# astra-vision/rain-rendering

Hardware: AMD Instinct MI355X
Metric: rainy frames/sec @ 1242x375, 100 mm/hr (higher is better)
Workload: dtype f64 alpha/mask, f32 colour

## Files before the change

__graft_entry__.py:

```python
import importlib
import os
import subprocess
import sys
import tempfile

ROOT = os.path.dirname(os.path.abspath(__file__))
if ROOT not in sys.path:
    sys.path.insert(0, ROOT)

CSRC = os.path.join(ROOT, 'rain-rendering_amd', 'csrc')
HIPCC = os.environ.get('HIPCC', '/opt/rocm/bin/hipcc')
HIP_FLAGS = ['--offload-arch=gfx950', '-O3', '-std=c++17', '-ffp-contract=off', '-fPIC', '-shared',
             '-Wno-unused-value', '-Wno-unused-result']


def _newer(target, sources):
    if not os.path.exists(target):
        return True
    t = os.path.getmtime(target)
    return any(os.path.getmtime(s) > t for s in sources)


def build(force=False):
    hip_src = os.path.join(CSRC, 'rainhip.hip')
    host_src = os.path.join(CSRC, 'rr_host.cpp')
    png_src = os.path.join(CSRC, 'rr_png.cpp')
    hip_dep = [hip_src, host_src, png_src] + sorted(os.path.join(CSRC, f) for f in os.listdir(CSRC) if f.endswith('.h')) + \
              [os.path.join(ROOT, 'include', 'rainhip.h')]
    lib = os.path.join(CSRC, 'librainhip.so')
    if force or _newer(lib, hip_dep):
        inc = ['-I' + os.path.join(ROOT, 'include'), '-I' + CSRC]
        objs = [os.path.join(CSRC, 'rainhip.o')]
        compile_flags = [f for f in HIP_FLAGS if f != '-shared']
        subprocess.check_call([HIPCC] + compile_flags + inc + ['-c', hip_src, '-o', objs[0]])
        for src in (host_src, png_src):
            obj = os.path.join(CSRC, os.path.basename(src)[:-4] + '.o')
            subprocess.check_call(['g++', '-O2', '-std=c++17', '-ffp-contract=off', '-fPIC', '-pthread', '-c'] + inc + [src, '-o', obj])
            objs.append(obj)
        subprocess.check_call([HIPCC, '--offload-arch=gfx950', '-fPIC', '-shared'] + objs + ['-lz', '-lpthread', '-o', lib])
    emu_src = os.path.join(ROOT, 'tests', 'hostemu', 'hostemu.cpp')
    emu = os.path.join(ROOT, 'tests', 'hostemu', 'libhostemu.so')
    if force or _newer(emu, [emu_src] + hip_dep[2:]):
        subprocess.check_call(['g++', '-O2', '-std=c++17', '-ffp-contract=off', '-fPIC', '-shared',
                               '-I' + os.path.join(ROOT, 'include'), '-I' + CSRC, emu_src, '-o', emu])
    noise_src = os.path.join(ROOT, 'tests', 'hostemu', 'noise_emu.cpp')
    noise_lib = os.path.join(ROOT, 'tests', 'hostemu', 'libnoiseemu.so')
    if force or _newer(noise_lib, [noise_src] + hip_dep[3:]):
        subprocess.check_call(['g++', '-O2', '-std=c++17', '-ffp-contract=off', '-fPIC', '-shared',
                               '-I' + os.path.join(ROOT, 'include'), '-I' + CSRC, noise_src, '-o', noise_lib])
    field_src = os.path.join(ROOT, 'tests', 'hostemu', 'field_emu.cpp')
    field_lib = os.path.join(ROOT, 'tests', 'hostemu', 'libfieldemu.so')
    if force or _newer(field_lib, [field_src] + hip_dep[3:]):
        subprocess.check_call(['g++', '-O2', '-std=c++17', '-ffp-contract=off', '-fPIC', '-shared',
                               '-I' + os.path.join(ROOT, 'include'), '-I' + CSRC, field_src, '-o', field_lib])
    rig_src = os.path.join(ROOT, 'tests', 'hostemu', 'rig_emu.cpp')
    rig_lib = os.path.join(ROOT, 'tests', 'hostemu', 'librigemu.so')
    if force or _newer(rig_lib, [rig_src] + hip_dep[3:]):
        subprocess.check_call(['g++', '-O2', '-std=c++17', '-ffp-contract=off', '-fPIC', '-shared',
                               '-I' + os.path.join(ROOT, 'include'), '-I' + CSRC, rig_src, '-o', rig_lib])
    importlib.import_module('rain-rendering_amd')
    hb = importlib.import_module('rain-rendering_amd.hip_backend')
    hb.load_library()


def smoke():
    import numpy as np
    build()
    sys.path.insert(0, os.path.join(ROOT, 'tests'))
    import helpers as h
    with tempfile.TemporaryDirectory() as tmp:
        sc = h.Scene(tmp, 96, 160, 120)
        bg, env = sc.frame_inputs(0)
        drops = sc.product_drops(0)
        rh = h.hb.RainHip(0)
        rh.set_streak_db(sc.db.streaks_light)
        rh.set_camera(sc.cam)
        out = rh.render_frames([dict(bg=bg, rainy_bg=bg, env_xyY=env, omega=sc.omega, drops=drops)])[0]
        ref = h.oracle_render(sc, 0, bg, bg, env, faithful=True)
        assert np.array_equal(out['status'], ref['status']), 'drop status mismatch'
        assert np.array_equal(out['mask'], ref['mask']), 'rainy_mask (f64) not bit-exact'
        assert np.array_equal(out['mask_i32'], ref['mask_i32']), 'rainy_mask (i32) not bit-exact'
        d = np.abs(out['image_u8'].astype(int) - ref['image_u8'].astype(int)).max()
        assert d <= 1, 'rainy_image differs by %d LSB' % d
        rh.close()
    print('smoke ok: %d drops, mask bit-exact, image max |d| = %d LSB' % (len(drops), d))


if __name__ == '__main__':
    build(force='--force' in sys.argv)
    if '--smoke' in sys.argv:
        smoke()
```

rain-rendering_amd/csrc/rainhip.hip:

```cpp
#include <hip/hip_runtime.h>

#include <dlfcn.h>

#include <cstddef>
#include <cstdio>
#include <cstdlib>
#include <algorithm>
#include <cstring>
#include <string>
#include <mutex>
#include <unordered_map>
#include <vector>

#include "rainhip.h"
#include "rr_device.h"
#include "rr_prepass.h"
#include "rr_deflate.h"
#include "rr_pngrows.h"
#include "rr_particles.h"

using namespace rr;

namespace {

// ... 59 lines not shown
    const global_ptr<const uint8_t> s = as_global(static_cast<const uint8_t*>(base)) + pix * 3;
    out[0] = (double)s[0] / 255.0; out[1] = (double)s[1] / 255.0; out[2] = (double)s[2] / 255.0;
  }
}
struct RawPx {
  uint32_t a, b, c, d, e, f;
};
typedef uint32_t u32x2_t __attribute__((ext_vector_type(2)));
__device__ inline void load_px3_raw2(const void* base, int kind, int64_t pa, int64_t pb, RawPx& qa, RawPx& qb) {
  if (kind == 0) {
    const global_ptr<const u32x2_t> s = as_global(static_cast<const u32x2_t*>(base));
    const u32x2_t a0 = s[pa * 3], a1 = s[pa * 3 + 1], a2 = s[pa * 3 + 2], b0 = s[pb * 3], b1 = s[pb * 3 + 1], b2 = s[pb * 3 + 2];
    qa = RawPx{a0.x, a0.y, a1.x, a1.y, a2.x, a2.y};
    qb = RawPx{b0.x, b0.y, b1.x, b1.y, b2.x, b2.y};
  } else if (kind == 1) {
    const global_ptr<const uint32_t> s = as_global(static_cast<const uint32_t*>(base));
    const uint32_t a0 = s[pa * 3], a1 = s[pa * 3 + 1], a2 = s[pa * 3 + 2], b0 = s[pb * 3], b1 = s[pb * 3 + 1], b2 = s[pb * 3 + 2];
    qa = RawPx{a0, a1, a2, 0u, 0u, 0u};
    qb = RawPx{b0, b1, b2, 0u, 0u, 0u};
  } else {
    const global_ptr<const uint8_t> s = as_global(static_cast<const uint8_t*>(base));
    const uint32_t a0 = s[pa * 3], a1 = s[pa * 3 + 1], a2 = s[pa * 3 + 2], b0 = s[pb * 3], b1 = s[pb * 3 + 1], b2 = s[pb * 3 + 2];
    qa = RawPx{a0, a1, a2, 0u, 0u, 0u};
    qb = RawPx{b0, b1, b2, 0u, 0u, 0u};
  }
}
__device__ inline void decode_px3(const RawPx& q, int kind, double out[3]) {
  if (kind == 0) {
    out[0] = __hiloint2double((int)q.b, (int)q.a);
    out[1] = __hiloint2double((int)q.d, (int)q.c);
    out[2] = __hiloint2double((int)q.f, (int)q.e);
  } else if (kind == 1) {
    out[0] = (double)__uint_as_float(q.a);
    out[1] = (double)__uint_as_float(q.b);
    out[2] = (double)__uint_as_float(q.c);
  } else {
    out[0] = (double)q.a / 255.0;
    out[1] = (double)q.b / 255.0;
    out[2] = (double)q.c / 255.0;
  }
}
__device__ inline int bg_kind(const FrameDesc& fr) { return (fr.in_types & RR_IN_BG_U8) ? 2 : ((fr.in_types & RR_IN_BG_F32) ? 1 : 0); }
__device__ inline int rainy_kind(const FrameDesc& fr) {
  if (fr.rainy_bg == fr.bg) return bg_kind(fr);
  return (fr.in_types & RR_IN_RAINY_U8) ? 2 : ((fr.in_types & RR_IN_RAINY_F32) ? 1 : 0);
}
typedef float float2_u __attribute__((ext_vector_type(2), aligned(4)));
typedef float float4_u __attribute__((ext_vector_type(4), aligned(4)));

__device__ inline void wave_lds_sync() {
  __builtin_amdgcn_fence(__ATOMIC_ACQ_REL, "wavefront");
  __builtin_amdgcn_wave_barrier();
}

#ifdef RR_PHASES
__device__ unsigned long long g_phase[8][8];
#define PH_DECL unsigned long long ph_t0_ = __builtin_readcyclecounter(), ph_acc_[8] = {0, 0, 0, 0, 0, 0, 0, 0};
#define PH_WAITVM asm volatile("s_waitcnt vmcnt(0)" ::: "memory");
#define PH(k)                                                   \
  {                                                             \
    const unsigned long long ph_n_ = __builtin_readcyclecounter(); \
    ph_acc_[k] += ph_n_ - ph_t0_;                               \
    ph_t0_ = ph_n_;                                             \
  }
#define PH_FLUSH(kid)                                           \
  if ((threadIdx.x & 63) == 0) {                                \
    for (int ph_q_ = 0; ph_q_ < 8; ph_q_++)                     \
      if (ph_acc_[ph_q_]) atomicAdd(&g_phase[kid][ph_q_], ph_acc_[ph_q_]); \
  }
#define PH_PARAMS , unsigned long long& ph_t0_, unsigned long long (&ph_acc_)[8]
#define PH_PASS , ph_t0_, ph_acc_
#define PH_COUNT(k) ph_acc_[k] += 1;
#else
#define PH_PARAMS
#define PH_PASS
#define PH_COUNT(k)
#define PH_DECL
#define PH_WAITVM
#define PH(k)
#define PH_FLUSH(kid)
#endif

struct Scratch {
  DropPlan* plan;
  CompRec* comp;
  CompRec32* comp32;
  int32_t* poly;
  int32_t* npts;
  int64_t* sizes;
  double* prefix;
  double* fband;
  double* arena;
  double* partial;
  double* means;
  int64_t* arena_need;
  int32_t* overflow;
  unsigned long long* need_max;
  int32_t* list_rot;
  int32_t* rot_total;
  int32_t* list_gen;
  int32_t* list_slow;
  int4* blur_items;
  int32_t* list_small;
  double* colpart;
  double* wtab;
  double* wtab_big;
  const uint8_t* tex_pad;
  const int64_t* tex_poff;
  uint4* fov_erec;
  uint32_t* fov_pix;
  int32_t* fov_list;
  int32_t* fov_list_n;
  uint8_t* blended;
  int32_t* pad_first;
  int32_t* eff_first;
  uint32_t* spans;
  int4* bbox;
  uint16_t* clist;
  int32_t* ccount;
  int32_t* counts;
  int32_t* list_big;
  int32_t* big_off;
  int32_t* bigs_list;
  int32_t* bigs_n;
  uint4* tkey;
  uint4* lrec;
  int32_t* canon;
  int32_t* htab;
  int32_t blur_bx, blur_by;
  int32_t* rows_list;
  int32_t* rows_n;
  int32_t* rows_hist;
  unsigned long long* rows_cost;
  int32_t* rows_next;
  int32_t* rows_bounds;
  int32_t* rows_fbase;
  int32_t* rows_sorted;
  const uint8_t* tex_pair;
  const int64_t* tex_qoff;
  int32_t colpart_f32;
  int32_t rows_on, n_tex;
  int32_t big_on, n_buckets;
};

__global__ __launch_bounds__(256) void k_env_prefix(const FrameDesc* frames, Dims dm, double* prefix) {
  const int lane = threadIdx.x & 63;
  const int row = blockIdx.x * 4 + (threadIdx.x >> 6), f = blockIdx.y;
  if (row >= dm.He) return;
  const FrameDesc& fr = frames[f];
  const int We = dm.We;
  const bool e32 = (fr.in_types & RR_IN_ENV_F32) != 0;
  const global_ptr<const double> env = as_global(static_cast<const double*>(fr.env)) + (int64_t)row * We * 3;
  const global_ptr<const double> om = as_global(static_cast<const double*>(fr.omega)) + (int64_t)row * We;
  const global_ptr<const float> envf = as_global(static_cast<const float*>(fr.env)) + (int64_t)row * We * 3;
  const global_ptr<const float> omf = as_global(static_cast<const float*>(fr.omega)) + (int64_t)row * We;
  double* P = prefix + ((int64_t)f * dm.He + row) * (int64_t)(We + 1) * 4;
  if (lane == 0) { P[0] = 0.0; P[1] = 0.0; P[2] = 0.0; P[3] = 0.0; }
  double carry[4] = {0, 0, 0, 0};
  for (int c0 = 0; c0 < We; c0 += 64) {
    const int c = c0 + lane;
    double v[4] = {0, 0, 0, 0};
    if (c < We) {
      const double w = e32 ? (double)omf[c] : om[c];
      v[0] = (e32 ? (double)envf[c * 3 + 0] : env[c * 3 + 0]) * w;
      v[1] = (e32 ? (double)envf[c * 3 + 1] : env[c * 3 + 1]) * w;
      v[2] = (e32 ? (double)envf[c * 3 + 2] : env[c * 3 + 2]) * w;
      v[3] = w;
    }
#pragma unroll
    for (int ofs = 1; ofs < 64; ofs <<= 1) {
#pragma unroll
      for (int k = 0; k < 4; k++) {
        const double u = __shfl_up(v[k], ofs);
        if (lane >= ofs) v[k] += u;
      }
    }
#pragma unroll
    for (int k = 0; k < 4; k++) v[k] += carry[k];
    if (c < We) {
      double* o = P + (int64_t)(c + 1) * 4;
      o[0] = v[0]; o[1] = v[1]; o[2] = v[2]; o[3] = v[3];
    }
#pragma unroll
    for (int k = 0; k < 4; k++) carry[k] = __shfl(v[k], 63);
  }
}

__global__ __launch_bounds__(256) void k_env_consts(Dims dm, const double* prefix, double* fband) {
  const int f = blockIdx.x, t = threadIdx.x;
  double sY = 0, sW = 0;
  for (int r = t; r < dm.He; r += 256) {
    const double* last = prefix + (((int64_t)f * dm.He + r) * (int64_t)(dm.We + 1) + dm.We) * 4;
    sY += last[2];
    sW += last[3];
  }
  __shared__ double a[256], b[256];
  a[t] = sY;
  b[t] = sW;
  __syncthreads();
  for (int ofs = 128; ofs > 0; ofs >>= 1) {
    if (t < ofs) {
      a[t] += a[t + ofs];
      b[t] += b[t + ofs];
    }
    __syncthreads();
  }
  if (t < COL_PARTS) {
    fband[(f * COL_PARTS + t) * 2 + 0] = t == 0 ? b[0] : 0.0;
    fband[(f * COL_PARTS + t) * 2 + 1] = t == 0 ? a[0] : 0.0;
  }
}

__device__ inline bool blur_is_slow(const DropPlan& p, const Scratch& sc) {
  return p.r1 > 0 && !blur_is_small(p) && !blur_layout(p, sc.blur_bx, sc.blur_by).fused;
}

constexpr int PLAN_DW = (int)(sizeof(DropPlan) / 4);
enum { LC_NONE = 0, LC_BIG_LDS = 1, LC_BIG = 2, LC_ROWS = 3, LC_ROT_INT = 4, LC_ROT = 5, LC_GEN = 6 };
enum { LB_NONE = 0, LB_SMALL = 1, LB_FUSED = 2, LB_SLOW = 3 };
__device__ inline uint4 make_list_rec(const DropPlan& p, const int32_t* tex_h, const int32_t* tex_w, const Scratch& sc);
__global__ __launch_bounds__(128) void k_plan(const FrameDesc* frames, Dims dm, rr_camera cam, const int32_t* tex_h,
                                              const int32_t* tex_w, int max_drops, int use_npts, Scratch sc) {
  static_assert(sizeof(DropPlan) % 4 == 0, "DropPlan layout");
  const int f = blockIdx.y;
  const int i = blockIdx.x * blockDim.x + threadIdx.x;
  const int lane = threadIdx.x & 63, wave = threadIdx.x >> 6;
  const FrameDesc& fr = frames[f];
  __shared__ uint32_t s_plan[2][32 * PLAN_DW];
  const bool act = i < fr.n_drops;
  const int64_t gi = (int64_t)f * max_drops + (act ? i : 0);
  DropPlan p;
  if (act) {
    rr_drop d = load_drop(fr.drops + i);
    int64_t size = 0;
    ExtGeom xg{false, 0, 0, 0, 0};
    if (fr.ext) {
      const rr_ext_tile& e = fr.ext[i];
      if (e.alpha) xg = ExtGeom{true, e.tw, e.th, e.min_x, e.min_y};
    }
    plan_drop<true>(d, cam, dm, tex_h, tex_w, fr.opacity, fr.strategy, p, size, xg);
    const int npts = use_npts ? sc.npts[gi] : 1;
    if (p.status != RR_DROP_OK || npts == 0) size = 0;
    if (size > 0 && blur_is_slow(p, sc)) size += ((int64_t)p.ew * p.eh + 15) & ~15LL;
    sc.sizes[gi] = size;
    uint32_t key[8];
    raw_tile_key(d, p, key);
    if (p.kind == KIND_EXT) key[0] = 0xffffffffu;
    sc.tkey[2 * gi] = make_uint4(key[0], key[1], key[2], key[3]);
    sc.tkey[2 * gi + 1] = make_uint4(key[4], key[5], key[6], key[7]);
    sc.lrec[gi] = make_list_rec(p, tex_h, tex_w, sc);
  }
  {
    const bool big = act && p.status == RR_DROP_OK && p.kind == KIND_BIG && sc.sizes[gi] > 0;
    const unsigned long long m = __ballot(big);
    if (m != 0ull) {
      int base = 0;
      if (lane == __ffsll((long long)m) - 1) base = atomicAdd(&sc.bigs_n[f], __popcll(m));
      base = __shfl(base, __ffsll((long long)m) - 1);
      if (big) sc.bigs_list[(int64_t)f * max_drops + base + __popcll(m & ((1ull << lane) - 1ull))] = i;
    }
  }
  const int wave_i0 = blockIdx.x * blockDim.x + wave * 64;
  uint32_t* stage = s_plan[wave];
  uint32_t* out = reinterpret_cast<uint32_t*>(sc.plan + (int64_t)f * max_drops + wave_i0);
#pragma unroll
  for (int half = 0; half < 2; half++) {
    if (act && (lane >> 5) == half) {
      const uint32_t* src = reinterpret_cast<const uint32_t*>(&p);
#pragma unroll
      for (int k = 0; k < PLAN_DW; k++) stage[(lane & 31) * PLAN_DW + k] = src[k];
    }
    wave_lds_sync();
    const int first = wave_i0 + half * 32;
    const int nrec = imax(imin(32, fr.n_drops - first), 0);
    for (int k = lane; k < nrec * PLAN_DW; k += 64) out[half * 32 * PLAN_DW + k] = stage[k];
    wave_lds_sync();
  }
}

__global__ __launch_bounds__(128) void k_plan_big(const FrameDesc* frames, const int32_t* tex_h, const int32_t* tex_w, int max_drops, Scratch sc) {
  const int f = blockIdx.y, j = blockIdx.x * blockDim.x + threadIdx.x;
  if (j >= sc.bigs_n[f]) return;
  const int i = sc.bigs_list[(int64_t)f * max_drops + j];
  const rr_drop d = load_drop(frames[f].drops + i);
  double mi[9];
  plan_big_homography(d, tex_w[d.tex_index], tex_h[d.tex_index], mi);
  double* o = sc.plan[(int64_t)f * max_drops + i].mi;
#pragma unroll
  for (int k = 0; k < 9; k++) o[k] = mi[k];
}

__global__ __launch_bounds__(1024) void k_scan(const FrameDesc* frames, int max_drops, int64_t arena_cap, Scratch sc) {
  const int f = blockIdx.x, t = threadIdx.x;
  const int n = frames[f].n_drops;
  const int chunk = (n + 1023) / 1024;
  const int i0 = t * chunk, i1 = min(i0 + chunk, n);
  const int64_t base = (int64_t)f * max_drops;
  int64_t s = 0;
  for (int i = i0; i < i1; i++) s += sc.sizes[base + i];
  __shared__ int64_t sh[1024];
  sh[t] = s;
  __syncthreads();
  for (int ofs = 1; ofs < 1024; ofs <<= 1) {
    int64_t v = (t >= ofs) ? sh[t - ofs] : 0;
    __syncthreads();
    sh[t] += v;
    __syncthreads();
  }
  int64_t run = ((t == 0) ? 0 : sh[t - 1]) + 16;
  const int64_t frame_base = (int64_t)f * arena_cap;
  if (t < 16 && arena_cap >= 16) sc.arena[frame_base + t] = 0.0;
  for (int i = i0; i < i1; i++) {
    DropPlan& p = sc.plan[base + i];
    int64_t sz = sc.sizes[base + i];
    if (run + sz > arena_cap) {
      sc.sizes[base + i] = 0;
    } else {
      p.a0_off = frame_base + run;
      p.a1_off = frame_base + run + (((int64_t)p.tw * p.th + 15) & ~15LL);
    }
    run += sz;
  }
  if (t == 1023) {
    const int64_t need = sh[1023] + 16;
    sc.arena_need[f] = need;
    if (need > arena_cap) {
      atomicExch(sc.overflow, 1);
      atomicMax(sc.need_max, (unsigned long long)need);
    }
  }
}

__device__ inline uint32_t raw_tile_hash(const uint4& a, const uint4& b) {
  uint32_t h = 2166136261u;
  auto mix = [&](uint32_t v) { h = (h ^ v) * 16777619u; };
  mix(a.x); mix(a.y); mix(a.z); mix(a.w); mix(b.x); mix(b.y); mix(b.z); mix(b.w);
  h ^= h >> 15;
  return h;
}
__global__ __launch_bounds__(256) void k_dedup(const FrameDesc* frames, int max_drops, int n_frames, int enable, Scratch sc) {
  const int f = blockIdx.y, i = blockIdx.x * 256 + (int)threadIdx.x;
  const int n = frames[f].n_drops;
  if (i >= n) return;
  const int gi = f * max_drops + i;
  const uint4 ka = sc.tkey[2 * (int64_t)gi], kb = sc.tkey[2 * (int64_t)gi + 1];
  int canon = gi;
  if (enable && ka.x != 0xffffffffu && sc.sizes[gi] != 0) {
    const uint32_t cap = 2u * (uint32_t)n_frames * (uint32_t)max_drops;
    uint32_t h = raw_tile_hash(ka, kb) % cap;
    for (;;) {
      const int prev = atomicCAS(&sc.htab[h], 0, gi + 1);
      if (prev == 0) break;
      const uint4 pa = sc.tkey[2 * (int64_t)(prev - 1)], pb = sc.tkey[2 * (int64_t)(prev - 1) + 1];
      if (pa.x == ka.x && pa.y == ka.y && pa.z == ka.z && pa.w == ka.w && pb.x == kb.x && pb.y == kb.y && pb.z == kb.z && pb.w == kb.w) {
        canon = prev - 1;
        break;
      }
      h = h + 1 == cap ? 0 : h + 1;
    }
    if (canon != gi) sc.plan[gi].a0_off = sc.plan[canon].a0_off;
  }
  sc.canon[gi] = canon;
  const unsigned long long dup = __ballot(canon != gi);
  if (dup != 0ull && (int)(threadIdx.x & 63) == __ffsll((long long)dup) - 1) atomicAdd(&sc.counts[f * 8 + 7], __popcll(dup));
}

constexpr int HE_MAX = 1024;
constexpr int FOV_WE_MAX = 4096;
constexpr int FOV_GROUPS = 3;

__device__ inline bool fov_rowspan_fast(const int32_t* px, const int32_t* py, int n, int y, int We, int& xl, int& xr) {
  int lo = 1 << 30, hi = -(1 << 30);
  for (int i = 0; i < n; i++) {
    const int j = (i + 1 == n) ? 0 : i + 1;
    const int x0 = px[i], y0 = py[i], x1 = px[j], y1 = py[j];
    const int ylo = imin(y0, y1), yhi = imax(y0, y1);
    if (y < ylo || y > yhi) continue;
    if (y0 == y1) {
      lo = imin(lo, imin(x0, x1));
      hi = imax(hi, imax(x0, x1));
    } else {
      const bool sw = y1 < y0;
      const int xa = sw ? x1 : x0, yA = sw ? y1 : y0, xb = sw ? x0 : x1, yB = sw ? y0 : y1;
      const int den = yB - yA;
      const int nn = 2 * (xb - xa) * (y - yA) + den;
      const int xv = xa + (int)floor((double)nn / (double)(2 * den));
      lo = imin(lo, xv);
      hi = imax(hi, xv);
    }
  }
  xl = imax(lo, 0);
  xr = imin(hi, We - 1);
  return xl <= xr;
}

template <int NCH, bool from_list>
__global__ __launch_bounds__(256) void k_fov_spans(const FrameDesc* frames, Dims dm, rr_camera cam, int max_drops, int Hp, int Dp, int use32, int cv_rule, Scratch sc) {
  const int f = blockIdx.y, wave = threadIdx.x >> 6, lane = threadIdx.x & 63;
  const FrameDesc& fr = frames[f];
  const int N = cam.n_fov, G = imin(64 / N, FOV_GROUPS);
  __shared__ double s_phi[2][RR_MAX_FOV];
  __shared__ float s_phi32[2][RR_MAX_FOV];
  __shared__ int s_px[4][FOV_GROUPS][POLY_STRIDE], s_py[4][FOV_GROUPS][POLY_STRIDE];
  __shared__ int s_xl[4][NCH * 64], s_xr[4][NCH * 64];
  __shared__ int4 s_edge[4][3 * POLY_STRIDE];
  if (threadIdx.x < RR_MAX_FOV) {
    s_phi[0][threadIdx.x] = cam.phi_cos[threadIdx.x];
    s_phi[1][threadIdx.x] = cam.phi_sin[threadIdx.x];
    s_phi32[0][threadIdx.x] = (float)cam.phi_cos[threadIdx.x];
    s_phi32[1][threadIdx.x] = (float)cam.phi_sin[threadIdx.x];
  }
  __syncthreads();
  const int n_eff = from_list ? sc.fov_list_n[f] : fr.n_drops;
  for (int wslot = blockIdx.x * 4 + wave; wslot * G < n_eff; wslot += gridDim.x * 4) {
  const int s0 = wslot * G;
  const int g = lane / N, k = lane - g * N;
  const bool act = g < G && s0 + g < n_eff;
  const int dg = act ? (from_list ? sc.fov_list[(int64_t)f * max_drops + s0 + g] : s0 + g) : 0;
  const int64_t gi = (int64_t)f * max_drops + dg;
  if (fr.strategy == 1) {
    if (act && k == 0) sc.npts[gi] = -1;
    return;
  }
  const bool ext = act && fr.ext && fr.ext[dg].alpha != nullptr;
  const int base = g * N, nxt_lane = base + (k + 1 == N ? 0 : k + 1);
  const unsigned long long gmask = act ? (((N >= 64 ? 0ull : (1ull << N)) - 1ull) << base) : 0ull;
  int ipx = 0, ipy = 0;
  bool cnd = false, vbad = true, ok = false;
  bool need64 = act && !ext && !use32;
  if (use32) {
    float azf = 0.f, erf = 0.f, pxf = 0.f, pyf = 0.f;
    int uns = 0;
    if (act && !ext) {
      FovSetup32 F;
      const rr_drop d = load_drop(fr.drops + dg);
      fov_setup32(d, (float)cam.fov_cos, (float)cam.fov_sin, F, uns);
      fov_vertex32(F, (float)cam.radius, s_phi32[0][k], s_phi32[1][k], dm.He, dm.We, azf, erf, pxf, pyf, uns);
    }
    const float az_n = __shfl(azf, act ? nxt_lane : lane), er_n = __shfl(erf, act ? nxt_lane : lane);
    bool c32 = false;
    if (act && !ext) c32 = fov_wrap_cnd32(azf, az_n, erf, er_n, uns);
    unsigned gor = 0;
#pragma unroll
// ... 656 lines not shown
  }
  for (int y = y0; y < y1; y++) row(y, RA, qa, qb);
#pragma unroll
  for (int d = 0; d < DPT; d++) {
    const int i = d0 + d * NT + t;
    if (i < d1) {
      float* o = reinterpret_cast<float*>(sc.colpart) + ((int64_t)(f * COL_PARTS + band) * 5) * max_drops + i;
#pragma unroll
      for (int k = 0; k < 4; k++) o[(int64_t)max_drops * k] = S[d][k];
      o[(int64_t)max_drops * 4] = ((any >> d) & 1u) ? 1.0f : 0.0f;
    }
  }
  {
    const int cl = (We - 1 - cw0) & ~1;
    if (chunk == 0 && We - 1 >= cw0 && cl < Cw && ((cl >> 1) & 63) == lane) {
      sc.fband[(f * COL_PARTS + band) * 2 + 0] = totw;
      sc.fband[(f * COL_PARTS + band) * 2 + 1] = totY;
    }
  }
}

__global__ __launch_bounds__(128) void k_fov_poly_general(const FrameDesc* frames, Dims dm, rr_camera cam, int max_drops, Scratch sc) {
  const int f = blockIdx.y, i = blockIdx.x * blockDim.x + threadIdx.x;
  const FrameDesc& fr = frames[f];
  if (i >= fr.n_drops) return;
  const int64_t gi = (int64_t)f * max_drops + i;
  int32_t* px = sc.poly + gi * 2 * POLY_STRIDE;
  const rr_drop d = load_drop(fr.drops + i);
  int npts = fov_polygon(d, cam, dm.He, dm.We, px, px + POLY_STRIDE);
  if (fr.strategy == 1) npts = -1;
  sc.npts[gi] = npts;
}

__global__ __launch_bounds__(256) void k_fov_sums_general(const FrameDesc* frames, Dims dm, int max_drops, Scratch sc, int cv_rule, int n_fov) {
  const int f = blockIdx.y;
  const int wave = threadIdx.x >> 6, lane = threadIdx.x & 63;
  const int i = blockIdx.x * 4 + wave;
  if (i >= frames[f].n_drops) return;
  const int64_t gi = (int64_t)f * max_drops + i;
  const int n = sc.npts[gi];
  double S[4] = {0, 0, 0, 0};
  int any = 0;
  if (n > 0) {
    const int32_t* px = sc.poly + gi * 2 * POLY_STRIDE;
    const int32_t* py = px + POLY_STRIDE;
    int ymin = lane < n ? py[lane] : 0x7fffffff, ymax = lane < n ? py[lane] : -0x7fffffff;
    for (int ofs = 32; ofs > 0; ofs >>= 1) {
      ymin = min(ymin, __shfl_xor(ymin, ofs));
      ymax = max(ymax, __shfl_xor(ymax, ofs));
    }
    const int ya = max(ymin, 0), yb = min(ymax, dm.He - 1);
    const double* P = sc.prefix + (int64_t)f * dm.He * (int64_t)(dm.We + 1) * 4;
    const bool cv = cv_rule && fov_fill_rule_cv_applies(px, py, n, n_fov, dm.He, dm.We);
    for (int y = ya + lane; y <= yb; y += 64) {
      int xl_, xr_;
      if (cv ? fov_rowspan_cv(px, py, n, y, dm.We, xl_, xr_) : fov_rowspan_fast(px, py, n, y, dm.We, xl_, xr_)) {
        any = 1;
        const double* row = P + (int64_t)y * (dm.We + 1) * 4;
        const double* hi = row + (int64_t)(xr_ + 1) * 4;
        const double* lo = row + (int64_t)xl_ * 4;
        for (int k = 0; k < 4; k++) S[k] += hi[k] - lo[k];
      }
    }
    for (int ofs = 32; ofs > 0; ofs >>= 1) {
      for (int k = 0; k < 4; k++) S[k] += __shfl_xor(S[k], ofs);
      any |= __shfl_xor(any, ofs);
    }
  }
  if (lane == 0) {
    for (int b = 0; b < COL_PARTS; b++) {
      double* o = sc.colpart + ((int64_t)(f * COL_PARTS + b) * 5) * max_drops + i;
      for (int k = 0; k < 4; k++) o[(int64_t)max_drops * k] = b == 0 ? S[k] : 0.0;
      o[(int64_t)max_drops * 4] = b == 0 ? (double)any : 0.0;
    }
  }
}

__global__ __launch_bounds__(256) void k_colour(const FrameDesc* frames, Dims dm, int max_drops, double cam_exposure, Scratch sc) {
  const int f = blockIdx.y;
  const int i = blockIdx.x * 256 + threadIdx.x;
  const FrameDesc& fr = frames[f];
  if (i >= fr.n_drops) return;
  const int64_t gi = (int64_t)f * max_drops + i;
  const DropPlan& p = sc.plan[gi];
  CompRec rec;
  rec.x0 = rec.y0 = rec.x1 = rec.y1 = 0;
  rec.ox = rec.oy = rec.pitch = rec.pad = 0;
  rec.off = 0;
  rec.tau_one = rec.g = 0;
  rec.K[0] = rec.K[1] = rec.K[2] = 0;
  rec.zdist = fr.depth ? fabs(as_global((const double*)fr.drops[i].wps)[2]) : 0.0;
  int status = p.status;
  bool blended = false;
  const int n = sc.npts[gi];
  if (n == 0) status = RR_DROP_FOV_FAIL;
  if (n < 0) {
    if (status == RR_DROP_OK && sc.sizes[gi] > 0) {
      blended = true;
      rec.K[0] = rec.K[1] = rec.K[2] = 1.0;
      rec.x0 = p.vis_x0;
      rec.y0 = p.vis_y0;
      rec.x1 = p.vis_x0 + p.vis_w;
      rec.y1 = p.vis_y0 + p.vis_h;
      rec.ox = -p.vis_x0;
      rec.oy = -p.vis_y0;
      rec.pitch = p.tw;
      rec.off = p.a0_off;
      rec.tau_one = p.tau_one;
      rec.g = p.g;
    }
  }
  if (n > 0) {
    double S[4] = {0, 0, 0, 0};
    bool any = false;
    double sumW = 0.0, sumY = 0.0;
    for (int b = 0; b < COL_PARTS; b++) {
      const int64_t at = ((int64_t)(f * COL_PARTS + b) * 5) * max_drops + i;
      if (sc.colpart_f32) {
        const float* part = reinterpret_cast<const float*>(sc.colpart) + at;
        for (int k = 0; k < 4; k++) S[k] += (double)part[(int64_t)max_drops * k];
        any = any || part[(int64_t)max_drops * 4] != 0.0f;
      } else {
        const double* part = sc.colpart + at;
        for (int k = 0; k < 4; k++) S[k] += part[(int64_t)max_drops * k];
        any = any || part[(int64_t)max_drops * 4] != 0.0;
      }
      sumW += sc.fband[(f * COL_PARTS + b) * 2 + 0];
      sumY += sc.fband[(f * COL_PARTS + b) * 2 + 1];
    }
    if (!any) status = RR_DROP_EMPTY_FOV;
    if (status == RR_DROP_OK && sc.sizes[gi] > 0) {
      blended = true;
      colour_from_sums(S, sumW, sumY / sumW, rec.K);
      if (p.r1 > 0) {
        const int fx0 = p.vis_x0 - p.crop_x + (p.shift - p.r2), fy0 = p.vis_y0 - p.crop_y + (p.shift - p.r1);
        rec.x0 = imax(p.vis_x0, fx0);
        rec.y0 = imax(p.vis_y0, fy0);
        rec.x1 = imin(p.vis_x0 + p.vis_w, fx0 + p.ew);
        rec.y1 = imin(p.vis_y0 + p.vis_h, fy0 + p.eh);
        if (rec.x1 <= rec.x0 || rec.y1 <= rec.y0) { rec.x0 = rec.y0 = rec.x1 = rec.y1 = 0; }
        rec.ox = -(fx0 - p.epad);
        rec.oy = -fy0;
        rec.pitch = p.epitch;
        rec.off = p.a1_off;
      } else {
        const int rx0 = p.vis_x0 - p.crop_x + p.shift, ry0 = p.vis_y0 - p.crop_y + p.shift;
        rec.x0 = imax(p.vis_x0, rx0);
        rec.y0 = imax(p.vis_y0, ry0);
        rec.x1 = imin(p.vis_x0 + p.vis_w, rx0 + p.tw);
        rec.y1 = imin(p.vis_y0 + p.vis_h, ry0 + p.th);
        if (rec.x1 <= rec.x0 || rec.y1 <= rec.y0) { rec.x0 = rec.y0 = rec.x1 = rec.y1 = 0; }
        rec.ox = -rx0;
        rec.oy = -ry0;
        rec.pitch = p.tw;
        rec.off = p.a0_off;
      }
      rec.tau_one = p.tau_one;
      rec.g = p.g;
    }
  }
  {
    const double BIG = 1.0e50;
    const bool tame = fabs(rec.tau_one) < BIG && (rec.tau_one == 0.0 || rec.tau_one > 1.0e-200) && fabs(rec.g) < BIG &&
                      fabs(rec.K[0]) < BIG && fabs(rec.K[1]) < BIG && fabs(rec.K[2]) < BIG && p.kind != KIND_EXT;
    rec.pad = tame ? 0 : 1;
  }
  sc.comp[gi] = rec;
// ... 105 lines not shown
constexpr int BIG_ROWS_MAX_PX = 8192;
__device__ inline bool tile_is_big_lds(const DropPlan& p, int sh, int sw) {
  return p.kind == KIND_BIG && (int64_t)(sh + 4) * (sw + 4) + 48 <= RW_PAIR_BYTES && p.tw >= 1 && p.th >= 1 && (int64_t)p.tw * p.th <= BIG_ROWS_MAX_PX && p.bw0 >= 1;
}
__global__ __launch_bounds__(256) void k_pair_textures(const uint8_t* texels, const int32_t* tex_h, const int32_t* tex_w,
                                                       const int64_t* tex_off, const int64_t* tex_qoff, uint8_t* pairs) {
  const int i = blockIdx.x, sh = tex_h[i], sw = tex_w[i], P = pair_pitch(sw);
  const uint8_t* g = texels + tex_off[i];
  uint16_t* dst = reinterpret_cast<uint16_t*>(pairs + tex_qoff[i]);
  for (int k = threadIdx.x; k < (sh + 3) * P; k += 256) {
    const int y = k / P - 2, x = k - (y + 2) * P - 2;
    const bool xin = x >= 0 && x < sw;
    const uint32_t lo = (xin && y >= 0 && y < sh) ? g[y * sw + x] : 0u, hi = (xin && y + 1 >= 0 && y + 1 < sh) ? g[(y + 1) * sw + x] : 0u;
    dst[k] = (uint16_t)(lo | (hi << 8));
  }
}

__global__ __launch_bounds__(256) void k_pad_textures(const uint8_t* texels, const int32_t* tex_h, const int32_t* tex_w,
                                                      const int64_t* tex_off, const int64_t* tex_poff, uint8_t* pad) {
  const int i = blockIdx.x, sh = tex_h[i], sw = tex_w[i], P = sw + 4;
  const uint8_t* g = texels + tex_off[i];
  uint8_t* dst = pad + tex_poff[i];
  for (int k = threadIdx.x; k < (sh + 4) * P; k += 256) {
    const int y = k / P - 2, x = k - (y + 2) * P - 2;
    dst[k] = (y >= 0 && y < sh && x >= 0 && x < sw) ? g[y * sw + x] : (uint8_t)0;
  }
}
__device__ inline void load_tex_copy(uint8_t* s_tex, const uint8_t* gpad, int sh, int sw) {
  const int n16 = ((sh + 4) * (sw + 4) + 15) >> 4;
  const uint4* g = reinterpret_cast<const uint4*>(gpad);
  uint4* d = reinterpret_cast<uint4*>(s_tex);
  for (int k = threadIdx.x; k < n16; k += 256) d[k] = g[k];
}

__device__ inline double lds_rot_sample(const uint8_t* s_tex, const double* s_lut, int P, int sh, int sw, int X0, int Y0,
                                        int2 d) {
  const int X = (X0 + d.x) >> 5, Y = (Y0 + d.y) >> 5;
  int sx = X >> 5, sy = Y >> 5;
  const int fx = X & 31, fy = Y & 31;
  sx = imin(imax(sx, -2), sw);
  sy = imin(imax(sy, -2), sh);
  const uint8_t* q = s_tex + (sy + 2) * P + (sx + 2);
  const double v00 = s_lut[q[0]], v01 = s_lut[q[1]], v10 = s_lut[q[P]], v11 = s_lut[q[P + 1]];
  const double ax_ = (double)(32 - fx), bx_ = (double)fx, ay_ = (double)(32 - fy), by_ = (double)fy;
  const double sm = ((v00 * (ay_ * ax_) + v01 * (ay_ * bx_)) + v10 * (by_ * ax_)) + v11 * (by_ * bx_);
  return sm * (1.0 / 1024.0);
}

__device__ inline void lds_rot_sample2(const uint8_t* s_tex, const double* s_lut, int P, int sh, int sw, int XA, int YA, int2 dA,
                                       int XB, int YB, int2 dB, double& outA, double& outB) {
  const int Xa = (XA + dA.x) >> 5, Ya = (YA + dA.y) >> 5, Xb = (XB + dB.x) >> 5, Yb = (YB + dB.y) >> 5;
  const int sxa = imin(imax(Xa >> 5, -2), sw), sya = imin(imax(Ya >> 5, -2), sh);
  const int sxb = imin(imax(Xb >> 5, -2), sw), syb = imin(imax(Yb >> 5, -2), sh);
  const uint8_t* qa = s_tex + (sya + 2) * P + (sxa + 2);
  const uint8_t* qb = s_tex + (syb + 2) * P + (sxb + 2);
  const int a0 = qa[0], a1 = qa[1], a2 = qa[P], a3 = qa[P + 1];
  const int b0 = qb[0], b1 = qb[1], b2 = qb[P], b3 = qb[P + 1];
  const double va0 = s_lut[a0], va1 = s_lut[a1], va2 = s_lut[a2], va3 = s_lut[a3];
  const double vb0 = s_lut[b0], vb1 = s_lut[b1], vb2 = s_lut[b2], vb3 = s_lut[b3];
  const int fxa = Xa & 31, fya = Ya & 31, fxb = Xb & 31, fyb = Yb & 31;
  const double axa = (double)(32 - fxa), bxa = (double)fxa, aya = (double)(32 - fya), bya = (double)fya;
  const double axb = (double)(32 - fxb), bxb = (double)fxb, ayb = (double)(32 - fyb), byb = (double)fyb;
  const double sa = ((va0 * (aya * axa) + va1 * (aya * bxa)) + va2 * (bya * axa)) + va3 * (bya * bxa);
  const double sb = ((vb0 * (ayb * axb) + vb1 * (ayb * bxb)) + vb2 * (byb * axb)) + vb3 * (byb * bxb);
  outA = sa * (1.0 / 1024.0);
  outB = sb * (1.0 / 1024.0);
}

constexpr int GEN_SLICES = 16;
__global__ __launch_bounds__(256) void k_tile_generic(const FrameDesc* frames, int max_drops, const uint8_t* texels,
                                                      const int32_t* tex_h, const int32_t* tex_w, const int64_t* tex_off,
                                                      const float* ctab, Scratch sc) {
  const int f = blockIdx.y, t = threadIdx.x;
  __shared__ double s_lut[256];
  __shared__ __attribute__((aligned(16))) uint8_t s_tex[TEX_LDS];
  __shared__ int2 s_adbd[NW_MAX];
  const int n_items = sc.counts[f * 8 + 1];
  if ((int)blockIdx.x >= n_items * GEN_SLICES) return;
  s_lut[t] = (double)t / 255.0;
  for (int work = blockIdx.x; work < n_items * GEN_SLICES; work += gridDim.x) {
  const int item = work / GEN_SLICES, slice = work - item * GEN_SLICES;
  const int li = sc.list_gen[(int64_t)f * max_drops + item];
  const int64_t gi = (int64_t)f * max_drops + li;
  const DropPlan& p = sc.plan[gi];
  if (p.kind == KIND_EXT) {
    const double* src = frames[f].ext[li].alpha;
    double* A0e = sc.arena + p.a0_off;
    for (int idx = t + 256 * slice; idx < p.tw * p.th; idx += 256 * GEN_SLICES) A0e[idx] = clip01(src[idx]);
    continue;
  }
  const int sh = tex_h[p.tex], sw = tex_w[p.tex];
  __syncthreads();
  const uint8_t* gtex = texels + tex_off[p.tex];
  const int P = sw + 4;
  const bool tex_fits = (sh + 4) * P <= TEX_LDS && !(p.kind == KIND_BIG && p.tw * p.th * 12 < sh * sw);
  if (tex_fits) load_tex_copy(s_tex, sc.tex_pad + sc.tex_poff[p.tex], sh, sw);
  double* A0 = sc.arena + p.a0_off;
  const bool area_fast = tex_fits && p.kind == KIND_ROT && p.rs_mode == RS_AREA_FAST && p.nW <= NW_MAX && tile_coords_safe(p);
  if (area_fast)
    for (int rx = t; rx < p.nW; rx += 256) s_adbd[rx] = make_int2((int)rot_adelta(p, rx), (int)rot_bdelta(p, rx));
  __syncthreads();
  const int n = p.tw * p.th;
  if (area_fast) {
    const int area = p.isx * p.isy, n4 = area & ~3;
    const float scale = 1.0f / (float)area;
    for (int idx = t + 256 * slice; idx < n; idx += 256 * GEN_SLICES) {
      const int dy = idx / p.tw, dx = idx - dy * p.tw;
      double sum = 0.0, q0 = 0.0, q1 = 0.0, q2 = 0.0;
      int k = 0;
      for (int ky = 0; ky < p.isy; ky++) {
        const int c = dy * p.isy + ky;
        const int ry = p.flip ? (p.nH - 1 - c) : c;
        const int X0 = (int)rot_X0(p, ry), Y0 = (int)rot_Y0(p, ry);
        for (int kx = 0; kx < p.isx; kx++, k++) {
          const double v = lds_rot_sample(s_tex, s_lut, P, sh, sw, X0, Y0, s_adbd[dx * p.isx + kx]);
          if (k >= n4) sum = sum + v;
          else {
            const int m = k & 3;
            if (m == 0) q0 = v;
            else if (m == 1) q1 = v;
            else if (m == 2) q2 = v;
            else sum = sum + (((q0 + q1) + q2) + v);
          }
        }
      }
      A0[dy * p.tw + dx] = clip01(sum * (double)scale);
    }
  } else if (tex_fits) {
    TexLutPad tx{s_tex, s_lut, sh, sw};
    for (int idx = t + 256 * slice; idx < n; idx += 256 * GEN_SLICES) {
      int y = idx / p.tw, x = idx - y * p.tw;
      A0[idx] = raw_tile_pixel(p, tx, ctab, x, y);
    }
  } else {
    TexLut tx{gtex, s_lut, sh, sw};
    for (int idx = t + 256 * slice; idx < n; idx += 256 * GEN_SLICES) {
      int y = idx / p.tw, x = idx - y * p.tw;
      A0[idx] = raw_tile_pixel(p, tx, ctab, x, y);
    }
  }
  }
}


struct TexLutWide {
  const uint8_t* t;
  const double* lut;
  int h, w;
  __device__ double at(int64_t y, int64_t x) const { return lut[t[y * w + x]]; }
  __device__ void at4(int64_t y, int64_t x, double v[4]) const {
    uint32_t u;
    __builtin_memcpy(&u, as_global(t) + (y * w + x), 4);
    v[0] = lut[u & 0xffu]; v[1] = lut[(u >> 8) & 0xffu]; v[2] = lut[(u >> 16) & 0xffu]; v[3] = lut[u >> 24];
  }
  __device__ double tap(int64_t y, int64_t x) const {
    if (y < 0 || y >= h || x < 0 || x >= w) return 0.0;
    return at(y, x);
  }
};

__global__ __launch_bounds__(256) void k_tile_big(const FrameDesc* frames, int max_drops, const uint8_t* texels,
                                                  const int32_t* tex_h, const int32_t* tex_w, const int64_t* tex_off,
                                                  const float* ctab, Scratch sc) {
  const int f = blockIdx.y, t = threadIdx.x;
  __shared__ double s_lut[256];
  __shared__ float s_ctab[128];
  const int n_big = sc.counts[f * 8 + 5], total = sc.counts[f * 8 + 6];
  if (total == 0) return;
  s_lut[t] = (double)t / 255.0;
  if (t < 128) s_ctab[t] = ctab[t];
  const int32_t* lbig = sc.list_big + (int64_t)f * max_drops;
  const int32_t* boff = sc.big_off + (int64_t)f * max_drops + f;
  const int lane = t & 63;
  __syncthreads();
  PH_DECL
  for (int pb = blockIdx.x * 256; pb < total; pb += gridDim.x * 256) {
    const int pix0 = pb + (t & ~63);
    if (pix0 >= total) continue;
    int lo = 0, hi = n_big;
    while (hi - lo > 1) {
      const int step = (hi - lo + 63) >> 6, idx = lo + lane * step;
      const bool le = idx < hi && boff[idx] <= pix0;
      const int cnt = __popcll(__ballot(le));
      lo += (cnt - 1) * step;
      hi = imin(hi, lo + step);
    }
    PH(0)
    const int pix = pb + t;
    if (pix >= total) continue;
    int j = lo;
    while (boff[j + 1] <= pix) j++;
    const int64_t gi = (int64_t)f * max_drops + lbig[j];
    const DropPlan& p = sc.plan[gi];
    const int local = pix - boff[j];
    const int y = local / p.tw, x = local - y * p.tw;
    TexLutWide tx{texels + tex_off[p.tex], s_lut, tex_h[p.tex], tex_w[p.tex]};
    PH(1)
    sc.arena[p.a0_off + local] = warp_big_pixel(p, tx, s_ctab, x, y);
    PH(2)
  }
  PH_FLUSH(1)
}

__global__ __launch_bounds__(256) void k_tile(const FrameDesc* frames, int max_drops, const uint8_t* texels,
                                              const int32_t* tex_h, const int32_t* tex_w, const int64_t* tex_off,
                                              Scratch sc) {
  const int t = threadIdx.x, lane = t & 63, wave = t >> 6;
  __shared__ DropPlan sp;
  __shared__ double s_lut[256];
  __shared__ __attribute__((aligned(16))) uint8_t s_tex[TEX_LDS];
  __shared__ int2 s_adbd[NW_MAX];
  __shared__ AreaSpan s_ax[TW_MAX];
  __shared__ double s_buf[BUF_MAX];
  __shared__ double s_can[4][CAN_W];
  __shared__ int4 s_row[4][ROWS_S];
  const int n_items = *sc.rot_total;
  if ((int)blockIdx.x >= n_items) return;
  s_lut[t] = (double)t / 255.0;
  PH_DECL
  for (int item = blockIdx.x; item < n_items; item += gridDim.x) {
  const int64_t gi = sc.list_rot[item];
  __syncthreads();
  PH(7)
  {
    const int32_t* src = reinterpret_cast<const int32_t*>(&sc.plan[gi]);
    int32_t* dst = reinterpret_cast<int32_t*>(&sp);
    for (int k = t; k < (int)(sizeof(DropPlan) / 4); k += 256) dst[k] = src[k];
  }
  __syncthreads();
  const DropPlan& p = sp;
  const int sh = tex_h[p.tex], sw = tex_w[p.tex];
  const int P = sw + 4;
  load_tex_copy(s_tex, sc.tex_pad + sc.tex_poff[p.tex], sh, sw);
  double* A0 = sc.arena + p.a0_off;
  const int tw = p.tw, th = p.th;
  const double sy_scale = p.scale_y;
  for (int rx = t; rx < p.nW; rx += 256) s_adbd[rx] = make_int2((int)rot_adelta(p, rx), (int)rot_bdelta(p, rx));
  for (int dx = t; dx < tw; dx += 256) s_ax[dx] = area_span(p.nW, p.scale_x, dx);
  __syncthreads();
  PH(0)
  const RowGeom geom = row_geom(p, sh, sw);
  const int pitch = imin(imax(tile_pitch(p, sh, sw), 1), CAN_W);
  const int Rw = imax(imin(ROWS_W, CAN_W / pitch), 1);
  const float inv_pitch = 1.0f / (float)pitch;
  double* can = s_can[wave];
  int4* rowp = s_row[wave];
  if (p.rs_mode == RS_AREA_FAST) {
    const int isx = p.isx, isy = p.isy, area = isx * isy, n4 = area & ~3;
    const float scale = 1.0f / (float)area;
    const int nsplit = th >= 3 ? 1 : (th == 2 ? 2 : 4);
    const int rows_par = 4 / nsplit;
    for (int dyb = 0; dyb < th; dyb += rows_par) {
      const int dy = dyb + wave / nsplit, part = wave % nsplit;
      const int dx0 = (part * tw) / nsplit, dx1 = ((part + 1) * tw) / nsplit;
      if (dy >= th || dx1 <= dx0) continue;
      const int colA = dx0 * isx, colB = dx1 * isx;
      const int pitch2 = imax(imin(pitch, colB - colA), 1);
      const int Rw2 = imax(imin(ROWS_W, CAN_W / pitch2), 1);
      const float inv_pitch2 = 1.0f / (float)pitch2;
      double sum = 0.0, q0 = 0.0, q1 = 0.0, q2 = 0.0;
      int k = 0;
      for (int c0 = dy * isy; c0 < (dy + 1) * isy; c0 += Rw2) {
        const int nr = imin(Rw2, (dy + 1) * isy - c0);
        if (lane < nr) {
          const int c = c0 + lane;
          const int ry = p.flip ? (p.nH - 1 - c) : c;
          const int X0 = (int)rot_X0(p, ry), Y0 = (int)rot_Y0(p, ry);
          int xa, n;
          row_interval(p, geom, X0, Y0, xa, n);
          const int xa2 = imax(xa, colA), xe2 = imin(xa + n, colB);
          rowp[lane] = make_int4(X0, Y0, xa2, imax(imin(xe2 - xa2, pitch2), 0));
        }
        wave_lds_sync();
        const int nidx = nr * pitch2;
        for (int idx = lane; idx < nidx; idx += 128) {
          const int ia = idx, ib = imin(idx + 64, nidx - 1);
          const int ra = (int)(((float)ia + 0.5f) * inv_pitch2), xa = ia - ra * pitch2;
          const int rb = (int)(((float)ib + 0.5f) * inv_pitch2), xb = ib - rb * pitch2;
          const int4 rwa = rowp[ra], rwb = rowp[rb];
          const bool oka = xa < rwa.w, okb = (idx + 64 < nidx) && xb < rwb.w;
          const int2 da = s_adbd[rwa.z + (oka ? xa : 0)], db = s_adbd[rwb.z + (okb ? xb : 0)];
          double va, vb;
          lds_rot_sample2(s_tex, s_lut, P, sh, sw, rwa.x, rwa.y, da, rwb.x, rwb.y, db, va, vb);
          if (oka) can[ia] = va;
          if (okb) can[ib] = vb;
        }
        wave_lds_sync();
        const bool mine = lane < dx1 - dx0;
        const int colL = (dx0 + lane) * isx;
        for (int r = 0; r < nr; r++) {
          const int4 rw = rowp[r];
          const double* row = can + r * pitch2 - rw.z;
          const int vlo = mine ? rw.z : (1 << 30), vhi = rw.z + rw.w;
          auto at = [&](int col) { return (col >= vlo && col < vhi) ? row[col] : 0.0; };
          int kx = 0;
          while (kx < isx) {
            if ((k & 3) == 0 && kx + 3 < isx && k + 3 < n4) {
              const double v0 = at(colL + kx), v1 = at(colL + kx + 1), v2 = at(colL + kx + 2), v3 = at(colL + kx + 3);
              sum = sum + (((v0 + v1) + v2) + v3);
              kx += 4;
              k += 4;
              continue;
            }
            const double v = at(colL + kx);
            if (k >= n4) sum = sum + v;
            else {
              const int m = k & 3;
              if (m == 0) q0 = v;
              else if (m == 1) q1 = v;
              else if (m == 2) q2 = v;
// ... 379 lines not shown
    for (int k = 0; k < NP; k++) {
      const int bx = tw <= bw0 ? 0 : div_by_f(x, bw0, inv_bw) * bw0;
      c[k] = warp_big_coord(p, bx, x, y);
      x += dr;
      y += dq;
      if (x >= tw) { x -= tw; y += 1; }
    }
    uint32_t u[NP][4];
    float cx[NP][4], cy[NP][4];
#pragma unroll
    for (int k = 0; k < NP; k++) {
      const uint8_t* col = tex00 + med3i(c[k].sx, -4, sw);
#pragma unroll
      for (int i = 0; i < 4; i++) {
        const uint32_t a = (uint32_t)(uintptr_t)(const __attribute__((address_space(3))) uint8_t*)(col + med3i(c[k].sy + i, -2, sh + 1) * P);
        const uint32_t* q = (const uint32_t*)(__attribute__((address_space(3))) uint32_t*)(uintptr_t)(a & ~3u);
        const uint32_t lo = q[0], hi = q[1];
        u[k][i] = __builtin_amdgcn_alignbit(hi, lo, (a & 3u) * 8u);
      }
      const float4 a = *reinterpret_cast<const float4*>(s_ctab + c[k].fx * 4), b = *reinterpret_cast<const float4*>(s_ctab + c[k].fy * 4);
      cx[k][0] = a.x; cx[k][1] = a.y; cx[k][2] = a.z; cx[k][3] = a.w;
      cy[k][0] = b.x; cy[k][1] = b.y; cy[k][2] = b.z; cy[k][3] = b.w;
    }
#pragma unroll
    for (int k = 0; k < NP; k++) {
      double pr[4][4];
#pragma unroll
      for (int i = 0; i < 4; i++) big_row_products(u[k][i], cy[k][i], cx[k], three, pr[i]);
      const bool interior = c[k].sx >= 0 && c[k].sx < width1 && c[k].sy >= 0 && c[k].sy < height1;
      double sum = 0.0;
      if (interior) {
#pragma unroll
        for (int i = 0; i < 4; i++) {
          double r = (pr[i][0] + pr[i][1]) + pr[i][2];
          r = r + pr[i][3];
          sum = (i == 0) ? r : sum + r;
        }
      } else {
#pragma unroll
        for (int i = 0; i < 4; i++)
#pragma unroll
          for (int j = 0; j < 4; j++) sum = sum + pr[i][j];
      }
      const int it = it0 + 64 * k + lane;
      if (it < n) A0[it] = clip01(sum);
    }
  }
  PH(7)
}

__global__ __launch_bounds__(1024) void k_tile_rows(int n_shares, const int32_t* tex_h, const int32_t* tex_w, const float* ctab, Scratch sc) {
  __shared__ __attribute__((aligned(16))) RowsShared S;
  const int t = threadIdx.x, lane = t & 63, wave = t >> 6;
  if ((uint32_t)(uintptr_t)(__attribute__((address_space(3))) double*)S.lut != 0u) __builtin_trap();
  S.lut[t & 255] = (double)(t & 255) / 255.0;
  RowsWave& W = S.w[wave];
  uint32_t three = 3;
  asm volatile("" : "+v"(three));
  constexpr int DONE = 0x7fffffff;
  PH_DECL
  if (t == 0) S.cur = -1;
  for (;;) {
    __syncthreads();
    if (t == 0) {
      const int share = (int)atomicAdd(sc.rows_next, 1);
      const bool any = share < n_shares;
      S.next = any ? sc.rows_bounds[share] : 0;
      S.end = any ? sc.rows_bounds[share + 1] : 0;
      S.first = any ? 1 : 0;
    }
    __syncthreads();
    if (!S.first) break;
    const int end = S.end;
    int pending = -1, ptex = -1, gi = 0;
    bool ctab_ok = false;
    for (;;) {
      if (pending < 0) {
        int i = 0;
        if (lane == 0) i = atomicAdd(&S.next, 1);
        i = __builtin_amdgcn_readfirstlane(i);
        if (i < end) {
          pending = i;
          gi = __builtin_amdgcn_readfirstlane(sc.rows_sorted[i]);
          ptex = __builtin_amdgcn_readfirstlane(as_constant(&sc.plan[gi])->tex);
          if (__builtin_amdgcn_readfirstlane(as_constant(&sc.plan[gi])->kind) == KIND_BIG) ptex += sc.n_tex;
        } else {
          pending = DONE;
        }
      }
      if (pending != DONE && ptex == S.cur) {
        DropPlan p;
        {
          const const_ptr<uint32_t> src = as_constant(reinterpret_cast<const uint32_t*>(&sc.plan[gi]));
          uint32_t* dst = reinterpret_cast<uint32_t*>(&p);
#pragma unroll
          for (int k = 0; k < (int)(sizeof(DropPlan) / 4); k++) dst[k] = src[k];
        }
        PH(0)
        if (ptex < sc.n_tex) {
          rows_tile(p, tex_h[ptex], tex_w[ptex], S, W, sc.arena, three PH_PASS);
          ctab_ok = false;
        } else {
          float* s_ctab = reinterpret_cast<float*>(W.buf);
          if (!ctab_ok) {
            wave_lds_sync();
            s_ctab[lane] = ctab[lane];
            s_ctab[lane + 64] = ctab[lane + 64];
            wave_lds_sync();
            ctab_ok = true;
          }
          big_tile<RR_BIG_NP>(p, tex_h[ptex - sc.n_tex], tex_w[ptex - sc.n_tex], S.pair, s_ctab, sc.arena, three PH_PASS);
        }
        pending = -1;
        continue;
      }
      if (lane == 0) { S.pend[wave] = pending; S.ptex[wave] = ptex; }
      __syncthreads();
      int m = DONE, mtex = -1;
      for (int k = 0; k < RW_WAVES; k++)
        if (S.pend[k] < m) { m = S.pend[k]; mtex = S.ptex[k]; }
      if (m == DONE) break;
      if (mtex < sc.n_tex) {
        const int64_t nb = pair_bytes(tex_h[mtex], tex_w[mtex]);
        const uint4* g = reinterpret_cast<const uint4*>(sc.tex_pair + sc.tex_qoff[mtex]);
        uint4* d = reinterpret_cast<uint4*>(S.pair);
        for (int k = t; k < (int)(nb >> 4); k += 1024) d[k] = g[k];
      } else {
        const int bt = mtex - sc.n_tex;
        const int n16 = ((tex_h[bt] + 4) * (tex_w[bt] + 4) + 2 + 15) >> 4;
        const uint4* g = reinterpret_cast<const uint4*>(sc.tex_pad + sc.tex_poff[bt]);
        uint4* d = reinterpret_cast<uint4*>(S.pair);
        if (t == 0) d[0] = uint4{0u, 0u, 0u, 0u};
        for (int k = t; k < n16; k += 1024) d[k + 1] = g[k];
      }
      if (t == 0) S.cur = mtex;
      __syncthreads();
      PH(5)
    }
  }
  PH_FLUSH(5)
}

constexpr int BLUR_ITEMS_PER_DROP = 8;

__device__ inline int blur_subtiles(const DropPlan& p, const BlurLayout& L) {
  return ((p.ew + L.wo - 1) / L.wo) * ((p.eh + L.ho - 1) / L.ho);
}

__device__ inline uint4 make_list_rec(const DropPlan& p, const int32_t* tex_h, const int32_t* tex_w, const Scratch& sc) {
  if (p.status != RR_DROP_OK) return make_uint4(0u, 0u, 0u, 0u);
  const int sh = tex_h[p.tex], sw = tex_w[p.tex];
  uint32_t cls, cost = 0u, bcls = LB_NONE, bwh = 0u, bns = 0u;
  if (p.kind == KIND_BIG) {
    if (sc.big_on && tile_is_big_lds(p, sh, sw)) { cls = LC_BIG_LDS; cost = (uint32_t)(RR_BIG_COST * ((p.tw * p.th + 63) / 64) + 4); }
    else { cls = LC_BIG; cost = (uint32_t)(p.tw * p.th); }
  } else if (sc.rows_on && p.kind != KIND_EXT && tile_is_rows(p, sh, sw)) { cls = LC_ROWS; cost = (uint32_t)rows_tile_cost(p, sh, sw); }
  else if (p.kind != KIND_EXT && tile_is_fast(p, sh, sw)) cls = p.rs_mode == RS_AREA_FAST ? LC_ROT_INT : LC_ROT;
  else cls = LC_GEN;
  if (p.r1 > 0) {
    if (blur_is_small(p)) bcls = LB_SMALL;
    else {
      const BlurLayout L = blur_layout(p, sc.blur_bx, sc.blur_by);
      if (L.fused) { bcls = LB_FUSED; bwh = (uint32_t)L.wo | ((uint32_t)L.ho << 16); bns = (uint32_t)blur_subtiles(p, L); }
      else bcls = LB_SLOW;
    }
  }
  return make_uint4(cls | (bcls << 4) | ((uint32_t)p.tex << 8), cost, bwh, bns);
}

__global__ __launch_bounds__(1024) void k_lists(const FrameDesc* frames, int max_drops, const int32_t* tex_h, const int32_t* tex_w,
                                                Scratch sc) {
  const int f = blockIdx.x, t = threadIdx.x;
  const int n = frames[f].n_drops;
  const int chunk = (n + 1023) / 1024;
  const int i0 = t * chunk, i1 = min(i0 + chunk, n);
  const int64_t base = (int64_t)f * max_drops;
  __shared__ int s_hist[RW_TEX_MAX], s_cost[RW_TEX_MAX];
  if (sc.rows_on) {
    for (int k = t; k < sc.n_buckets; k += 1024) s_hist[k] = s_cost[k] = 0;
    __syncthreads();
  }
  constexpr int NC = 11;
  int c[NC] = {0, 0, 0, 0, 0, 0, 0, 0, 0, 0, 0};
  for (int i = i0; i < i1; i++) {
    const uint4 r = sc.lrec[base + i];
    const uint32_t cls = r.x & 15u, bcls = (r.x >> 4) & 7u;
    if (cls == LC_NONE || sc.sizes[base + i] == 0) continue;
    const int tex = (int)(r.x >> 8);
    if (sc.canon[base + i] == (int)(base + i)) {
      if (cls == LC_BIG_LDS) {
        c[9]++;
        c[10] += sc.plan[base + i].tw * sc.plan[base + i].th;
        atomicAdd(&s_hist[sc.n_tex + tex], 1);
        atomicAdd(&s_cost[sc.n_tex + tex], (int)r.y);
      } else if (cls == LC_BIG) { c[6]++; c[7] += (int)r.y; }
      else if (cls == LC_ROWS) {
        c[8]++;
        atomicAdd(&s_hist[tex], 1);
        atomicAdd(&s_cost[tex], (int)r.y);
      }
      else if (cls == LC_ROT_INT) c[5]++;
      else if (cls == LC_ROT) c[0]++;
      else c[1]++;
    }
    if (bcls == LB_SMALL) c[4]++;
    else if (bcls == LB_FUSED) c[2] += imin((int)r.w, BLUR_ITEMS_PER_DROP);
    else if (bcls == LB_SLOW) c[3]++;
  }
  __shared__ int sh[1024][NC];
  for (int k = 0; k < NC; k++) sh[t][k] = c[k];
  __syncthreads();
  for (int ofs = 1; ofs < 1024; ofs <<= 1) {
    int v[NC] = {0, 0, 0, 0, 0, 0, 0, 0, 0, 0, 0};
    if (t >= ofs)
      for (int k = 0; k < NC; k++) v[k] = sh[t - ofs][k];
    __syncthreads();
    for (int k = 0; k < NC; k++) sh[t][k] += v[k];
    __syncthreads();
  }
  int o[NC];
  for (int k = 0; k < NC; k++) o[k] = (t == 0) ? 0 : sh[t - 1][k];
  const int n_int = sh[1023][5];
  const int n_rot_rows = sh[1023][8];
  o[0] += n_int;
  __shared__ int s_rot_base;
  if (t == 0) s_rot_base = atomicAdd(sc.rot_total, sh[1023][0] + sh[1023][5]);
  __syncthreads();
  int32_t* lrot = sc.list_rot + s_rot_base;
  int32_t* lgen = sc.list_gen + base;
  int32_t* lslow = sc.list_slow + base;
  int32_t* lsmall = sc.list_small + base;
  int32_t* lbig = sc.list_big + base;
  int32_t* lrows = sc.rows_list + base;
  int32_t* boff = sc.big_off + base + f;
  int4* items = sc.blur_items + base * BLUR_ITEMS_PER_DROP;
  for (int i = i0; i < i1; i++) {
    const uint4 r = sc.lrec[base + i];
    const uint32_t cls = r.x & 15u, bcls = (r.x >> 4) & 7u;
    if (cls == LC_NONE || sc.sizes[base + i] == 0) continue;
    if (sc.canon[base + i] == (int)(base + i)) {
      if (cls == LC_BIG_LDS) lrows[n_rot_rows + o[9]++] = i;
      else if (cls == LC_BIG) {
        boff[o[6]] = o[7];
        lbig[o[6]++] = i;
        o[7] += (int)r.y;
      } else if (cls == LC_ROWS) lrows[o[8]++] = i;
      else if (cls == LC_ROT_INT) lrot[o[5]++] = (int32_t)(base + i);
      else if (cls == LC_ROT) lrot[o[0]++] = (int32_t)(base + i);
      else lgen[o[1]++] = i;
    }
    if (bcls == LB_SMALL) lsmall[o[4]++] = i;
    else if (bcls == LB_FUSED) {
      const int ns = (int)r.w;
      const int ni = imin(ns, BLUR_ITEMS_PER_DROP);
      const int per = (ns + ni - 1) / ni;
      for (int k = 0; k < ni; k++) {
        const int st0 = k * per;
        items[o[2]++] = make_int4(i, st0, imax(imin(per, ns - st0), 0), (int)r.z);
      }
    } else if (bcls == LB_SLOW) lslow[o[3]++] = i;
  }
  if (t == 1023) {
    for (int k = 0; k < 5; k++) sc.counts[f * 8 + k] = sh[1023][k];
    sc.counts[f * 8 + 0] = sh[1023][0] + sh[1023][5];
    sc.counts[f * 8 + 5] = sh[1023][6];
    sc.counts[f * 8 + 6] = sh[1023][7];
    boff[sh[1023][6]] = sh[1023][7];
    sc.rows_n[3 * f] = sh[1023][8];
    sc.rows_n[3 * f + 1] = sh[1023][9];
    sc.rows_n[3 * f + 2] = sh[1023][10];
  }
  if (sc.rows_on) {
    for (int k = t; k < sc.n_buckets; k += 1024) {
      const int cnt = s_hist[k];
      sc.rows_fbase[(int64_t)f * RW_TEX_MAX + k] = cnt ? atomicAdd(&sc.rows_hist[k], cnt) : 0;
      if (cnt) atomicAdd(&sc.rows_cost[k], (unsigned long long)s_cost[k]);
    }
  }
}

__global__ __launch_bounds__(1024) void k_rows_scatter(int max_drops, Scratch sc) {
  const int f = blockIdx.x, t = threadIdx.x;
  __shared__ int s_start[RW_TEX_MAX], s_rank[RW_TEX_MAX];
  const int nf = sc.rows_n[3 * f] + sc.rows_n[3 * f + 1];
  if (nf == 0) return;
  const int own = t < sc.n_buckets ? sc.rows_hist[t] : 0;
  s_start[t] = own;
  __syncthreads();
  for (int ofs = 1; ofs < 1024; ofs <<= 1) {
    const int v = t >= ofs ? s_start[t - ofs] : 0;
    __syncthreads();
    s_start[t] += v;
    __syncthreads();
  }
  const int excl = s_start[t] - own;
  __syncthreads();
  s_start[t] = excl;
  s_rank[t] = t < sc.n_buckets ? sc.rows_fbase[(int64_t)f * RW_TEX_MAX + t] : 0;
  __syncthreads();
  const int64_t base = (int64_t)f * max_drops;
  for (int j = t; j < nf; j += 1024) {
    const int i = sc.rows_list[base + j];
    const DropPlan& p = sc.plan[base + i];
    const int tex = p.tex + (p.kind == KIND_BIG ? sc.n_tex : 0);
    const int pos = s_start[tex] + atomicAdd(&s_rank[tex], 1);
    sc.rows_sorted[pos] = (int32_t)(base + i);
  }
}

__device__ void gauss_half_table(double sigma, int r, double* hw ) {
  const int t = threadIdx.x;
  for (int k = t; k <= r; k += blockDim.x) hw[k] = gauss_phi(sigma, r - k);
  __syncthreads();
  __shared__ double s_tot;
  if (t == 0) {
    double tot = 0.0;
    for (int x = -r; x <= r; x++) tot = tot + hw[r - (x < 0 ? -x : x)];
    s_tot = tot;
  }
  __syncthreads();
  const double tot = s_tot;
  for (int k = t; k <= r; k += blockDim.x) hw[k] = hw[k] / tot;
  __syncthreads();
}


constexpr int BW_LANES = 4;
__global__ __launch_bounds__(256) void k_blur_weights(const FrameDesc* frames, int max_drops, Scratch sc) {
  constexpr int NG = 256 / BW_LANES;
  __shared__ double s_hw[NG][BR_MAX + 2];
  const int f = blockIdx.y, grp = threadIdx.x / BW_LANES, l = threadIdx.x % BW_LANES;
  const int idx = blockIdx.x * NG + grp;
  const int i = idx >> 1, axis = idx & 1;
  int r = 0;
  double sigma = 0.0;
  const int64_t gi = (int64_t)f * max_drops + (i < frames[f].n_drops ? i : 0);
  if (i < frames[f].n_drops) {
    const DropPlan& p = sc.plan[gi];
    if (p.status == RR_DROP_OK && sc.sizes[gi] != 0 && p.r1 > 0 && p.r1 <= BR_MAX) {
      r = axis ? p.r2 : p.r1;
      sigma = axis ? p.sig2 : p.sig1;
    }
  }
  double* tab = s_hw[grp];
  for (int k = l; k <= r && r > 0; k += BW_LANES) tab[k] = gauss_phi(sigma, r - k);
  wave_lds_sync();
  if (l == 0 && r > 0) {
    double tot = 0.0;
    for (int x = -r; x <= r; x++) tot = tot + tab[r - (x < 0 ? -x : x)];
    tab[BR_MAX + 1] = tot;
  }
  wave_lds_sync();
  if (r > 0) {
    const double tot = tab[BR_MAX + 1];
    double* hw = sc.wtab + (gi * 2 + axis) * (BR_MAX + 1);
    for (int k = l; k <= r; k += BW_LANES) hw[k] = tab[k] / tot;
  }
}

template <class W>
__device__ inline void blur4(const double* c0, int st, W hw, int r, double& acc0, double& acc1, double& acc2, double& acc3) {
  auto at = [&](int k) { return c0[__mul24(k, st)]; };
  const double wc = hw(r);
  acc0 = c0[0] * wc; acc1 = at(1) * wc; acc2 = at(2) * wc; acc3 = at(3) * wc;
  double a0 = at(-r), a1 = at(1 - r), a2 = at(2 - r), a3 = at(3 - r);
  double b0 = at(r), b1 = at(1 + r), b2 = at(2 + r), b3 = at(3 + r);
  int ii = -r;
  for (; ii + 3 < 0; ii += 4) {
    const double w0 = hw(ii + r), w1 = hw(ii + 1 + r), w2 = hw(ii + 2 + r), w3 = hw(ii + 3 + r);
    const double na0 = at(4 + ii), na1 = at(5 + ii), na2 = at(6 + ii), na3 = at(7 + ii);
    const double nb0 = at(-ii - 1), nb1 = at(-ii - 2), nb2 = at(-ii - 3), nb3 = at(-ii - 4);
    acc0 = acc0 + (a0 + b0) * w0; acc1 = acc1 + (a1 + b1) * w0; acc2 = acc2 + (a2 + b2) * w0; acc3 = acc3 + (a3 + b3) * w0;
    acc0 = acc0 + (a1 + nb0) * w1; acc1 = acc1 + (a2 + b0) * w1; acc2 = acc2 + (a3 + b1) * w1; acc3 = acc3 + (na0 + b2) * w1;
    acc0 = acc0 + (a2 + nb1) * w2; acc1 = acc1 + (a3 + nb0) * w2; acc2 = acc2 + (na0 + b0) * w2; acc3 = acc3 + (na1 + b1) * w2;
    acc0 = acc0 + (a3 + nb2) * w3; acc1 = acc1 + (na0 + nb1) * w3; acc2 = acc2 + (na1 + nb0) * w3; acc3 = acc3 + (na2 + b0) * w3;
    a0 = na0; a1 = na1; a2 = na2; a3 = na3;
    b3 = nb0; b2 = nb1; b1 = nb2; b0 = nb3;
  }
  for (; ii < 0; ii++) {
    const double w = hw(ii + r);
    const double na = at(4 + ii);
    const double nb = at(-ii - 1);
    acc0 = acc0 + (a0 + b0) * w;
    acc1 = acc1 + (a1 + b1) * w;
    acc2 = acc2 + (a2 + b2) * w;
    acc3 = acc3 + (a3 + b3) * w;
    a0 = a1; a1 = a2; a2 = a3; a3 = na;
    b3 = b2; b2 = b1; b1 = b0; b0 = nb;
  }
}

template <int NO, class W>
__device__ inline void blur_n(const double* c0, int st, W hw, int r, double (&acc)[NO]) {
  const double wc = hw(r);
#pragma unroll
  for (int j = 0; j < NO; j++) acc[j] = c0[__mul24(j, st)] * wc;
  for (int ii = -r; ii < 0; ii++) {
    const double w = hw(ii + r);
#pragma unroll
    for (int j = 0; j < NO; j++) acc[j] = acc[j] + (c0[__mul24(j + ii, st)] + c0[__mul24(j - ii, st)]) * w;
  }
}

__device__ inline void glds_dword(const void* src, uint32_t lds_byte) {
  uint32_t keep;
  asm volatile("s_mov_b32 %0, m0\n\ts_mov_b32 m0, %2\n\ts_nop 0\n\tglobal_load_lds_dword %1, off\n\ts_mov_b32 m0, %0"
               : "=&s"(keep)
               : "v"(src), "s"(__builtin_amdgcn_readfirstlane((int)lds_byte))
               : "memory");
}
__device__ inline void glds_dwordx4(const void* src, uint32_t lds_byte) {
  uint32_t keep;
  asm volatile("s_mov_b32 %0, m0\n\ts_mov_b32 m0, %2\n\ts_nop 0\n\tglobal_load_lds_dwordx4 %1, off\n\ts_mov_b32 m0, %0"
               : "=&s"(keep)
               : "v"(src), "s"(__builtin_amdgcn_readfirstlane((int)lds_byte))
               : "memory");
}
__global__ __launch_bounds__(256, 4) void k_blur_fused_dma(const FrameDesc* frames, int max_drops, Scratch sc) {
  const int f = blockIdx.y, t = threadIdx.x, lane = t & 63, G = gridDim.x;
  const int wave = __builtin_amdgcn_readfirstlane(t >> 6);
  extern __shared__ __attribute__((aligned(16))) double s_dyn[];
  constexpr int TAB = 2 * (BR_MAX + 1);
  double* tabs = s_dyn;
  double* X = s_dyn + 2 * TAB;
  double* Y = X + sc.blur_bx;
  const uint32_t lds_tabs = (uint32_t)(uintptr_t)(__attribute__((address_space(3))) double*)tabs;
  const uint32_t lds_x = (uint32_t)(uintptr_t)(__attribute__((address_space(3))) double*)X;
  const int n_items = sc.counts[f * 8 + 2];
  if ((int)blockIdx.x >= n_items) return;
  const global_ptr<const uint32_t> items_w = as_global(reinterpret_cast<const uint32_t*>(sc.blur_items + (int64_t)f * max_drops * BLUR_ITEMS_PER_DROP));
  const DropPlan* plans = sc.plan + (int64_t)f * max_drops;
  auto load_item = [&](int item) { return items_w[(int64_t)item * 4 + (lane & 3)]; };
  auto load_plan = [&](int i) { return as_global(reinterpret_cast<const uint32_t*>(plans + i))[lane]; };
  struct PlanView {
    int r1, r2, ew, eh, tw, th, epitch, epad;
    long long a0_off, a1_off;
  };
  auto unpack = [&](uint32_t pv) {
    auto F = [&](size_t byte_off) { return (int)__builtin_amdgcn_readlane((int)pv, (int)(byte_off / 4)); };
    PlanView o;
    o.r1 = F(offsetof(DropPlan, r1)); o.r2 = F(offsetof(DropPlan, r2)); o.ew = F(offsetof(DropPlan, ew)); o.eh = F(offsetof(DropPlan, eh));
    o.tw = F(offsetof(DropPlan, tw)); o.th = F(offsetof(DropPlan, th)); o.epitch = F(offsetof(DropPlan, epitch)); o.epad = F(offsetof(DropPlan, epad));
    o.a0_off = (long long)(((unsigned long long)(unsigned)F(offsetof(DropPlan, a0_off) + 4) << 32) | (unsigned)F(offsetof(DropPlan, a0_off)));
    o.a1_off = (long long)(((unsigned long long)(unsigned)F(offsetof(DropPlan, a1_off) + 4) << 32) | (unsigned)F(offsetof(DropPlan, a1_off)));
    return o;
  };
  auto item_of = [&](uint32_t iv) {
    return make_int4((int)__builtin_amdgcn_readlane((int)iv, 0), (int)__builtin_amdgcn_readlane((int)iv, 1),
                     (int)__builtin_amdgcn_readlane((int)iv, 2), (int)__builtin_amdgcn_readlane((int)iv, 3));
  };
  struct Geo {
    int y0, x0, ho, wo, hop, hi, yp, xa, wd, nx, xs, ys, e_lo, e_hi;
  };
  auto geo = [&](const PlanView& p, int Lwo, int Lho, int st) {
    Geo g;
    const int ntx = (p.ew + Lwo - 1) / Lwo;
    const int sty = st / ntx, stx = st - sty * ntx;
    g.y0 = sty * Lho; g.x0 = stx * Lwo;
    g.ho = imin(Lho, p.eh - g.y0);
    g.wo = imin(Lwo, p.ew - g.x0);
    g.hop = (g.ho + 3) & ~3;
    const int wi = g.wo + 2 * p.r2;
    g.hi = g.hop + 2 * p.r1;
    g.yp = blur_y_pitch(g.wo, p.r2);
    g.xa = imax(0, 2 * p.r2 - g.x0);
    const int xb = imin(wi, p.tw + 2 * p.r2 - g.x0);
    g.wd = imax(xb - g.xa, 0);
    g.nx = g.wd * g.hi;
    g.xs = g.x0 - 2 * p.r2 + g.xa; g.ys = g.y0 - 2 * p.r1;
    const int ra = imin(imax(-g.ys, 0), g.hi), rb = imax(imin(p.th - g.ys, g.hi), ra);
    g.e_lo = ra * g.wd; g.e_hi = rb * g.wd;
    return g;
  };
  auto stage = [&](const PlanView& p, const Geo& g, int drop, bool tables, int tb) {
    if (g.e_hi > g.e_lo && g.wd == p.tw) {
      const char* src = reinterpret_cast<const char*>(sc.arena + p.a0_off + (int64_t)g.ys * p.tw);
      const int a = (g.e_lo + 1) & ~1, b = g.e_hi & ~1;
      for (int e0 = (a & ~511); e0 < b; e0 += 512) {
        const int e = e0 + wave * 128 + 2 * lane;
        if (e >= a && e < b) glds_dwordx4(src + (int64_t)e * 8, lds_x + (uint32_t)(e0 + wave * 128) * 8u);
      }
      if (wave == 0 && (g.e_lo & 1) && lane < 2) glds_dword(src + (int64_t)g.e_lo * 8 + lane * 4, lds_x + (uint32_t)g.e_lo * 8u);
      if (wave == 1 && (g.e_hi & 1) && g.e_hi - 1 >= g.e_lo && lane < 2) glds_dword(src + (int64_t)(g.e_hi - 1) * 8 + lane * 4, lds_x + (uint32_t)(g.e_hi - 1) * 8u);
    } else if (g.e_hi > g.e_lo) {
      const int wdd = imax(g.wd, 1);
      const float inv_wd = 1.0f / (float)wdd;
      const int dq = (int)((128.0f + 0.5f) * inv_wd), dr = 128 - dq * wdd;
      const char* src = reinterpret_cast<const char*>(sc.arena + p.a0_off) + (lane & 1) * 4;
      const int c0 = g.e_lo >> 7, c1 = (g.e_hi + 127) >> 7;
      int e = c0 * 128 + wave * 32 + (lane >> 1);
      int yy = (int)(((float)e + 0.5f) * inv_wd), xc = e - yy * wdd;
      for (int c = c0; c < c1; c++) {
        if (e >= g.e_lo && e < g.e_hi)
          glds_dword(src + (int64_t)((g.ys + yy) * p.tw + (g.xs + xc)) * 8, lds_x + (uint32_t)(c * 128 + wave * 32) * 8u);
        e += 128;
        xc += dr;
        yy += dq;
        if (xc >= wdd) { xc -= wdd; yy += 1; }
      }
    }
    if (tables) {
      const char* wt = reinterpret_cast<const char*>(sc.wtab + ((int64_t)f * max_drops + drop) * TAB);
      if (wave == 3 && lane < TAB / 2) glds_dwordx4(wt + lane * 16, lds_tabs + (uint32_t)(tb * TAB) * 8u);
    }
  };
  uint32_t iv0 = load_item(blockIdx.x);
  uint32_t pv0 = load_plan((int)__builtin_amdgcn_readlane((int)iv0, 0));
  uint32_t iv1 = load_item(imin((int)blockIdx.x + G, n_items - 1));
  uint32_t pv1 = load_plan((int)__builtin_amdgcn_readlane((int)iv1, 0));
  uint32_t iv2 = load_item(imin((int)blockIdx.x + 2 * G, n_items - 1));
  int it = blockIdx.x;
  int4 item = item_of(iv0);
  PlanView p = unpack(pv0);
  int st = item.y, tb = 0;
  Geo g = geo(p, item.w & 0xffff, item.w >> 16, st);
  stage(p, g, item.x, true, tb);
  PH_DECL
  for (;;) {
    const int r1 = p.r1, r2 = p.r2;
    const double* hw1 = tabs + tb * TAB;
    const double* hw2 = hw1 + (BR_MAX + 1);
    {
      const int nz2 = (g.yp * g.hop + 1) >> 1;
      double2* Y2 = reinterpret_cast<double2*>(Y);
      for (int i = t; i < nz2; i += 256) Y2[i] = make_double2(0.0, 0.0);
    }
    asm volatile("s_waitcnt vmcnt(0)" ::: "memory");
// ... 12 lines not shown
        has_next = false;
      }
    }
    {
      iv1 = new_item ? iv2 : iv1;
      pv1 = load_plan((int)__builtin_amdgcn_readlane((int)iv1, 0));
      iv2 = load_item(imin(new_item ? it + 3 * G : it + 2 * G, n_items - 1));
    }
    for (int i = t; i < g.e_lo; i += 256) X[i] = 0.0;
    for (int i = g.e_hi + t; i < g.nx; i += 256) X[i] = 0.0;
    PH(0)
    __syncthreads();
    PH(1)
    {
      const int wd = g.wd, nrb = g.hop >> 2, nv = nrb * wd;
      const float inv_wd = 1.0f / (float)imax(wd, 1);
      for (int idx = t; idx < nv; idx += 256) {
        const int rb = (int)(((float)idx + 0.5f) * inv_wd), xq = idx - rb * wd;
        const double* c0 = X + (4 * rb + r1) * wd + xq;
        double acc0, acc1, acc2, acc3;
        blur4(c0, wd, [&](int k) { return hw1[k]; }, r1, acc0, acc1, acc2, acc3);
        double* o = Y + 4 * rb * g.yp + g.xa + xq;
        o[0] = acc0;
        o[g.yp] = acc1;
        o[2 * g.yp] = acc2;
        o[3 * g.yp] = acc3;
      }
    }
    PH(2)
    __syncthreads();
    PH(3)
    Geo ng = g;
    if (has_next) {
      ng = geo(np, nitem.w & 0xffff, nitem.w >> 16, nst);
      stage(np, ng, nitem.x, ntb != tb, ntb);
    }
    PH(6)
    {
      const int ncb = (g.wo + 3) >> 2, nh = ncb * g.ho;
      const float inv_ho = 1.0f / (float)g.ho;
      double* dst = sc.arena + p.a1_off;
      for (int idx = t; idx < nh; idx += 256) {
        const int cb = (int)(((float)idx + 0.5f) * inv_ho), yq = idx - cb * g.ho;
        const double* c0 = Y + yq * g.yp + 4 * cb + r2;
        double acc0, acc1, acc2, acc3;
        if (r2 > 0) {
          blur4(c0, 1, [&](int k) { return hw2[k]; }, r2, acc0, acc1, acc2, acc3);
        } else {
          acc0 = c0[0]; acc1 = c0[1]; acc2 = c0[2]; acc3 = c0[3];
        }
        const int xo = 4 * cb;
        double* o = dst + (int64_t)(g.y0 + yq) * p.epitch + p.epad + (g.x0 + xo);
        if (xo + 3 < g.wo) {
          o[0] = acc0; o[1] = acc1; o[2] = acc2; o[3] = acc3;
        } else {
          o[0] = acc0;
          if (xo + 1 < g.wo) o[1] = acc1;
          if (xo + 2 < g.wo) o[2] = acc2;
        }
      }
    }
    PH(4)
    if (!has_next) break;
    __syncthreads();
    PH(5)
    if (new_item) it += G;
    item = nitem; p = np; st = nst; tb = ntb; g = ng;
  }
  PH_FLUSH(3)
}

typedef double double2_v __attribute__((ext_vector_type(2)));
struct SmallItem {
  int li, r1, r2, tw, th, pw, ph, epitch, epad;
  long long a0, a1;
};
__global__ __launch_bounds__(256, 4) void k_blur_small(const FrameDesc* frames, int max_drops, Scratch sc) {
  const int f = blockIdx.y, lane = threadIdx.x & 63, wave = threadIdx.x >> 6;
  __shared__ __attribute__((aligned(16))) double Xs[4][BS_X], Ys[4][BS_Y];
  double* X = Xs[wave];
  double* Y = Ys[wave];
  const int n_items = sc.counts[f * 8 + 4];
  const global_ptr<const int32_t> list = as_global(sc.list_small + (int64_t)f * max_drops);
  const DropPlan* plans = sc.plan + (int64_t)f * max_drops;
  const int stride = gridDim.x * 4;
  int it = blockIdx.x * 4 + wave;
  if (it >= n_items) return;
  auto load_plan = [&](int li) { return as_global(reinterpret_cast<const uint32_t*>(plans + li))[lane]; };
  auto unpack = [&](uint32_t pv, int li) {
    auto F = [&](size_t byte_off) { return (int)__builtin_amdgcn_readlane((int)pv, (int)(byte_off / 4)); };
    static_assert(offsetof(DropPlan, a1_off) + 8 <= 256, "DropPlan layout");
    SmallItem o;
    o.li = li;
    o.r1 = F(offsetof(DropPlan, r1)); o.r2 = F(offsetof(DropPlan, r2)); o.tw = F(offsetof(DropPlan, tw)); o.th = F(offsetof(DropPlan, th));
    o.pw = F(offsetof(DropPlan, ew)); o.ph = F(offsetof(DropPlan, eh)); o.epitch = F(offsetof(DropPlan, epitch)); o.epad = F(offsetof(DropPlan, epad));
    o.a0 = (long long)(((unsigned long long)(unsigned)F(offsetof(DropPlan, a0_off) + 4) << 32) | (unsigned)F(offsetof(DropPlan, a0_off)));
    o.a1 = (long long)(((unsigned long long)(unsigned)F(offsetof(DropPlan, a1_off) + 4) << 32) | (unsigned)F(offsetof(DropPlan, a1_off)));
    return o;
  };
  double2_v R[4];
  double nw1 = 0.0, nw2 = 0.0;
  auto issue = [&](const SmallItem& d) {
    const global_ptr<const double2_v> raw2 = as_global(reinterpret_cast<const double2_v*>(sc.arena + d.a0));
    const int n = d.tw * d.th;
#pragma unroll
    for (int j = 0; j < 4; j++) {
      const int k2 = lane + 64 * j;
      R[j] = double2_v{0.0, 0.0};
      if (2 * k2 < n) R[j] = raw2[k2];
    }
    const global_ptr<const double> wt = as_global(sc.wtab + ((int64_t)f * max_drops + d.li) * 2 * (BR_MAX + 1));
    nw1 = (lane <= d.r1) ? wt[d.r1 - lane] : 0.0;
    nw2 = (d.r2 > 0 && lane <= d.r2) ? wt[(BR_MAX + 1) + d.r2 - lane] : 0.0;
  };
  PH_DECL
  const int li0 = __builtin_amdgcn_readfirstlane(list[it]);
  SmallItem cur = unpack(load_plan(li0), li0);
  issue(cur);
  bool has_next = it + stride < n_items;
  int li1 = has_next ? __builtin_amdgcn_readfirstlane(list[it + stride]) : li0;
  uint32_t pv_next = load_plan(li1);
  int32_t li2_v = (it + 2 * stride < n_items) ? list[it + 2 * stride] : 0;
  for (;;) {
    const int r1 = cur.r1, r2 = cur.r2, pw = cur.pw, ph = cur.ph, tw = cur.tw, th = cur.th;
    const int php = (ph + 3) & ~3, hi = php + 2 * r1, yp = blur_y_pitch(pw, r2);
    double* tile = sc.arena + cur.a1;
    {
      const int n = tw * th, top = 2 * r1 * tw;
      double2* X2 = reinterpret_cast<double2*>(X);
#pragma unroll
      for (int j = 0; j < 4; j++) {
        const int k2 = lane + 64 * j;
        if (2 * k2 < n) X2[(top >> 1) + k2] = make_double2(R[j].x, 2 * k2 + 1 < n ? R[j].y : 0.0);
      }
      for (int i = lane; i < (top >> 1); i += 64) X2[i] = make_double2(0.0, 0.0);
      const int e0 = (top + n + 1) >> 1, e1 = (tw * hi + 1) >> 1;
      for (int i = e0 + lane; i < e1; i += 64) X2[i] = make_double2(0.0, 0.0);
      const int nz2 = (yp * php + 1) >> 1;
      double2* Y2 = reinterpret_cast<double2*>(Y);
      for (int i = lane; i < nz2; i += 64) Y2[i] = make_double2(0.0, 0.0);
    }
    const double w1 = nw1, w2 = nw2;
    wave_lds_sync();
    PH(0)
    SmallItem nxt = cur;
    if (has_next) {
      nxt = unpack(pv_next, li1);
      issue(nxt);
      if (it + 2 * stride < n_items) {
        li1 = __builtin_amdgcn_readfirstlane(li2_v);
        pv_next = load_plan(li1);
        if (it + 3 * stride < n_items) li2_v = list[it + 3 * stride];
      }
    }
    const float inv_tw = 1.0f / (float)tw;
    const int nv4 = (php >> 2) * tw;
    if (nv4 <= 16) {
      const int idx = lane;
      if (idx < 4 * nv4) {
        const int row = (int)(((float)idx + 0.5f) * inv_tw), x = idx - row * tw;
        double a[1];
        blur_n<1>(X + (__mul24(row + r1, tw) + x), tw, [&](int k) { return readlane_f64(w1, r1 - k); }, r1, a);
        Y[__mul24(row, yp) + 2 * r2 + x] = a[0];
      }
    } else if (nv4 <= 32) {
      const int idx = lane;
      if (idx < 2 * nv4) {
        const int rb = (int)(((float)idx + 0.5f) * inv_tw), x = idx - rb * tw;
        double a[2];
        blur_n<2>(X + (__mul24(2 * rb + r1, tw) + x), tw, [&](int k) { return readlane_f64(w1, r1 - k); }, r1, a);
        double* o = Y + (__mul24(2 * rb, yp) + 2 * r2 + x);
        o[0] = a[0];
        o[yp] = a[1];
      }
    } else {
      const int nv = nv4;
      for (int idx = lane; idx < nv; idx += 64) {
        const int rb = (int)(((float)idx + 0.5f) * inv_tw), x = idx - rb * tw;
        const double* c0 = X + (__mul24(4 * rb + r1, tw) + x);
        double a0, a1, a2, a3;
        blur4(c0, tw, [&](int k) { return readlane_f64(w1, r1 - k); }, r1, a0, a1, a2, a3);
        double* o = Y + (__mul24(4 * rb, yp) + 2 * r2 + x);
        o[0] = a0;
        o[yp] = a1;
        o[2 * yp] = a2;
        o[3 * yp] = a3;
      }
    }
    wave_lds_sync();
    PH(1)
    const int ncb = (pw + 3) >> 2, nh = ncb * ph;
    const float inv_ph = 1.0f / (float)ph;
    if (nh <= 16 && r2 > 0) {
      const int idx = lane;
      if (idx < pw * ph) {
        const int x = (int)(((float)idx + 0.5f) * inv_ph), yq = idx - x * ph;
        double a[1];
        blur_n<1>(Y + (__mul24(yq, yp) + x + r2), 1, [&](int k) { return readlane_f64(w2, r2 - k); }, r2, a);
        tile[(int64_t)yq * cur.epitch + cur.epad + x] = a[0];
      }
    } else if (nh <= 32 && r2 > 0) {
      const int idx = lane, nc2 = (pw + 1) >> 1;
      if (idx < nc2 * ph) {
        const int cb = (int)(((float)idx + 0.5f) * inv_ph), yq = idx - cb * ph, xo = 2 * cb;
        double a[2];
        blur_n<2>(Y + (__mul24(yq, yp) + xo + r2), 1, [&](int k) { return readlane_f64(w2, r2 - k); }, r2, a);
        double* o = tile + (int64_t)yq * cur.epitch + cur.epad + xo;
        o[0] = a[0];
        if (xo + 1 < pw) o[1] = a[1];
      }
    } else {
      for (int idx = lane; idx < nh; idx += 64) {
        const int cb = (int)(((float)idx + 0.5f) * inv_ph), yq = idx - cb * ph;
        const double* c0 = Y + (__mul24(yq, yp) + 4 * cb + r2);
        double a0, a1, a2, a3;
        if (r2 > 0) {
          blur4(c0, 1, [&](int k) { return readlane_f64(w2, r2 - k); }, r2, a0, a1, a2, a3);
        } else {
          a0 = c0[0]; a1 = c0[1]; a2 = c0[2]; a3 = c0[3];
        }
        const int xo = 4 * cb;
        double* o = tile + (int64_t)yq * cur.epitch + cur.epad + xo;
        if (xo + 3 < pw) {
          o[0] = a0; o[1] = a1; o[2] = a2; o[3] = a3;
        } else {
          o[0] = a0;
          if (xo + 1 < pw) o[1] = a1;
          if (xo + 2 < pw) o[2] = a2;
        }
      }
    }
    wave_lds_sync();
    PH(2)
    if (!has_next) break;
    it += stride;
    cur = nxt;
    has_next = it + stride < n_items;
  }
  PH_FLUSH(2)
}

constexpr int BIG_GROUPS = 64;
constexpr int BIG_ROWS = 16;
constexpr int BIG_COL_LDS = 2048;

template <class F>
__device__ inline void visit_taps(int a0, int a1, int b0, int b1, int r, F f) {
  a0 = imax(a0, -r); a1 = imin(a1, -1);
  b0 = imax(b0, -r); b1 = imin(b1, -1);
  if (a0 > a1) { a0 = b0; a1 = b1; b0 = 0; b1 = -1; }
  if (b0 <= b1 && b0 < a0) { int t = a0; a0 = b0; b0 = t; t = a1; a1 = b1; b1 = t; }
  if (b0 <= b1 && b0 <= a1 + 1) { a1 = imax(a1, b1); b0 = 0; b1 = -1; }
  for (int ii = a0; ii <= a1; ii++) f(ii);
  for (int ii = b0; ii <= b1; ii++) f(ii);
}

constexpr int SLOW_CAP = 256;
__global__ __launch_bounds__(256) void k_blur_big_weights(const FrameDesc* frames, int max_drops, Scratch sc) {
  const int f = blockIdx.y;
  __shared__ double hw[MAX_R + 1];
  const int n_items = imin(sc.counts[f * 8 + 3], SLOW_CAP);
  for (int w = blockIdx.x; w < 2 * n_items; w += gridDim.x) {
    const int it = w >> 1, axis = w & 1;
    const DropPlan& p = sc.plan[(int64_t)f * max_drops + sc.list_slow[(int64_t)f * max_drops + it]];
    const int r = axis ? p.r2 : p.r1;
    __syncthreads();
    if (r > 0) {
      gauss_half_table(axis ? p.sig2 : p.sig1, r, hw);
      double* o = sc.wtab_big + (((int64_t)f * SLOW_CAP + it) * 2 + axis) * (MAX_R + 1);
      for (int k = threadIdx.x; k <= r; k += 256) o[k] = hw[k];
    }
  }
}

template <int AXIS>
__global__ __launch_bounds__(256) void k_blur(const FrameDesc* frames, int max_drops, Scratch sc) {
  const int f = blockIdx.y, t = threadIdx.x;
  __shared__ double hw[MAX_R + 1];
  __shared__ double s_in[BIG_COL_LDS];
  const int n_items = sc.counts[f * 8 + 3];
  int cur = -1;
  for (int w = blockIdx.x; w < n_items * BIG_GROUPS; w += gridDim.x) {
    const int it = w / BIG_GROUPS, g = w - it * BIG_GROUPS;
    const int64_t gi = (int64_t)f * max_drops + sc.list_slow[(int64_t)f * max_drops + it];
    const DropPlan& p = sc.plan[gi];
    const int r = AXIS == 0 ? p.r1 : p.r2;
    const int tw = p.tw, th = p.th, ew = p.ew, eh = p.eh, r1 = p.r1, r2 = p.r2;
    if (AXIS == 0 ? g >= tw : g * BIG_ROWS >= eh) continue;
    const double* raw = sc.arena + p.a0_off;
    double* fin = sc.arena + p.a1_off;
    double* tmp = fin + (((int64_t)p.epitch * eh + 15) & ~15LL);
    __syncthreads();
    if (cur != it) {
      if (r > 0) {
        if (it < SLOW_CAP) {
          const double* wt = sc.wtab_big + (((int64_t)f * SLOW_CAP + it) * 2 + AXIS) * (MAX_R + 1);
          for (int k = t; k <= r; k += 256) hw[k] = wt[k];
          __syncthreads();
        } else {
          gauss_half_table(AXIS == 0 ? p.sig1 : p.sig2, r, hw);
        }
      }
      cur = it;
    }
    if (AXIS == 0) {
      for (int rx = g; rx < tw; rx += BIG_GROUPS) {
        const bool lds = th <= BIG_COL_LDS;
        __syncthreads();
        if (lds)
          for (int k = t; k < th; k += 256) s_in[k] = raw[(int64_t)k * tw + rx];
        __syncthreads();
        auto R = [&](int yy) -> double {
          const int ry = yy - r1;
          return (ry >= 0 && ry < th) ? (lds ? s_in[ry] : raw[(int64_t)ry * tw + rx]) : 0.0;
        };
        for (int y = t; y < eh; y += 256) {
          double acc = R(y) * hw[r];
          visit_taps(r1 - y, r1 - y + th - 1, y - r1 - th + 1, y - r1, r, [&](int ii) { acc = acc + (R(y + ii) + R(y - ii)) * hw[ii + r]; });
          tmp[(int64_t)y * tw + rx] = acc;
        }
      }
    } else {
      for (int y0 = g * BIG_ROWS; y0 < eh; y0 += BIG_GROUPS * BIG_ROWS) {
        const int nr = imin(BIG_ROWS, eh - y0);
        const bool lds = nr * tw <= BIG_COL_LDS;
        __syncthreads();
        if (lds)
          for (int k = t; k < nr * tw; k += 256) s_in[k] = tmp[(int64_t)y0 * tw + k];
        __syncthreads();
        for (int idx = t; idx < nr * ew; idx += 256) {
          const int yy = idx / ew, x = idx - yy * ew;
          auto T = [&](int xx) -> double {
            const int rx = xx - r2;
            return (rx >= 0 && rx < tw) ? (lds ? s_in[yy * tw + rx] : tmp[(int64_t)(y0 + yy) * tw + rx]) : 0.0;
          };
          double acc;
          if (r2 > 0) {
            acc = T(x) * hw[r];
            visit_taps(r2 - x, r2 - x + tw - 1, x - r2 - tw + 1, x - r2, r, [&](int ii) { acc = acc + (T(x + ii) + T(x - ii)) * hw[ii + r]; });
          } else {
            acc = T(x);
          }
          fin[(int64_t)(y0 + yy) * p.epitch + p.epad + x] = acc;
        }
      }
    }
  }
}

__global__ __launch_bounds__(256) void k_bin(const FrameDesc* frames, Dims dm, int max_drops, int ctiles_x, int nct, Scratch sc) {
  const int f = blockIdx.y, ct = blockIdx.x;
  const int cty = ct / ctiles_x, ctx_ = ct - cty * ctiles_x;
  const int t = threadIdx.x, lane = t & 63, wave = t >> 6;
  const int n = frames[f].n_drops;
  const int x0 = ctx_ * CTILE, y0 = cty * CTILE, x1 = min(x0 + CTILE, dm.W), y1 = min(y0 + CTILE, dm.H);
  const int4* bbox = sc.bbox + (int64_t)f * max_drops;
  uint16_t* out = sc.clist + ((int64_t)f * nct + ct) * max_drops;
  __shared__ int s_cnt[4];
  int total = 0;
  for (int base = 0; base < n; base += 256) {
    const int i = base + t;
    bool hit = false;
    if (i < n) {
      const int4 bb = bbox[i];
      hit = bb.x < x1 && bb.z > x0 && bb.y < y1 && bb.w > y0;
    }
    const unsigned long long bal = __ballot(hit);
    if (lane == 0) s_cnt[wave] = __popcll(bal);
    __syncthreads();
    int off = total;
    for (int w = 0; w < 4; w++) {
      const int cw = s_cnt[w];
      if (w < wave) off += cw;
      total += cw;
    }
    if (hit) out[off + __popcll(bal & ((1ull << lane) - 1ull))] = (uint16_t)i;
    __syncthreads();
  }
  if (t == 0) sc.ccount[(int64_t)f * nct + ct] = total;
}

constexpr int BIN_SEG = 8192;
__global__ __launch_bounds__(256) void k_bin_rows(const FrameDesc* frames, Dims dm, int max_drops, int ctiles_x, int nct, Scratch sc) {
  const int f = blockIdx.y, cty = blockIdx.x;
  const int t = threadIdx.x, lane = t & 63, wave = t >> 6;
  const int n = frames[f].n_drops;
  const int y0 = cty * CTILE, y1 = min(y0 + CTILE, dm.H);
  const int4* bbox = sc.bbox + (int64_t)f * max_drops;
  __shared__ uint16_t s_idx[BIN_SEG], s_x0[BIN_SEG], s_x1[BIN_SEG];
  __shared__ int s_cnt[4];
  __shared__ int s_total[64];
  for (int k = t; k < ctiles_x; k += 256) s_total[k] = 0;
  for (int seg = 0; seg < n; seg += BIN_SEG) {
    const int seg_n = min(BIN_SEG, n - seg);
    int m = 0;
    for (int base = 0; base < seg_n; base += 256) {
      const int i = seg + base + t;
      bool hit = false;
      int4 bb = make_int4(0, 0, 0, 0);
      if (base + t < seg_n) {
        bb = bbox[i];
        hit = bb.x < bb.z && bb.y < y1 && bb.w > y0;
      }
      const unsigned long long bal = __ballot(hit);
      if (lane == 0) s_cnt[wave] = __popcll(bal);
      __syncthreads();
      int off = m;
      for (int w = 0; w < 4; w++) {
        const int cw = s_cnt[w];
        if (w < wave) off += cw;
        m += cw;
      }
      if (hit) {
        const int o = off + __popcll(bal & ((1ull << lane) - 1ull));
        s_idx[o] = (uint16_t)i;
        s_x0[o] = (uint16_t)imax(bb.x, 0);
        s_x1[o] = (uint16_t)imin(bb.z, 65535);
      }
      __syncthreads();
    }
    for (int ctx_ = wave; ctx_ < ctiles_x; ctx_ += 4) {
      const int x0 = ctx_ * CTILE, x1 = min(x0 + CTILE, dm.W);
      uint16_t* out = sc.clist + ((int64_t)f * nct + (cty * ctiles_x + ctx_)) * max_drops;
      int total = s_total[ctx_];
      for (int base = 0; base < m; base += 64) {
        const int k = base + lane;
        const bool hit = k < m && (int)s_x0[k] < x1 && (int)s_x1[k] > x0;
        const unsigned long long bal = __ballot(hit);
        if (hit) out[total + __popcll(bal & ((1ull << lane) - 1ull))] = s_idx[k];
        total += __popcll(bal);
      }
      if (lane == 0) s_total[ctx_] = total;
    }
    __syncthreads();
  }
  __syncthreads();
  for (int k = t; k < ctiles_x; k += 256) sc.ccount[(int64_t)f * nct + cty * ctiles_x + k] = s_total[k];
}

__global__ __launch_bounds__(256) void k_pad_visits(const FrameDesc* frames, Dims dm, int max_drops, Scratch sc) {
  const int f = blockIdx.y, i = blockIdx.x * 4 + (threadIdx.x >> 6), lane = threadIdx.x & 63;
  if (i >= frames[f].n_drops) return;
  const int64_t gi = (int64_t)f * max_drops + i;
  if (!sc.blended[gi]) return;
  const DropPlan& p = sc.plan[gi];
  const int4 e = sc.bbox[gi];
  const int w = p.vis_w, n = p.vis_w * p.vis_h;
  const int64_t base = (int64_t)f * dm.H * dm.W;
  for (int k = lane; k < n; k += 64) {
    const int y = p.vis_y0 + k / w, x = p.vis_x0 + k % w;
    if (x < 0 || y < 0 || x >= dm.W || y >= dm.H) continue;
    const bool in_tile = x >= e.x && x < e.z && y >= e.y && y < e.w;
    atomicMin((in_tile ? sc.eff_first : sc.pad_first) + base + (int64_t)y * dm.W + x, i);
  }
}
__device__ inline double clip_unit_np(double v) { return v < 0.0 ? 0.0 : (v > 1.0 ? 1.0 : v); }

__global__ __launch_bounds__(256) void k_composite(const FrameDesc* frames, Dims dm, rr_camera cam, int max_drops, int tiles_x,
                                                   int tiles_y, int ctiles_x, int nct, Scratch sc) {
  const int f = blockIdx.y;
  const int ntiles = tiles_x * tiles_y, per_xcd = (ntiles + 7) / 8;
  const int tile = (int)(blockIdx.x % 8) * per_xcd + (int)(blockIdx.x / 8);
  if (tile >= ntiles) return;
  const int tyi = tile / tiles_x, txi = tile - tyi * tiles_x;
  const int t = threadIdx.x, lane = t & 63, wave = t >> 6;
  const FrameDesc& fr = frames[f];
  const int tx0 = txi * TILE, ty0 = tyi * TILE, tx1 = min(tx0 + TILE, dm.W), ty1 = min(ty0 + TILE, dm.H);
  static_assert(TILE == 16, "k_composite: four 8x8 quarters");
  const int px = tx0 + 8 * (wave & 1) + (lane & 7), py = ty0 + 8 * (wave >> 1) + (lane >> 3);
  const bool live = px < dm.W && py < dm.H;
  const int64_t pix = (int64_t)py * dm.W + px;
  double c[3] = {0, 0, 0}, m = 0.0;
  double sum_b = 0.0;
  if (live) {
    load_px3(fr.rainy_bg, rainy_kind(fr), pix, c);
    if (fr.bg == fr.rainy_bg) {
      sum_b = (c[0] + c[1]) + c[2];
    } else {
      double b[3];
      load_px3(fr.bg, bg_kind(fr), pix, b);
      sum_b = (b[0] + b[1]) + b[2];
    }
  }
  if (sc.pad_first && live) {
    const int64_t q = (int64_t)f * dm.H * dm.W + pix;
    if (sc.pad_first[q] < sc.eff_first[q])
      for (int k = 0; k < 3; k++) c[k] = clip_unit_np(c[k]);
  }
  double scene = 1.0e300;
  if (fr.depth && live)
    scene = fr.depth_f64 ? as_global((const double*)fr.depth)[pix] : (double)as_global((const float*)fr.depth)[pix];
  const double ex = cam.exposure_s, ex_rcp = 1.0 / ex;
  const bool tame_px = !live || (fabs(c[0]) < 1.0e50 && fabs(c[1]) < 1.0e50 && fabs(c[2]) < 1.0e50);
  const bool slow_wave = __ballot(!tame_px) != 0ull || (__double_as_longlong(ex) & 0xFFFFFFFFFFFFFLL) == 0xFFFFFFFFFFFFFLL ||
                         !(ex > 1.0e-100 && ex < 1.0e100);
  const CompRec* comp = sc.comp + (int64_t)f * max_drops;
  const int4* bbox = sc.bbox + (int64_t)f * max_drops;
  const double* arena = sc.arena;
  const int ct = (ty0 / CTILE) * ctiles_x + (tx0 / CTILE);
  const uint16_t* clist = sc.clist + ((int64_t)f * nct + ct) * max_drops;
  const int n = sc.ccount[(int64_t)f * nct + ct];
  __shared__ int s_list[4][256];
  __shared__ int s_cnt[4][4];
  const int xm = tx0 + 8, ym = ty0 + 8;
  for (int base = 0; base < n; base += 256) {
    const int k = base + t;
    unsigned hitm = 0;
    int i = 0;
    if (k < n) {
      i = clist[k];
      const int4 bb = bbox[i];
      if (bb.x < tx1 && bb.z > tx0 && bb.y < ty1 && bb.w > ty0) {
        const unsigned xl = bb.x < xm, xr = bb.z > xm, yt = bb.y < ym, yb = bb.w > ym;
        hitm = (xl & yt) | ((xr & yt) << 1) | ((xl & yb) << 2) | ((xr & yb) << 3);
      }
    }
    unsigned long long bal[4];
#pragma unroll
    for (int q = 0; q < 4; q++) bal[q] = __ballot((hitm >> q) & 1u);
    if (lane < 4) s_cnt[wave][lane] = __popcll(lane == 0 ? bal[0] : (lane == 1 ? bal[1] : (lane == 2 ? bal[2] : bal[3])));
    __syncthreads();
    int total = 0;
#pragma unroll
    for (int q = 0; q < 4; q++) {
      int off = 0, tq = 0;
      for (int w = 0; w < 4; w++) {
        const int cw = s_cnt[w][q];
        if (w < wave) off += cw;
// ... 1369 lines not shown
  r.used[idx] = false;
  if (bytes > r.cap[idx]) {
    if (r.host[idx]) HIPCHK(hipHostFree(r.host[idx]));
    r.host[idx] = nullptr;
    r.cap[idx] = 0;
    const size_t want = bytes + bytes / 2 + 4096;
    HIPCHK(hipHostMalloc(&r.host[idx], want, hipHostMallocDefault));
    r.cap[idx] = want;
  }
  host = r.host[idx];
  return RR_OK;
}
int ring_commit(rr_ctx* ctx, rr_ctx::DescRing& r, int idx, hipStream_t s) {
  HIPCHK(hipEventRecord(r.ev[idx], s));
  r.used[idx] = true;
  return RR_OK;
}

struct ProfScope {
  rr_ctx* ctx;
  hipStream_t s;
  ProfEntry pe;
  bool on;
  ProfScope(rr_ctx* c, hipStream_t st, const char* name) : ctx(c), s(st), on(c->prof) {
    if (on) {
      pe.name = name;
      pe.a = get_event(c);
      pe.b = get_event(c);
      hipEventRecord(pe.a, s);
    }
  }
  ~ProfScope() {
    if (on) {
      hipEventRecord(pe.b, s);
      ctx->prof_pending.push_back(pe);
    }
  }
};

void prof_collect(rr_ctx* ctx) {
  for (auto& pe : ctx->prof_pending) {
    float ms = 0.f;
    hipEventSynchronize(pe.b);
    hipEventElapsedTime(&ms, pe.a, pe.b);
    bool found = false;
    for (auto& s : ctx->prof_stats)
      if (!strcmp(s.name, pe.name)) {
        s.launches++;
        s.total_ms += ms;
        found = true;
        break;
      }
    if (!found) {
      rr_kernel_stat s;
      memset(&s, 0, sizeof(s));
      strncpy(s.name, pe.name, sizeof(s.name) - 1);
      s.launches = 1;
      s.total_ms = ms;
      ctx->prof_stats.push_back(s);
    }
    ctx->ev_pool.push_back(pe.a);
    ctx->ev_pool.push_back(pe.b);
  }
  ctx->prof_pending.clear();
}

bool fov_fast_path(const rr_ctx* ctx, const Dims& dm) {
  return !ctx->general_fov && dm.He <= HE_MAX && dm.We <= FOV_WE_MAX && (int64_t)dm.We * dm.He < (1 << 22) && ctx->cam.n_fov * 1 <= 64 &&
         ctx->cam.n_fov >= 3;
}

int ensure_scratch(rr_ctx* ctx, int n, int max_drops, const Dims& dm, bool need_comp_out) {
  const bool grow_frames = n > ctx->cap_frames;
  const bool grow_drops = max_drops > ctx->cap_drops;
  const bool dims_change = dm.H != ctx->cap_dims.H || dm.W != ctx->cap_dims.W || dm.He != ctx->cap_dims.He || dm.We != ctx->cap_dims.We;
  const bool general = !fov_fast_path(ctx, dm);
  if (grow_frames || grow_drops || dims_change || (need_comp_out && !ctx->d_comp_out) || general != ctx->scratch_general || ctx->cam.n_fov > ctx->erec_nfov) {
    HIPCHK(hipDeviceSynchronize());
    const int F = grow_frames ? n : ctx->cap_frames;
    const int D = grow_drops ? max_drops : ctx->cap_drops;
    const size_t fd = (size_t)F * (size_t)(D > 0 ? D : 1);
    const int Hp = (dm.He + 3) & ~3;
    int rc;
    if ((rc = dev_alloc(ctx, ctx->sc.plan, fd))) return rc;
    if ((rc = dev_alloc(ctx, ctx->sc.comp, fd))) return rc;
    if ((rc = dev_alloc(ctx, ctx->sc.comp32, fd))) return rc;
    if ((rc = dev_alloc(ctx, ctx->sc.npts, fd))) return rc;
    if ((rc = dev_alloc(ctx, ctx->sc.sizes, fd))) return rc;
    if ((rc = dev_alloc(ctx, ctx->sc.list_rot, fd))) return rc;
    if ((rc = dev_alloc(ctx, ctx->sc.rows_list, fd))) return rc;
    if ((rc = dev_alloc(ctx, ctx->sc.rows_sorted, fd))) return rc;
    if ((rc = dev_alloc(ctx, ctx->sc.rows_n, (size_t)F * 3))) return rc;
    if ((rc = dev_alloc(ctx, ctx->sc.rows_hist, (size_t)RW_TEX_MAX * 3 + 16))) return rc;
    ctx->sc.rows_cost = reinterpret_cast<unsigned long long*>(ctx->sc.rows_hist + RW_TEX_MAX);
    ctx->sc.rows_next = ctx->sc.rows_hist + 3 * RW_TEX_MAX;
    ctx->sc.rot_total = ctx->sc.rows_next + 1;
    if ((rc = dev_alloc(ctx, ctx->sc.rows_bounds, (size_t)RW_SHARE_MAX + 1))) return rc;
    if ((rc = dev_alloc(ctx, ctx->sc.rows_fbase, (size_t)F * RW_TEX_MAX))) return rc;
    if ((rc = dev_alloc(ctx, ctx->sc.fov_list, fd))) return rc;
    if ((rc = dev_alloc(ctx, ctx->sc.fov_erec, general ? 1 : fd * (size_t)(ctx->cam.n_fov > 0 ? ctx->cam.n_fov : RR_MAX_FOV)))) return rc;
    if ((rc = dev_alloc(ctx, ctx->sc.fov_pix, general ? 1 : fd * (size_t)(ctx->cam.n_fov > 0 ? ctx->cam.n_fov : RR_MAX_FOV)))) return rc;
    ctx->erec_nfov = ctx->cam.n_fov;
    if ((rc = dev_alloc(ctx, ctx->sc.fov_list_n, (size_t)F))) return rc;
    if ((rc = dev_alloc(ctx, ctx->sc.list_gen, fd))) return rc;
    if ((rc = dev_alloc(ctx, ctx->sc.list_slow, fd))) return rc;
    if ((rc = dev_alloc(ctx, ctx->sc.blur_items, fd * 8))) return rc;
    if ((rc = dev_alloc(ctx, ctx->sc.list_small, fd))) return rc;
    if ((rc = dev_alloc(ctx, ctx->sc.colpart, fd * COL_PARTS * 5))) return rc;
    if ((rc = dev_alloc(ctx, ctx->sc.wtab, fd * 2 * (BR_MAX + 1)))) return rc;
    if ((rc = dev_alloc(ctx, ctx->sc.wtab_big, (size_t)F * SLOW_CAP * 2 * (MAX_R + 1)))) return rc;
    if (general) {
      if ((rc = dev_alloc(ctx, ctx->sc.poly, fd * 2 * POLY_STRIDE))) return rc;
      if ((rc = dev_alloc(ctx, ctx->sc.prefix, (size_t)F * dm.He * (size_t)(dm.We + 1) * 4))) return rc;
      if ((rc = dev_alloc(ctx, ctx->sc.spans, 1))) return rc;
    } else {
      if ((rc = dev_alloc(ctx, ctx->sc.poly, 1))) return rc;
      if ((rc = dev_alloc(ctx, ctx->sc.prefix, 1))) return rc;
      const size_t per_frame = (size_t)(((D > 0 ? D : 1) + 1 + 7) & ~7) * (size_t)Hp;
      if ((rc = dev_alloc(ctx, ctx->sc.spans, (size_t)F * per_frame))) return rc;
      HIPCHK(hipMemset(ctx->sc.spans, 0, sizeof(uint32_t) * (size_t)F * per_frame));
    }
    ctx->scratch_general = general;
    ctx->scratch_hp = Hp;
    if ((rc = dev_alloc(ctx, ctx->sc.bbox, fd))) return rc;
    if ((rc = dev_alloc(ctx, ctx->sc.blended, fd))) return rc;
    {
      const size_t nct = (size_t)((dm.W + CTILE - 1) / CTILE) * ((dm.H + CTILE - 1) / CTILE);
      if ((rc = dev_alloc(ctx, ctx->sc.clist, fd * nct))) return rc;
      if ((rc = dev_alloc(ctx, ctx->sc.ccount, (size_t)F * nct))) return rc;
    }
    if ((rc = dev_alloc(ctx, ctx->sc.counts, (size_t)F * 8))) return rc;
    if ((rc = dev_alloc(ctx, ctx->sc.canon, fd))) return rc;
    if ((rc = dev_alloc(ctx, ctx->sc.bigs_list, fd))) return rc;
    if ((rc = dev_alloc(ctx, ctx->sc.bigs_n, (size_t)F))) return rc;
    if ((rc = dev_alloc(ctx, ctx->sc.tkey, fd * 2))) return rc;
    if ((rc = dev_alloc(ctx, ctx->sc.lrec, fd))) return rc;
    if ((rc = dev_alloc(ctx, ctx->sc.list_big, fd))) return rc;
    if ((rc = dev_alloc(ctx, ctx->sc.big_off, fd + F))) return rc;
    if ((rc = dev_alloc(ctx, ctx->sc.htab, fd * 2))) return rc;
    if ((rc = dev_alloc(ctx, ctx->sc.fband, (size_t)F * COL_PARTS * 2))) return rc;
    const int ntiles = ((dm.W + TILE - 1) / TILE) * ((dm.H + TILE - 1) / TILE);
    if ((rc = dev_alloc(ctx, ctx->sc.partial, (size_t)F * ntiles * 4))) return rc;
    if ((rc = dev_alloc(ctx, ctx->sc.means, (size_t)F * 4))) return rc;
    if ((rc = dev_alloc(ctx, ctx->sc.arena_need, (size_t)F))) return rc;
    if ((rc = dev_alloc(ctx, ctx->d_frames, (size_t)F))) return rc;
    if ((rc = dev_alloc(ctx, ctx->d_comp_out, (size_t)F * dm.H * dm.W * 3))) return rc;
    if (ctx->arena_cap == 0) ctx->arena_cap = (int64_t)(D > 0 ? D : 1) * 1024 + (1 << 20);
    if ((rc = dev_alloc(ctx, ctx->sc.arena, (size_t)F * (size_t)ctx->arena_cap))) return rc;
    ctx->cap_frames = F;
    ctx->cap_drops = D;
    ctx->cap_dims = dm;
  }
  return RR_OK;
}

int grow_arena(rr_ctx* ctx) {
  HIPCHK(hipDeviceSynchronize());
  unsigned long long need = 0;
  HIPCHK(hipMemcpy(&need, ctx->sc.need_max, sizeof(need), hipMemcpyDeviceToHost));
  if ((int64_t)need > ctx->arena_cap) {
    const int64_t cap = ((int64_t)need + (int64_t)need / 4 + (1 << 16) + 15) & ~15LL;
    ctx->arena_cap = cap;
    int rc = dev_alloc(ctx, ctx->sc.arena, (size_t)ctx->cap_frames * (size_t)cap);
    if (rc) return rc;
  }
  HIPCHK(hipMemset(ctx->sc.need_max, 0, sizeof(unsigned long long)));
  return RR_OK;
// ... 157 lines not shown
      const int v32 = fov32 ? 1 : 0;
      const dim3 grid((max_drops + 4 * G - 1) / (4 * G), n);
      if (dda) {
        HIPCHK(hipMemsetAsync(sc.fov_list_n, 0, sizeof(int32_t) * (size_t)n, fs));
        {
          hipLaunchKernelGGL(k_fov_dda, dim3((max_drops + 64 * DDA_WAVES - 1) / (64 * DDA_WAVES), n), dim3(64 * DDA_WAVES), 0, fs, ctx->d_frames, dm, ctx->cam, D, Hp, Dp,
                             cv_rule ? 1 : 0, sc);
        }
        const dim3 lgrid(imin((int)grid.x, 8), n);
        if (dm.He <= 384)
          hipLaunchKernelGGL((k_fov_spans<6, true>), lgrid, dim3(256), 0, fs, ctx->d_frames, dm, ctx->cam, D, Hp, Dp, 0, cv_rule ? 1 : 0, sc);
        else if (dm.He <= 512)
          hipLaunchKernelGGL((k_fov_spans<8, true>), lgrid, dim3(256), 0, fs, ctx->d_frames, dm, ctx->cam, D, Hp, Dp, 0, cv_rule ? 1 : 0, sc);
        else
          hipLaunchKernelGGL((k_fov_spans<16, true>), lgrid, dim3(256), 0, fs, ctx->d_frames, dm, ctx->cam, D, Hp, Dp, 0, cv_rule ? 1 : 0, sc);
      } else if (dm.He <= 384)
        hipLaunchKernelGGL((k_fov_spans<6, false>), grid, dim3(256), 0, fs, ctx->d_frames, dm, ctx->cam, D, Hp, Dp, v32, cv_rule ? 1 : 0, sc);
      else if (dm.He <= 512)
        hipLaunchKernelGGL((k_fov_spans<8, false>), grid, dim3(256), 0, fs, ctx->d_frames, dm, ctx->cam, D, Hp, Dp, v32, cv_rule ? 1 : 0, sc);
      else
        hipLaunchKernelGGL((k_fov_spans<16, false>), grid, dim3(256), 0, fs, ctx->d_frames, dm, ctx->cam, D, Hp, Dp, v32, cv_rule ? 1 : 0, sc);
    } else {
      ProfScope ps(ctx, fs, "k_fov_poly");
      hipLaunchKernelGGL(k_fov_poly_general, dim3((max_drops + 127) / 128, n), dim3(128), 0, fs, ctx->d_frames, dm, ctx->cam, D, sc);
    }
    sc.colpart_f32 = (fast && fov32) ? 1 : 0;
    if (fast) {
      ProfScope ps(ctx, fs, "k_fov_sums");
      const size_t row_bytes = ((size_t)(dm.We + 1) * 2 + 16 * 2) * sizeof(double);
      auto passes = [&](int nt) { return ((((dm.We + nt / 64 - 1) / (nt / 64)) + 1) / 2 * 2 + 127) / 128; };
      const int NT = 1024;
      const bool e1 = passes(NT) <= 1;
      const int DPT = ctx->fov_dpt ? ctx->fov_dpt : (max_drops <= NT ? 1 : (max_drops <= 2 * NT ? 2 : (max_drops <= 4 * NT ? 4 : 8)));
      const int rpb = ((dm.He + COL_PARTS - 1) / COL_PARTS + 3) & ~3;
      const int nchunk = (max_drops + NT * DPT - 1) / (NT * DPT);
      const dim3 grid(COL_PARTS * 2 * nchunk, n);
      auto launch = [&](auto kern) -> hipError_t {
        hipError_t e = hipFuncSetAttribute(reinterpret_cast<const void*>(kern), hipFuncAttributeMaxDynamicSharedMemorySize, (int)row_bytes);
        if (e != hipSuccess) return e;
        hipLaunchKernelGGL(kern, grid, dim3(NT), row_bytes, fs, ctx->d_frames, dm, D, Hp, Dp, rpb, nchunk, sc);
        return hipSuccess;
      };
      auto launch32 = [&](auto kern) -> hipError_t {
        const size_t bytes = ((size_t)(dm.We + 1) * 4 + 16 * 4) * sizeof(float);
        hipError_t e = hipFuncSetAttribute(reinterpret_cast<const void*>(kern), hipFuncAttributeMaxDynamicSharedMemorySize, (int)bytes);
        if (e != hipSuccess) return e;
        hipLaunchKernelGGL(kern, dim3(COL_PARTS * nchunk, n), dim3(NT), bytes, fs, ctx->d_frames, dm, D, Hp, Dp, rpb, nchunk, sc);
        return hipSuccess;
      };
      bool all32 = true;
      for (int f = 0; f < n; f++) all32 = all32 && (in[f].in_types & RR_IN_ENV_F32);
      for (int f = 0; f < n && !all32; f++)
        if (in[f].in_types & RR_IN_ENV_F32) {
          ctx->err = "RR_IN_ENV_F32 must be set for every frame of a batch or for none";
          return RR_E_ARG;
        }
      hipError_t e = fov32
                         ? (all32 ? (e1 ? (DPT == 1 ? launch32(k_fov_sums32<1, 1, true>) : DPT == 2 ? launch32(k_fov_sums32<2, 1, true>) : DPT == 4 ? launch32(k_fov_sums32<4, 1, true>) : launch32(k_fov_sums32<8, 1, true>))
                                        : (DPT == 1 ? launch32(k_fov_sums32<1, 2, true>) : DPT == 2 ? launch32(k_fov_sums32<2, 2, true>) : DPT == 4 ? launch32(k_fov_sums32<4, 2, true>) : launch32(k_fov_sums32<8, 2, true>)))
                                  : (e1 ? (DPT == 1 ? launch32(k_fov_sums32<1, 1, false>) : DPT == 2 ? launch32(k_fov_sums32<2, 1, false>) : DPT == 4 ? launch32(k_fov_sums32<4, 1, false>) : launch32(k_fov_sums32<8, 1, false>))
                                        : (DPT == 1 ? launch32(k_fov_sums32<1, 2, false>) : DPT == 2 ? launch32(k_fov_sums32<2, 2, false>) : DPT == 4 ? launch32(k_fov_sums32<4, 2, false>) : launch32(k_fov_sums32<8, 2, false>))))
                     : e1 ? (DPT == 1 ? launch(k_fov_sums<1, 1>) : DPT == 2 ? launch(k_fov_sums<2, 1>) : DPT == 4 ? launch(k_fov_sums<4, 1>) : launch(k_fov_sums<8, 1>))
                        : (DPT == 1 ? launch(k_fov_sums<1, 2>) : DPT == 2 ? launch(k_fov_sums<2, 2>) : DPT == 4 ? launch(k_fov_sums<4, 2>) : launch(k_fov_sums<8, 2>));
      if (e != hipSuccess) {
        ctx->err = std::string("k_fov_sums: ") + hipGetErrorString(e);
        return RR_E_HIP;
      }
    } else {
      {
        ProfScope ps(ctx, fs, "k_env_prefix");
        hipLaunchKernelGGL(k_env_prefix, dim3((dm.He + 3) / 4, n), dim3(256), 0, fs, ctx->d_frames, dm, sc.prefix);
        hipLaunchKernelGGL(k_env_consts, dim3(n), dim3(256), 0, fs, dm, sc.prefix, sc.fband);
      }
      {
        ProfScope ps(ctx, fs, "k_fov_sums_general");
        hipLaunchKernelGGL(k_fov_sums_general, dim3((max_drops + 3) / 4, n), dim3(256), 0, fs, ctx->d_frames, dm, D, sc, ctx->fill_rule, ctx->cam.n_fov);
      }
    }
    {
      ProfScope ps(ctx, bs, "k_plan");
      HIPCHK(hipMemsetAsync(sc.bigs_n, 0, sizeof(int32_t) * (size_t)n, bs));
      hipLaunchKernelGGL(k_plan, dim3((max_drops + 127) / 128, n), dim3(128), 0, bs, ctx->d_frames, dm, ctx->cam, ctx->d_tex_h,
                         ctx->d_tex_w, D, fs == bs ? 1 : 0, sc);
      hipLaunchKernelGGL(k_plan_big, dim3((max_drops + 127) / 128, n), dim3(128), 0, bs, ctx->d_frames, ctx->d_tex_h, ctx->d_tex_w, D, sc);
    }
    {
      ProfScope ps(ctx, bs, "k_scan");
      hipLaunchKernelGGL(k_scan, dim3(n), dim3(1024), 0, bs, ctx->d_frames, D, ctx->arena_cap, sc);
    }
    {
      ProfScope ps(ctx, bs, "k_dedup");
      HIPCHK(hipMemsetAsync(sc.htab, 0, sizeof(int32_t) * 2 * (size_t)n * D, bs));
      HIPCHK(hipMemsetAsync(sc.counts, 0, sizeof(int32_t) * 8 * (size_t)n, bs));
      HIPCHK(hipMemsetAsync(sc.rows_hist, 0, sizeof(int32_t) * (RW_TEX_MAX * 3 + 16), bs));
      hipLaunchKernelGGL(k_dedup, dim3((max_drops + 255) / 256, n), dim3(256), 0, bs, ctx->d_frames, D, n, ctx->dedup ? 1 : 0, sc);
    }
    {
      ProfScope ps(ctx, bs, "k_lists");
      hipLaunchKernelGGL(k_lists, dim3(n), dim3(1024), 0, bs, ctx->d_frames, D, ctx->d_tex_h, ctx->d_tex_w, sc);
      if (sc.rows_on) {
        hipLaunchKernelGGL(k_rows_scatter, dim3(n), dim3(1024), 0, bs, D, sc);
        hipLaunchKernelGGL(k_rows_shares, dim3(1), dim3(1024), 0, bs, rows_wgs * ctx->rows_shares, sc);
      }
    }
    {
      ProfScope ps(ctx, s, "k_tile_generic");
      hipLaunchKernelGGL(k_tile_generic, dim3(imin((max_drops + 3) / 4, imax(2, imin(64, 2048 / n))), n), dim3(256), 0, s, ctx->d_frames, D, ctx->d_tex,
                         ctx->d_tex_h, ctx->d_tex_w, ctx->d_tex_off, ctx->d_ctab, sc);
    }
    {
      ProfScope ps(ctx, s, "k_tile_big");
      hipLaunchKernelGGL(k_tile_big, dim3(sc.big_on ? imax(16, imin(1024, 16384 / n)) : 1024, n), dim3(256), 0, s, ctx->d_frames, D, ctx->d_tex, ctx->d_tex_h, ctx->d_tex_w,
                         ctx->d_tex_off, ctx->d_ctab, sc);
    }
    if (sc.rows_on) {
      ProfScope ps(ctx, s, "k_tile_rows");
      hipLaunchKernelGGL(k_tile_rows, dim3(rows_wgs), dim3(64 * RW_WAVES), 0, s, rows_wgs * ctx->rows_shares, ctx->d_tex_h, ctx->d_tex_w, ctx->d_ctab, sc);
    }
    {
      ProfScope ps(ctx, s, "k_tile");
      const int64_t cap = sc.rows_on ? 2048 : 16384;
      hipLaunchKernelGGL(k_tile, dim3((unsigned)std::max<int64_t>(1, std::min<int64_t>((int64_t)n * max_drops, cap))), dim3(256), 0, s, ctx->d_frames, D, ctx->d_tex,
                         ctx->d_tex_h, ctx->d_tex_w, ctx->d_tex_off, sc);
    }
    {
      ProfScope ps(ctx, s, "k_blur_weights");
      hipLaunchKernelGGL(k_blur_weights, dim3((2 * max_drops + 256 / BW_LANES - 1) / (256 / BW_LANES), n), dim3(256), 0, s, ctx->d_frames, D, sc);
    }
    {
      ProfScope ps(ctx, s, "k_blur_small");
      hipLaunchKernelGGL(k_blur_small, dim3(imin((max_drops + 3) / 4, grid_cap(2048)), n), dim3(256), 0, s, ctx->d_frames, D, sc);
    }
    {
      ProfScope ps(ctx, s, "k_blur_fused");
      const size_t lds = sizeof(double) * (size_t)(4 * (BR_MAX + 1) + sc.blur_bx + sc.blur_by);
      const dim3 grid(imin((max_drops + 1) / 2, grid_cap(4096)), n);
      hipLaunchKernelGGL(k_blur_fused_dma, grid, dim3(256), lds, s, ctx->d_frames, D, sc);
    }
    {
      ProfScope ps(ctx, s, "k_blur_big_weights");
      hipLaunchKernelGGL(k_blur_big_weights, dim3(64, n), dim3(256), 0, s, ctx->d_frames, D, sc);
    }
    {
      ProfScope ps(ctx, s, "k_blur_rows");
      hipLaunchKernelGGL(k_blur<0>, dim3(256, n), dim3(256), 0, s, ctx->d_frames, D, sc);
    }
    {
      ProfScope ps(ctx, s, "k_blur_cols");
      hipLaunchKernelGGL(k_blur<1>, dim3(256, n), dim3(256), 0, s, ctx->d_frames, D, sc);
    }
    HIPCHK(join.now());
    {
      ProfScope ps(ctx, s, "k_colour");
      hipLaunchKernelGGL(k_colour, dim3((max_drops + 255) / 256, n), dim3(256), 0, s, ctx->d_frames, dm, D, ctx->cam.exposure_s, sc);
    }
  }
  const int ctiles_x = (dm.W + CTILE - 1) / CTILE, nct = ctiles_x * ((dm.H + CTILE - 1) / CTILE);
  {
    ProfScope ps(ctx, s, "k_bin");
    if (ctiles_x <= 64)
      hipLaunchKernelGGL(k_bin_rows, dim3(nct / ctiles_x, n), dim3(256), 0, s, ctx->d_frames, dm, D, ctiles_x, nct, sc);
    else
      hipLaunchKernelGGL(k_bin, dim3(nct, n), dim3(256), 0, s, ctx->d_frames, dm, D, ctiles_x, nct, sc);
  }
  sc.pad_first = sc.eff_first = nullptr;
  bool wild = ctx->wild_pixels;
  for (int f = 0; f < n; f++) wild = wild && !in[f].ext;
// ... 460 lines not shown
    {
      ProfScope ps(ctx, s, "k_particles");
      hipLaunchKernelGGL(k_particles, dim3(n), dim3(512), 0, s, ctx->d_sims, H, W, ctx->d_dgrid, ctx->d_cdf, ctx->n_grid, ctx->d_ratio_db,
                         drops_out, cap, n_out, n_noisy > 0 ? 1 : 0);
    }
    {
      ProfScope ps(ctx, s, "k_particle_draws");
      hipLaunchKernelGGL(k_particle_draws, dim3(n), dim3(64), 0, s, ctx->d_sims, drops_out, cap, n_out, n_noisy > 0 ? 1 : 0);
    }
  }
  HIPCHK(hipGetLastError());
  if (n_noisy > 0) return enqueue_noise(ctx, n, sims, H, W, drops_out, cap, n_out, s);
  return RR_OK;
}

int check_overflow(rr_ctx* ctx, hipStream_t s) {
  int32_t ovf = 0;
  HIPCHK(hipMemcpyAsync(&ovf, ctx->sc.overflow, sizeof(int32_t), hipMemcpyDeviceToHost, s));
  HIPCHK(hipStreamSynchronize(s));
  if (!ovf) return RR_OK;
  int rc = grow_arena(ctx);
  if (rc) return rc;
  HIPCHK(hipMemset(ctx->sc.overflow, 0, sizeof(int32_t)));
  ctx->err = "tile arena overflow: arena regrown, re-enqueue the batch";
  return RR_E_ARENA;
}

}

extern "C" {

int rr_version(void) { return RR_VERSION; }
int rr_sizeof_drop(void) { return (int)sizeof(rr_drop); }
int rr_sizeof_camera(void) { return (int)sizeof(rr_camera); }
int rr_sizeof_frame_in(void) { return (int)sizeof(rr_frame_in); }
int rr_sizeof_frame_out(void) { return (int)sizeof(rr_frame_out); }
int rr_sizeof_prepass_in(void) { return (int)sizeof(rr_prepass_in); }
int rr_sizeof_prepass_out(void) { return (int)sizeof(rr_prepass_out); }
int rr_sizeof_prepass_kernels(void) { return (int)sizeof(rr_prepass_kernels); }

int rr_create(rr_ctx** out, int device) {
  if (!out) return RR_E_ARG;
  *out = nullptr;
  int count = 0;
  if (hipGetDeviceCount(&count) != hipSuccess || count <= 0 || device < 0 || device >= count) return RR_E_NO_DEVICE;
  hipDeviceProp_t prop;
  if (hipGetDeviceProperties(&prop, device) != hipSuccess) return RR_E_NO_DEVICE;
  if (strncmp(prop.gcnArchName, "gfx9", 4) != 0) return RR_E_NO_DEVICE;
  if (prop.warpSize != 64) return RR_E_NO_DEVICE;
  rr_ctx* ctx = new rr_ctx();
  ctx->device = device;
  ctx->n_cu = prop.multiProcessorCount > 0 ? prop.multiProcessorCount : 256;
  if (hipSetDevice(device) != hipSuccess || hipStreamCreateWithFlags(&ctx->stream, hipStreamNonBlocking) != hipSuccess) {
    delete ctx;
    return RR_E_HIP;
  }
  float tab[128];
  build_cubic_tab(tab);
  if (hipMalloc((void**)&ctx->d_ctab, sizeof(tab)) != hipSuccess ||
      hipMemcpy(ctx->d_ctab, tab, sizeof(tab), hipMemcpyHostToDevice) != hipSuccess ||
      hipMalloc((void**)&ctx->sc.overflow, sizeof(int32_t) * (2 + RR_PIPE_SLOTS)) != hipSuccess ||
      hipMemset(ctx->sc.overflow, 0, sizeof(int32_t) * (2 + RR_PIPE_SLOTS)) != hipSuccess ||
      hipMalloc((void**)&ctx->sc.need_max, sizeof(unsigned long long)) != hipSuccess ||
      hipMemset(ctx->sc.need_max, 0, sizeof(unsigned long long)) != hipSuccess || hipDeviceSynchronize() != hipSuccess) {
    rr_destroy(ctx);
    return RR_E_HIP;
  }
  *out = ctx;
  return RR_OK;
}

int rr_destroy(rr_ctx* ctx) {
  if (!ctx) return RR_E_ARG;
  hipSetDevice(ctx->device);
  hipDeviceSynchronize();
  if (ctx->own_tex) hipFree(ctx->d_tex);
  hipFree(ctx->d_tex_h);
  hipFree(ctx->d_tex_w);
  hipFree(ctx->d_tex_off);
  hipFree(ctx->d_tex_pad);
  hipFree(ctx->d_tex_poff);
  hipFree(ctx->d_ctab);
  hipFree(ctx->d_lut);
  hipFree(ctx->sc.plan);
  hipFree(ctx->sc.comp);
  hipFree(ctx->sc.comp32);
  hipFree(ctx->sc.poly);
  hipFree(ctx->sc.npts);
  hipFree(ctx->sc.sizes);
  hipFree(ctx->sc.list_rot);
  hipFree(ctx->sc.fov_erec);
  hipFree(ctx->sc.fov_pix);
  hipFree(ctx->sc.rows_list);
  hipFree(ctx->sc.rows_sorted);
  hipFree(ctx->sc.rows_n);
  hipFree(ctx->sc.rows_hist);
  hipFree(ctx->sc.rows_fbase);
  hipFree(ctx->sc.rows_bounds);
  hipFree(ctx->d_tex_pair);
  hipFree(ctx->d_tex_qoff);
  hipFree(ctx->sc.fov_list);
  hipFree(ctx->sc.fov_list_n);
  hipFree(ctx->sc.list_gen);
  hipFree(ctx->sc.list_slow);
  hipFree(ctx->sc.blur_items);
  hipFree(ctx->sc.counts);
  hipFree(ctx->sc.canon);
  hipFree(ctx->sc.bigs_list);
  hipFree(ctx->sc.bigs_n);
  hipFree(ctx->sc.tkey);
  hipFree(ctx->sc.lrec);
  hipFree(ctx->sc.list_big);
  hipFree(ctx->sc.big_off);
  hipFree(ctx->sc.htab);
  hipFree(ctx->sc.list_small);
  hipFree(ctx->sc.colpart);
  hipFree(ctx->sc.wtab);
  hipFree(ctx->sc.wtab_big);
  hipFree(ctx->sc.spans);
  hipFree(ctx->sc.bbox);
  hipFree(ctx->sc.blended);
  hipFree(ctx->d_pad_first);
  hipFree(ctx->d_pngz_slots);
  hipFree(ctx->d_pngz_meta);
  hipFree(ctx->d_eff_first);
  hipFree(ctx->sc.clist);
  hipFree(ctx->sc.ccount);
  hipFree(ctx->sc.prefix);
  hipFree(ctx->sc.fband);
  hipFree(ctx->sc.arena);
  hipFree(ctx->sc.partial);
  hipFree(ctx->sc.means);
  hipFree(ctx->sc.arena_need);
  hipFree(ctx->sc.overflow);
  hipFree(ctx->sc.need_max);
  hipFree(ctx->d_omega);
  hipFree(ctx->d_omega32);
  hipFree(ctx->d_aug);
  hipFree(ctx->d_dgrid);
  hipFree(ctx->d_cdf);
  hipFree(ctx->d_ratio_db);
  hipFree(ctx->d_sims);
  hipFree(ctx->d_gen_drops);
  hipFree(ctx->d_gen_counts);
  hipFree(ctx->d_field_cnt);
  for (void* b : ctx->noise_blocks) hipFree(b);
  hipFree(ctx->d_noise_desc);
  if (ctx->ev_noise) hipEventDestroy(ctx->ev_noise);
  for (auto* r : {&ctx->ring_frames, &ctx->ring_pre, &ctx->ring_sims, &ctx->ring_noise})
    for (int k = 0; k < rr_ctx::DescRing::N; k++) {
      if (r->host[k]) hipHostFree(r->host[k]);
      if (r->ev[k]) hipEventDestroy(r->ev[k]);
    }
  hipFree(ctx->d_frames);
  hipFree(ctx->d_comp_out);
  for (auto& sl : ctx->slots) {
    hipFree(sl.st.bg);
    hipFree(sl.st.rainy);
    hipFree(sl.st.env);
    hipFree(sl.st.omega);
    hipFree(sl.st.comp);
    hipFree(sl.st.mask);
    hipFree(sl.st.drops);
    hipFree(sl.st.rgb);
    hipFree(sl.st.mask_i);
    hipFree(sl.st.status);
    hipFree(sl.st.colour);
// ... 1478 lines not shown
```

rain-rendering_amd/csrc/rr_device.h:

```cpp
#pragma once
#include <math.h>
#include <stdint.h>

#include "rainhip.h"

#if defined(__HIPCC__)
#include <hip/hip_runtime.h>
#define RR_HD __host__ __device__ inline
#else
#define RR_HD inline
#endif

#if defined(__clang__)
#pragma clang fp contract(off)
#endif

namespace rr {

enum { KIND_BIG = 0, KIND_ROT = 1, KIND_EXT = 2 };
enum { RS_AREA = 0, RS_AREA_FAST = 1, RS_LINEAR = 2 };

struct Dims {
  int32_t H, W, He, We;
};

struct DropPlan {
  int32_t status;
  int32_t kind;
  int32_t tex;
  int32_t flip;
  int32_t tw, th;
  int32_t shift;
  int32_t pw, ph;
  int32_t r1, r2;
  int32_t vis_x0, vis_y0, vis_w, vis_h;
  int32_t crop_x, crop_y;
  int32_t ew;
  int32_t bw0;
  int32_t nW, nH;
  int32_t rs_mode;
  int32_t isx, isy;
  int32_t eh;
  int32_t epitch, epad;
  int64_t a0_off, a1_off;
  double sig1, sig2;
  double tau_one, g;
  double mi[9];
  double ma[6];
  double scale_x, scale_y, inv_sx, inv_sy;
};

struct CompRec {
  int32_t x0, y0, x1, y1;
  int32_t ox, oy;
  int32_t pitch, pad;
  int64_t off;
  double tau_one, g;
  double K[3];
  double zdist;
};

struct CompRec32 {
  uint32_t xx;
  uint32_t yy;
  int64_t base;
  uint32_t pitch_slow;
  float te, kg[3];
  int32_t spare0;
  double zdist;
  int32_t spare[4];
};
static_assert(sizeof(CompRec32) == 64, "CompRec32 is read as 16-byte words");

RR_HD int64_t cv_round(double v) {
  if (!(v == v)) return -2147483648LL;
  if (v < -2147483648.0) return -2147483648LL;
  if (v > 2147483647.0) return 2147483647LL;
  return (int64_t)rint(v);
}
RR_HD int64_t sat_short(int64_t v) { return v < -32768 ? -32768 : (v > 32767 ? 32767 : v); }
RR_HD int32_t imin(int32_t a, int32_t b) { return b < a ? b : a; }
RR_HD int32_t imax(int32_t a, int32_t b) { return b > a ? b : a; }
RR_HD double dmin(double a, double b) { return b < a ? b : a; }
RR_HD double dmax(double a, double b) { return b > a ? b : a; }
RR_HD double clip01(double x) { return x < 0.0 ? 0.0 : (x > 1.0 ? 1.0 : x); }
RR_HD int32_t iabs(int32_t a) { return a < 0 ? -a : a; }

RR_HD double det_exp(double x) {
  const double LN2_HI = 6.93147180369123816490e-01;
  const double LN2_LO = 1.90821492927058770002e-10;
  const double INV_LN2 = 1.44269504088896338700e+00;
  double k = rint(x * INV_LN2);
  double r = (x - k * LN2_HI) - k * LN2_LO;
  double p = 1.0 / 6227020800.0;
  p = p * r + 1.0 / 479001600.0;
  p = p * r + 1.0 / 39916800.0;
  p = p * r + 1.0 / 3628800.0;
  p = p * r + 1.0 / 362880.0;
  p = p * r + 1.0 / 40320.0;
  p = p * r + 1.0 / 5040.0;
  p = p * r + 1.0 / 720.0;
  p = p * r + 1.0 / 120.0;
  p = p * r + 1.0 / 24.0;
  p = p * r + 1.0 / 6.0;
  p = p * r + 1.0 / 2.0;
  p = p * r + 1.0;
  p = p * r + 1.0;
  return ldexp(p, (int)k);
}

RR_HD double det_log(double x) {
  int e;
  double m = frexp(x, &e);
  if (m < 0.70710678118654752440) {
    m = m * 2.0;
    e = e - 1;
  }
  const double k = (double)e;
  const double f = m - 1.0;
  const double hfsq = 0.5 * f * f;
  const double s = f / (2.0 + f);
  const double z = s * s;
  const double w = z * z;
  const double t1 = w * (3.999999999940941908e-01 + w * (2.222219843214978396e-01 + w * 1.531383769920937332e-01));
  const double t2 = z * (6.666666666666735130e-01 + w * (2.857142874366239149e-01 + w * (1.818357216161805012e-01 + w * 1.479819860511658591e-01)));
  const double r = t2 + t1;
  return k * 6.93147180369123816490e-01 - ((hfsq - (s * (hfsq + r) + k * 1.90821492927058770002e-10)) - f);
}

RR_HD void det_sincos(double x, double& sn, double& cn) {
  const double k = rint(x * 6.36619772367581382433e-01);
  const double r = ((x - k * 1.57079632673412561417e+00) - k * 6.07710050630396597660e-11) - k * 2.02226624879595063154e-21;
  const double z = r * r;
// ... 905 lines not shown
RR_HD void solve8(double A[8][8], double b[8], double x[8]) {
#pragma unroll
  for (int col = 0; col < 8; col++) {
    int piv = col;
    double best = fabs(A[col][col]);
#pragma unroll
    for (int r = col + 1; r < 8; r++)
      if (fabs(A[r][col]) > best) { best = fabs(A[r][col]); piv = r; }
#pragma unroll
    for (int r = col + 1; r < 8; r++)
      if (r == piv) {
#pragma unroll
        for (int c = 0; c < 8; c++) { double t = A[col][c]; A[col][c] = A[r][c]; A[r][c] = t; }
        double t = b[col]; b[col] = b[r]; b[r] = t;
      }
#pragma unroll
    for (int r = col + 1; r < 8; r++) {
      double f = A[r][col] / A[col][col];
#pragma unroll
      for (int c = col + 1; c < 8; c++) A[r][c] = A[r][c] - f * A[col][c];
      b[r] = b[r] - f * b[col];
    }
  }
#pragma unroll
  for (int r = 7; r >= 0; r--) {
    double s = b[r];
#pragma unroll
    for (int c = r + 1; c < 8; c++) s = s - A[r][c] * x[c];
    x[r] = s / A[r][r];
  }
}

RR_HD void invert3(const double m[9], double t[9]) {
  double d = m[0] * (m[4] * m[8] - m[5] * m[7]) - m[1] * (m[3] * m[8] - m[5] * m[6]) + m[2] * (m[3] * m[7] - m[4] * m[6]);
  if (d == 0.0 || !(fabs(d) < 1.7e308)) {
    for (int i = 0; i < 9; i++) t[i] = 0.0;
    return;
  }
  d = 1.0 / d;
  t[0] = (m[4] * m[8] - m[5] * m[7]) * d;
  t[1] = (m[2] * m[7] - m[1] * m[8]) * d;
  t[2] = (m[1] * m[5] - m[2] * m[4]) * d;
  t[3] = (m[5] * m[6] - m[3] * m[8]) * d;
  t[4] = (m[0] * m[8] - m[2] * m[6]) * d;
  t[5] = (m[2] * m[3] - m[0] * m[5]) * d;
  t[6] = (m[3] * m[7] - m[4] * m[6]) * d;
  t[7] = (m[1] * m[6] - m[0] * m[7]) * d;
  t[8] = (m[0] * m[4] - m[1] * m[3]) * d;
}

RR_HD int py_slice_index(int i, int n) {
  if (i < 0) { i += n; if (i < 0) i = 0; }
  else if (i > n) i = n;
  return i;
}

RR_HD void raw_tile_key(const rr_drop& d, const DropPlan& p, uint32_t key[8]) {
  for (int k = 0; k < 8; k++) key[k] = 0u;
  key[0] = 0xffffffffu;
  if (p.status != RR_DROP_OK || (p.kind != KIND_BIG && p.kind != KIND_ROT)) return;
  if (p.tw < 0 || p.tw > 65535 || p.th < 0 || p.th > 65535) return;
  if (p.kind == KIND_BIG) {
    const double d0 = floor(d.iw1), d1 = floor(d.iw2);
    if (!(d0 > -2.0e9 && d0 < 2.0e9 && d1 > -2.0e9 && d1 < 2.0e9)) return;
    const int minx = imax(imin(d.x0, d.x1), 0), miny = imax(imin(d.y0, d.y1), 0);
    key[2] = (uint32_t)(d.x0 - minx);
    key[3] = (uint32_t)(d.y0 - miny);
    key[4] = (uint32_t)(d.x1 - minx);
    key[5] = (uint32_t)(d.y1 - miny);
    key[6] = (uint32_t)(int32_t)d0;
    key[7] = (uint32_t)(int32_t)d1;
  } else {
    uint64_t a, b;
    const double al = d.rot_cos, be = d.rot_sin;
    __builtin_memcpy(&a, &al, 8);
    __builtin_memcpy(&b, &be, 8);
    key[2] = (uint32_t)a; key[3] = (uint32_t)(a >> 32);
    key[4] = (uint32_t)b; key[5] = (uint32_t)(b >> 32);
  }
  key[0] = (uint32_t)p.kind | ((uint32_t)(p.flip & 1) << 4) | ((uint32_t)p.tex << 8);
  key[1] = (uint32_t)p.tw | ((uint32_t)p.th << 16);
}

RR_HD void plan_big_homography(const rr_drop& d, int sw, int sh, double mi[9]) {
  const double d0 = floor(d.iw1), d1 = floor(d.iw2);
  const int minx = imax(imin(d.x0, d.x1), 0), miny = imax(imin(d.y0, d.y1), 0);
  float src[4][2] = {{0.f, 0.f}, {(float)sw, 0.f}, {(float)sw, (float)sh}, {0.f, (float)sh}};
  float dst[4][2];
  dst[0][0] = (float)(d.x0 - minx);                        dst[0][1] = (float)(d.y0 - miny);
  dst[1][0] = (float)((double)(d.x0 - minx) + d0);         dst[1][1] = (float)(d.y0 - miny);
  dst[2][0] = (float)(((double)(d.x1 - minx) + d1) + 0.001); dst[2][1] = (float)(d.y1 - miny);
  dst[3][0] = (float)((double)(d.x1 - minx) + 0.001);      dst[3][1] = (float)(d.y1 - miny);
  double A[8][8], bb[8], xx[8];
#pragma unroll
  for (int i = 0; i < 8; i++)
#pragma unroll
    for (int j = 0; j < 8; j++) A[i][j] = 0.0;
#pragma unroll
  for (int i = 0; i < 4; i++) {
    double sx = src[i][0], sy = src[i][1], ddx = dst[i][0], ddy = dst[i][1];
    A[i][0] = A[i + 4][3] = sx;
    A[i][1] = A[i + 4][4] = sy;
    A[i][2] = A[i + 4][5] = 1.0;
    A[i][6] = -sx * ddx;
    A[i][7] = -sy * ddx;
    A[i + 4][6] = -sx * ddy;
    A[i + 4][7] = -sy * ddy;
    bb[i] = ddx;
    bb[i + 4] = ddy;
  }
  solve8(A, bb, xx);
  double M[9] = {xx[0], xx[1], xx[2], xx[3], xx[4], xx[5], xx[6], xx[7], 1.0};
  invert3(M, mi);
}

struct ExtGeom {
  bool has;
  int tw, th, min_x, min_y;
};
template <bool DEFER_BIG = false>
RR_HD void plan_drop(const rr_drop& d, const rr_camera& cam, const Dims& dm, const int32_t* tex_h, const int32_t* tex_w,
                     double opacity_attenuation, int strategy, DropPlan& p, int64_t& size_out, const ExtGeom xg);
template <bool DEFER_BIG = false>
RR_HD void plan_drop(const rr_drop& d, const rr_camera& cam, const Dims& dm, const int32_t* tex_h, const int32_t* tex_w,
                     double opacity_attenuation, int strategy, DropPlan& p, int64_t& size_out, const rr_ext_tile* ext = nullptr) {
  const bool has = ext && ext->alpha;
  plan_drop<DEFER_BIG>(d, cam, dm, tex_h, tex_w, opacity_attenuation, strategy, p, size_out,
                       ExtGeom{has, has ? ext->tw : 0, has ? ext->th : 0, has ? ext->min_x : 0, has ? ext->min_y : 0});
}
template <bool DEFER_BIG>
RR_HD void plan_drop(const rr_drop& d, const rr_camera& cam, const Dims& dm, const int32_t* tex_h, const int32_t* tex_w,
                     double opacity_attenuation, int strategy, DropPlan& p, int64_t& size_out, const ExtGeom xg) {
  size_out = 0;
  p.status = RR_DROP_OK;
  p.tex = d.tex_index;
  p.flip = 0;
  p.bw0 = 1;
  p.nW = p.nH = 0;
  p.rs_mode = RS_AREA;
  p.isx = p.isy = 1;
  p.eh = 0;
  p.epitch = p.epad = 0;
  p.a0_off = p.a1_off = 0;
  p.ew = 0;
  p.scale_x = p.scale_y = p.inv_sx = p.inv_sy = 1.0;
  for (int i = 0; i < 9; i++) p.mi[i] = 0.0;
  for (int i = 0; i < 6; i++) p.ma[i] = 0.0;
  p.vis_x0 = p.vis_y0 = p.vis_w = p.vis_h = p.crop_x = p.crop_y = 0;
  p.tw = p.th = p.pw = p.ph = p.shift = p.r1 = p.r2 = 0;
  p.sig1 = p.sig2 = 0.0;
  const int W = dm.W, H = dm.H;
  const int sh = tex_h[d.tex_index], sw = tex_w[d.tex_index];

  int minCx, minCy;
  if (xg.has) {
    p.kind = KIND_EXT;
    p.tw = imax(xg.tw, 1);
    p.th = imax(xg.th, 1);
    minCx = xg.min_x;
    minCy = xg.min_y;
  } else if (d.type == 0) {
    p.kind = KIND_BIG;
    double d0 = floor(d.iw1), d1 = floor(d.iw2);
    int minx = imax(imin(d.x0, d.x1), 0), miny = imax(imin(d.y0, d.y1), 0);
    double maxx = dmin(dmax((double)d.x0 + d0, (double)d.x1 + d1), (double)W);
    int maxy = imin(imax(d.y0, d.y1), H);
    int s0 = (int)(maxx - (double)minx), s1 = maxy - miny;
    p.tw = imax(s0, 1);
    p.th = imax(s1, 1);
    if (!DEFER_BIG) plan_big_homography(d, sw, sh, p.mi);
    int bh0 = imin(16, p.th);
    int bw0 = imin(1024 / bh0, p.tw);
    p.bw0 = bw0;
    minCx = minx;
    minCy = miny;
  } else {
    p.kind = KIND_ROT;
    p.flip = (d.x1 > W / 2) ? 1 : 0;
    p.th = imax(iabs(d.y1 - d.y0), 2);
    p.tw = imax(iabs(d.x1 - d.x0), d.max_width + 2);
    double cX = (double)sw / 2.0, cY = (double)sh / 2.0;
    double cxf = (double)(float)cX, cyf = (double)(float)cY;
    double al = d.rot_cos, be = d.rot_sin;
    double M[6] = {al, be, (1 - al) * cxf - be * cyf, -be, al, be * cxf + (1 - al) * cyf};
    double cs = fabs(M[0]), sn = fabs(M[1]);
    int nW = (int)((double)sh * sn + (double)sw * cs);
    int nH = (int)((double)sh * cs + (double)sw * sn);
    M[2] += ((double)nW / 2.0) - cX;
    M[5] += ((double)nH / 2.0) - cY;
    p.nW = nW;
    p.nH = nH;
    double D = M[0] * M[4] - M[1] * M[3];
    D = (D != 0.0) ? 1.0 / D : 0.0;
    double A11 = M[4] * D, A22 = M[0] * D;
    M[0] = A11;
    M[1] = M[1] * (-D);
    M[3] = M[3] * (-D);
    M[4] = A22;
    double b1 = -M[0] * M[2] - M[1] * M[5];
    double b2 = -M[3] * M[2] - M[4] * M[5];
    M[2] = b1;
    M[5] = b2;
    for (int i = 0; i < 6; i++) p.ma[i] = M[i];
    if (nW <= 0 || nH <= 0) {
      p.status = RR_DROP_FOV_FAIL;
      return;
    }
    p.inv_sx = (double)p.tw / (double)nW;
    p.inv_sy = (double)p.th / (double)nH;
    p.scale_x = 1.0 / p.inv_sx;
    p.scale_y = 1.0 / p.inv_sy;
    int isx = (int)cv_round(p.scale_x), isy = (int)cv_round(p.scale_y);
    const double EPS = 2.220446049250313e-16;
    bool fast = fabs(p.scale_x - (double)isx) < EPS && fabs(p.scale_y - (double)isy) < EPS;
    if (p.scale_x >= 1.0 && p.scale_y >= 1.0) {
      if (fast) { p.rs_mode = RS_AREA_FAST; p.isx = isx; p.isy = isy; }
      else p.rs_mode = RS_AREA;
    } else {
      p.rs_mode = RS_LINEAR;
    }
    minCx = d.x0;
    minCy = d.y0;
  }

  if (strategy == 1) {
    p.pw = p.tw;
    p.ph = p.th;
    const int sx = py_slice_index(minCx, W), ex = py_slice_index(minCx + p.tw, W);
    const int sy = py_slice_index(minCy, H), ey = py_slice_index(minCy + p.th, H);
    p.vis_x0 = sx;
    p.vis_y0 = sy;
    p.vis_w = imax(ex - sx, 0);
    p.vis_h = imax(ey - sy, 0);
    p.tau_one = cam.exposure_s * 1.0;
    p.g = p.tau_one / cam.tau_zero;
    p.ew = p.tw;
    p.eh = p.th;
    size_out = (p.vis_w > 0 && p.vis_h > 0) ? (((int64_t)p.tw * p.th + 15) & ~15LL) : 0;
    return;
  }
  double o = fabs(d.wps[2]);
  double cc = ((o - cam.focus_plane) * cam.focal_sq) / (o * (cam.focus_plane - cam.focal_m) * cam.f_number);
  cc = fabs(cc / cam.sensor_px);
  if (!(cc < 1.7e308)) { p.status = RR_DROP_BAD_COC; return; }
  if (10.0 * cc >= (double)(RR_MAX_SHIFT + 1)) { p.status = RR_DROP_TOO_BIG; return; }
  p.shift = (int)(10.0 * cc);
  p.sig1 = cc;
  p.sig2 = cc / 2.0;
  p.r1 = (p.sig1 > 1e-15) ? (int)(4.0 * p.sig1 + 0.5) : 0;
  p.r2 = (p.sig2 > 1e-15) ? (int)(4.0 * p.sig2 + 0.5) : 0;
  p.pw = p.tw + 2 * p.shift;
  p.ph = p.th + 2 * p.shift;

  int tmpx = minCx - p.shift, tmpy = minCy - p.shift;
  int mcx = imin(imax(tmpx, 0), W), mcy = imin(imax(tmpy, 0), H);
  int dx = mcx - tmpx, dy = mcy - tmpy;
  int cw, ch;
  if (dx < 0) { cw = imax(p.pw + dx, 0); p.crop_x = 0; } else { cw = imax(p.pw - dx, 0); p.crop_x = dx; }
  if (dy < 0) { ch = imax(p.ph + dy, 0); p.crop_y = 0; } else { ch = imax(p.ph - dy, 0); p.crop_y = dy; }
  p.vis_x0 = mcx;
  p.vis_y0 = mcy;
  p.vis_w = imax(imin(mcx + cw, W) - mcx, 0);
  p.vis_h = imax(imin(mcy + ch, H) - mcy, 0);

  double d_avg = (d.iw1 + d.iw2) / 2.0;
  double length_opacity = opacity_attenuation * d_avg / ((double)d.length + d_avg);
  p.tau_one = cam.exposure_s * length_opacity;
  p.g = p.tau_one / cam.tau_zero;

  p.ew = p.tw + 2 * p.r2;
  p.eh = p.th + 2 * p.r1;
  p.epad = 0;
  p.epitch = p.ew;
  size_out = (p.vis_w > 0 && p.vis_h > 0) ? (((int64_t)p.tw * p.th + 15) & ~15LL) + (p.r1 > 0 ? (((int64_t)p.epitch * p.eh + 15) & ~15LL) : 0) : 0;
}

RR_HD double blur_axis0(const double* src, int pw, int ph, int x, int y, const double* hw, int r) {
  double acc = src[(int64_t)y * pw + x] * hw[r];
  for (int ii = -r; ii < 0; ii++) {
    int ya = y + ii, yb = y - ii;
    double va = (ya >= 0) ? src[(int64_t)ya * pw + x] : 0.0;
    double vb = (yb < ph) ? src[(int64_t)yb * pw + x] : 0.0;
    acc = acc + (va + vb) * hw[ii + r];
  }
  return acc;
}
RR_HD double blur_axis1(const double* src, int pw, int ph, int x, int y, const double* hw, int r) {
  (void)ph;
  const double* row = src + (int64_t)y * pw;
  double acc = row[x] * hw[r];
  for (int ii = -r; ii < 0; ii++) {
    int xa = x + ii, xb = x - ii;
    double va = (xa >= 0) ? row[xa] : 0.0;
    double vb = (xb < pw) ? row[xb] : 0.0;
    acc = acc + (va + vb) * hw[ii + r];
  }
  return acc;
}

RR_HD void blend_pixel(double A, double tau_one, double exposure, double g, const double K[3], double bgr[3], double& mask) {
  double t = (A * tau_one) / exposure;
  double u = 1.0 - t;
  for (int c = 0; c < 3; c++) {
    double v = u * bgr[c] + (A * K[c]) * g;
    bgr[c] = clip01(v);
  }
  mask = mask + A;
}

constexpr int BLUR_BX = 2816;
constexpr int BLUR_BY = 2048;
constexpr int BR_MAX = 48;

struct BlurLayout {
  int fused;
  int wo, ho;
  int single;
};
RR_HD int blur_x_doubles(int wo, int ho, int r1, int r2, int tw) { return imin(wo + 2 * r2, tw) * (((ho + 3) & ~3) + 2 * r1); }
RR_HD int blur_y_pitch(int wo, int r2) { return (((wo + 3) & ~3) + 2 * r2) | 1; }
RR_HD int blur_y_doubles(int wo, int ho, int r2) { return blur_y_pitch(wo, r2) * ((ho + 3) & ~3); }

RR_HD BlurLayout blur_layout(const DropPlan& p, int BX_MAX, int BY_MAX) {
  BlurLayout b{0, 0, 0, 0};
  if (p.r1 <= 0 || p.r1 > BR_MAX) return b;
  if (blur_x_doubles(p.ew, p.eh, p.r1, p.r2, p.tw) <= BX_MAX && blur_y_doubles(p.ew, p.eh, p.r2) <= BY_MAX) {
    b.fused = 1; b.wo = p.ew; b.ho = p.eh; b.single = 1;
    return b;
  }
  {
    const int hy = (BY_MAX / blur_y_pitch(p.ew, p.r2)) & ~3;
    const int hx = ((BX_MAX / imin(p.ew + 2 * p.r2, p.tw)) - 2 * p.r1) & ~3;
    const int hb = imin(hy, hx);
    if (hb >= imax(8, p.r1)) {
      b.fused = 1; b.wo = p.ew; b.ho = imin(hb, p.eh);
      return b;
    }
  }
  const double rr2 = (double)imax(p.r2, 1), rr1 = (double)p.r1;
  int wi = (int)sqrt((double)BX_MAX * rr2 / rr1);
  wi = imax(imin(wi, p.ew + 2 * p.r2), 2 * p.r2 + 4);
  int hi = BX_MAX / wi;
  hi = imin(hi, ((p.eh + 3) & ~3) + 2 * p.r1);
  wi = imin(BX_MAX / hi, p.ew + 2 * p.r2);
  int wo = wi - 2 * p.r2, ho = (hi - 2 * p.r1) & ~3;
  if (ho > p.eh) ho = p.eh;
  for (int it = 0; it < 64 && wo >= 1 && ho >= 1; it++) {
    if (blur_x_doubles(wo, ho, p.r1, p.r2, p.tw) <= BX_MAX && blur_y_doubles(wo, ho, p.r2) <= BY_MAX) {
      b.fused = 1; b.wo = wo; b.ho = ho; b.single = (wo >= p.ew && ho >= p.eh) ? 1 : 0;
      return b;
    }
    if (blur_x_doubles(wo, ho, p.r1, p.r2, p.tw) > BX_MAX) { if (wo > 4) wo -= 1; else ho -= 4; }
    else ho -= 4;
  }
  return b;
}
constexpr int BS_X = 512;
constexpr int BS_Y = 768;

// ... 8 lines not shown
```

Measured before the change: 18470.

## Split monolithic DropPlan into compact per-stage tile, blur and placement records

Replaces the single large DropPlan array with three smaller 16-byte-aligned records (TileRec, BlurRec, PlaceRec), each holding only the fields one consumer stage needs, with pack/unpack helpers. Downstream kernels read the smaller record with vector or uniform loads instead of copying the whole plan. k_plan_big also now solves the 8x8 homography cooperatively across 8 lanes with shuffles. This is meant to cut memory traffic and register pressure from the oversized plan struct, at the cost of more packing code and bit-packed fields that assume limits on radius and shift.

```diff
diff --git a/__graft_entry__.py b/__graft_entry__.py
--- a/__graft_entry__.py
+++ b/__graft_entry__.py
@@ -58,6 +58,11 @@
     if force or _newer(rig_lib, [rig_src] + hip_dep[3:]):
         subprocess.check_call(['g++', '-O2', '-std=c++17', '-ffp-contract=off', '-fPIC', '-shared',
                                '-I' + os.path.join(ROOT, 'include'), '-I' + CSRC, rig_src, '-o', rig_lib])
+    rec_src = os.path.join(ROOT, 'tests', 'hostemu', 'records_emu.cpp')
+    rec_lib = os.path.join(ROOT, 'tests', 'hostemu', 'librecordsemu.so')
+    if force or _newer(rec_lib, [rec_src] + hip_dep[3:]):
+        subprocess.check_call(['g++', '-O2', '-std=c++17', '-ffp-contract=off', '-fPIC', '-shared',
+                               '-I' + os.path.join(ROOT, 'include'), '-I' + CSRC, rec_src, '-o', rec_lib])
     importlib.import_module('rain-rendering_amd')
     hb = importlib.import_module('rain-rendering_amd.hip_backend')
     hb.load_library()
diff --git a/rain-rendering_amd/csrc/rainhip.hip b/rain-rendering_amd/csrc/rainhip.hip
--- a/rain-rendering_amd/csrc/rainhip.hip
+++ b/rain-rendering_amd/csrc/rainhip.hip
@@ -165,7 +165,9 @@
 #endif
 
 struct Scratch {
-  DropPlan* plan;
+  TileRec* trec;
+  BlurRec* brec;
+  PlaceRec* prec;
   CompRec* comp;
   CompRec32* comp32;
   int32_t* poly;
@@ -298,18 +300,53 @@
   return p.r1 > 0 && !blur_is_small(p) && !blur_layout(p, sc.blur_bx, sc.blur_by).fused;
 }
 
-constexpr int PLAN_DW = (int)(sizeof(DropPlan) / 4);
+template <class R>
+__device__ inline R load_rec(const R* g) {
+  static_assert(sizeof(R) % 16 == 0, "records are read as 16-byte words");
+  constexpr int NW = (int)(sizeof(R) / 16);
+  uint4 w[NW];
+  const uint4* s = reinterpret_cast<const uint4*>(g);
+#pragma unroll
+  for (int k = 0; k < NW; k++) w[k] = s[k];
+  R r;
+  __builtin_memcpy(&r, w, sizeof(R));
+  return r;
+}
+template <class R>
+__device__ inline R load_rec_uniform(const R* g) {
+  constexpr int ND = (int)(sizeof(R) / 4);
+  const const_ptr<uint32_t> src = as_constant(reinterpret_cast<const uint32_t*>(g));
+  uint32_t w[ND];
+#pragma unroll
+  for (int k = 0; k < ND; k++) w[k] = src[k];
+  R r;
+  __builtin_memcpy(&r, w, sizeof(R));
+  return r;
+}
+template <class R>
+__device__ inline void store_recs(const R& rec, int lane, int nrec, uint4* stage, R* out) {
+  constexpr int NW = (int)(sizeof(R) / 16);
+  if (lane < nrec) {
+    uint4 w[NW];
+    __builtin_memcpy(w, &rec, sizeof(R));
+#pragma unroll
+    for (int k = 0; k < NW; k++) stage[lane * NW + k] = w[k];
+  }
+  wave_lds_sync();
+  uint4* o = reinterpret_cast<uint4*>(out);
+  for (int k = lane; k < nrec * NW; k += 64) o[k] = stage[k];
+  wave_lds_sync();
+}
 enum { LC_NONE = 0, LC_BIG_LDS = 1, LC_BIG = 2, LC_ROWS = 3, LC_ROT_INT = 4, LC_ROT = 5, LC_GEN = 6 };
 enum { LB_NONE = 0, LB_SMALL = 1, LB_FUSED = 2, LB_SLOW = 3 };
 __device__ inline uint4 make_list_rec(const DropPlan& p, const int32_t* tex_h, const int32_t* tex_w, const Scratch& sc);
 __global__ __launch_bounds__(128) void k_plan(const FrameDesc* frames, Dims dm, rr_camera cam, const int32_t* tex_h,
                                               const int32_t* tex_w, int max_drops, int use_npts, Scratch sc) {
-  static_assert(sizeof(DropPlan) % 4 == 0, "DropPlan layout");
   const int f = blockIdx.y;
   const int i = blockIdx.x * blockDim.x + threadIdx.x;
   const int lane = threadIdx.x & 63, wave = threadIdx.x >> 6;
   const FrameDesc& fr = frames[f];
-  __shared__ uint32_t s_plan[2][32 * PLAN_DW];
+  __shared__ uint4 s_stage[2][64 * (sizeof(TileRec) / 16)];
   const bool act = i < fr.n_drops;
   const int64_t gi = (int64_t)f * max_drops + (act ? i : 0);
   DropPlan p;
@@ -344,33 +381,79 @@
     }
   }
   const int wave_i0 = blockIdx.x * blockDim.x + wave * 64;
-  uint32_t* stage = s_plan[wave];
-  uint32_t* out = reinterpret_cast<uint32_t*>(sc.plan + (int64_t)f * max_drops + wave_i0);
-#pragma unroll
-  for (int half = 0; half < 2; half++) {
-    if (act && (lane >> 5) == half) {
-      const uint32_t* src = reinterpret_cast<const uint32_t*>(&p);
-#pragma unroll
-      for (int k = 0; k < PLAN_DW; k++) stage[(lane & 31) * PLAN_DW + k] = src[k];
-    }
-    wave_lds_sync();
-    const int first = wave_i0 + half * 32;
-    const int nrec = imax(imin(32, fr.n_drops - first), 0);
-    for (int k = lane; k < nrec * PLAN_DW; k += 64) out[half * 32 * PLAN_DW + k] = stage[k];
-    wave_lds_sync();
-  }
-}
-
-__global__ __launch_bounds__(128) void k_plan_big(const FrameDesc* frames, const int32_t* tex_h, const int32_t* tex_w, int max_drops, Scratch sc) {
-  const int f = blockIdx.y, j = blockIdx.x * blockDim.x + threadIdx.x;
-  if (j >= sc.bigs_n[f]) return;
-  const int i = sc.bigs_list[(int64_t)f * max_drops + j];
-  const rr_drop d = load_drop(frames[f].drops + i);
-  double mi[9];
-  plan_big_homography(d, tex_w[d.tex_index], tex_h[d.tex_index], mi);
-  double* o = sc.plan[(int64_t)f * max_drops + i].mi;
-#pragma unroll
-  for (int k = 0; k < 9; k++) o[k] = mi[k];
+  const int nrec = imax(imin(64, fr.n_drops - wave_i0), 0);
+  const int64_t w0 = (int64_t)f * max_drops + wave_i0;
+  TileRec tr;
+  BlurRec br;
+  PlaceRec pr;
+  if (act) {
+    tile_rec_pack(p, tr);
+    blur_rec_pack(p, br);
+    place_rec_pack(p, pr);
+  }
+  store_recs(tr, lane, nrec, s_stage[wave], sc.trec + w0);
+  store_recs(br, lane, nrec, s_stage[wave], sc.brec + w0);
+  store_recs(pr, lane, nrec, s_stage[wave], sc.prec + w0);
+}
+
+constexpr int PB_DROPS = 32;
+__global__ __launch_bounds__(256) void k_plan_big(const FrameDesc* frames, const int32_t* tex_h, const int32_t* tex_w, int max_drops, Scratch sc) {
+  const int f = blockIdx.y, r = threadIdx.x & 7, g0 = (threadIdx.x & 63) & ~7;
+  const int n = sc.bigs_n[f];
+  for (int j = blockIdx.x * PB_DROPS + (threadIdx.x >> 3); j < n; j += gridDim.x * PB_DROPS) {
+    const int i = sc.bigs_list[(int64_t)f * max_drops + j];
+    const rr_drop d = load_drop(frames[f].drops + i);
+    double A[8], b;
+    big_system_row(d, tex_w[d.tex_index], tex_h[d.tex_index], r, A, b);
+    auto from = [&](double v, int row) { return __shfl(v, g0 + row); };
+#pragma unroll
+    for (int col = 0; col < 8; col++) {
+      int piv = col;
+      const double mine = fabs(A[col]);
+      double best = from(mine, col);
+#pragma unroll
+      for (int q = col + 1; q < 8; q++) {
+        const double v = from(mine, q);
+        if (v > best) { best = v; piv = q; }
+      }
+      if (piv != col) {
+        const int src = r == col ? piv : (r == piv ? col : r);
+#pragma unroll
+        for (int c = 0; c < 8; c++) A[c] = from(A[c], src);
+        b = from(b, src);
+      }
+      const double pc = from(A[col], col), pb = from(b, col);
+      double prow[8];
+#pragma unroll
+      for (int c = col + 1; c < 8; c++) prow[c] = from(A[c], col);
+      if (r > col) {
+        const double fq = A[col] / pc;
+#pragma unroll
+        for (int c = col + 1; c < 8; c++) A[c] = A[c] - fq * prow[c];
+        b = b - fq * pb;
+      }
+    }
+    double x[8];
+#pragma unroll
+    for (int q = 7; q >= 0; q--) {
+      double s = b;
+#pragma unroll
+      for (int c = q + 1; c < 8; c++) s = s - A[c] * x[c];
+      x[q] = from(s / A[q], q);
+    }
+    const double M[9] = {x[0], x[1], x[2], x[3], x[4], x[5], x[6], x[7], 1.0};
+    double mi[9];
+    invert3(M, mi);
+    if (r == 0) {
+      TileRec& t = sc.trec[(int64_t)f * max_drops + i];
+      double2* o = reinterpret_cast<double2*>(t.m);
+#pragma unroll
+      for (int k = 0; k < 4; k++) o[k] = make_double2(mi[2 * k], mi[2 * k + 1]);
+      uint64_t bits;
+      __builtin_memcpy(&bits, &mi[8], 8);
+      *reinterpret_cast<uint2*>(t.u) = make_uint2((uint32_t)bits, (uint32_t)(bits >> 32));
+    }
+  }
 }
 
 __global__ __launch_bounds__(1024) void k_scan(const FrameDesc* frames, int max_drops, int64_t arena_cap, Scratch sc) {
@@ -394,13 +477,15 @@
   const int64_t frame_base = (int64_t)f * arena_cap;
   if (t < 16 && arena_cap >= 16) sc.arena[frame_base + t] = 0.0;
   for (int i = i0; i < i1; i++) {
-    DropPlan& p = sc.plan[base + i];
     int64_t sz = sc.sizes[base + i];
     if (run + sz > arena_cap) {
       sc.sizes[base + i] = 0;
     } else {
-      p.a0_off = frame_base + run;
-      p.a1_off = frame_base + run + (((int64_t)p.tw * p.th + 15) & ~15LL);
+      longlong2* bo = reinterpret_cast<longlong2*>(&sc.brec[base + i]);
+      const int4 wh = reinterpret_cast<const int4*>(&sc.brec[base + i])[1];
+      const int64_t a0 = frame_base + run;
+      *bo = make_longlong2(a0, a0 + (((int64_t)wh.x * wh.y + 15) & ~15LL));
+      sc.trec[base + i].a0_off = a0;
     }
     run += sz;
   }
@@ -441,7 +526,7 @@
       }
       h = h + 1 == cap ? 0 : h + 1;
     }
-    if (canon != gi) sc.plan[gi].a0_off = sc.plan[canon].a0_off;
+    if (canon != gi) sc.brec[gi].a0_off = sc.brec[canon].a0_off;
   }
   sc.canon[gi] = canon;
   const unsigned long long dup = __ballot(canon != gi);
@@ -1264,7 +1349,9 @@
   const FrameDesc& fr = frames[f];
   if (i >= fr.n_drops) return;
   const int64_t gi = (int64_t)f * max_drops + i;
-  const DropPlan& p = sc.plan[gi];
+  DropPlan p{};
+  place_rec_unpack(load_rec(sc.prec + gi), p);
+  blur_rec_unpack(load_rec(sc.brec + gi), p);
   CompRec rec;
   rec.x0 = rec.y0 = rec.x1 = rec.y1 = 0;
   rec.ox = rec.oy = rec.pitch = rec.pad = 0;
@@ -1536,7 +1623,8 @@
   const int item = work / GEN_SLICES, slice = work - item * GEN_SLICES;
   const int li = sc.list_gen[(int64_t)f * max_drops + item];
   const int64_t gi = (int64_t)f * max_drops + li;
-  const DropPlan& p = sc.plan[gi];
+  DropPlan p{};
+  tile_rec_unpack(load_rec_uniform(sc.trec + gi), p);
   if (p.kind == KIND_EXT) {
     const double* src = frames[f].ext[li].alpha;
     double* A0e = sc.arena + p.a0_off;
@@ -1645,7 +1733,8 @@
     int j = lo;
     while (boff[j + 1] <= pix) j++;
     const int64_t gi = (int64_t)f * max_drops + lbig[j];
-    const DropPlan& p = sc.plan[gi];
+    DropPlan p{};
+    tile_rec_unpack(load_rec(sc.trec + gi), p);
     const int local = pix - boff[j];
     const int y = local / p.tw, x = local - y * p.tw;
     TexLutWide tx{texels + tex_off[p.tex], s_lut, tex_h[p.tex], tex_w[p.tex]};
@@ -1676,10 +1765,14 @@
   const int64_t gi = sc.list_rot[item];
   __syncthreads();
   PH(7)
-  {
-    const int32_t* src = reinterpret_cast<const int32_t*>(&sc.plan[gi]);
-    int32_t* dst = reinterpret_cast<int32_t*>(&sp);
-    for (int k = t; k < (int)(sizeof(DropPlan) / 4); k += 256) dst[k] = src[k];
+  if (t < 64) {
+    DropPlan q{};
+    tile_rec_unpack(load_rec_uniform(sc.trec + gi), q);
+    const uint32_t* src = reinterpret_cast<const uint32_t*>(&q);
+    uint32_t* dst = reinterpret_cast<uint32_t*>(&sp);
+#pragma unroll
+    for (int k = 0; k < (int)(sizeof(DropPlan) / 4); k++)
+      if (t == (k & 63)) dst[k] = src[k];
   }
   __syncthreads();
   const DropPlan& p = sp;
@@ -2225,20 +2318,16 @@
         if (i < end) {
           pending = i;
           gi = __builtin_amdgcn_readfirstlane(sc.rows_sorted[i]);
-          ptex = __builtin_amdgcn_readfirstlane(as_constant(&sc.plan[gi])->tex);
-          if (__builtin_amdgcn_readfirstlane(as_constant(&sc.plan[gi])->kind) == KIND_BIG) ptex += sc.n_tex;
+          const uint32_t kft = (uint32_t)__builtin_amdgcn_readfirstlane((int)as_constant(&sc.trec[gi])->kft);
+          ptex = (int)(kft >> 8);
+          if ((int)(kft & 3u) == KIND_BIG) ptex += sc.n_tex;
         } else {
           pending = DONE;
         }
       }
       if (pending != DONE && ptex == S.cur) {
-        DropPlan p;
-        {
-          const const_ptr<uint32_t> src = as_constant(reinterpret_cast<const uint32_t*>(&sc.plan[gi]));
-          uint32_t* dst = reinterpret_cast<uint32_t*>(&p);
-#pragma unroll
-          for (int k = 0; k < (int)(sizeof(DropPlan) / 4); k++) dst[k] = src[k];
-        }
+        DropPlan p{};
+        tile_rec_unpack(load_rec_uniform(sc.trec + gi), p);
         PH(0)
         if (ptex < sc.n_tex) {
           rows_tile(p, tex_h[ptex], tex_w[ptex], S, W, sc.arena, three PH_PASS);
@@ -2286,6 +2375,7 @@
 
 constexpr int BLUR_ITEMS_PER_DROP = 8;
 
+__device__ inline int big_lds_cost(int px) { return RR_BIG_COST * ((px + 63) / 64) + 4; }
 __device__ inline int blur_subtiles(const DropPlan& p, const BlurLayout& L) {
   return ((p.ew + L.wo - 1) / L.wo) * ((p.eh + L.ho - 1) / L.ho);
 }
@@ -2295,7 +2385,7 @@
   const int sh = tex_h[p.tex], sw = tex_w[p.tex];
   uint32_t cls, cost = 0u, bcls = LB_NONE, bwh = 0u, bns = 0u;
   if (p.kind == KIND_BIG) {
-    if (sc.big_on && tile_is_big_lds(p, sh, sw)) { cls = LC_BIG_LDS; cost = (uint32_t)(RR_BIG_COST * ((p.tw * p.th + 63) / 64) + 4); }
+    if (sc.big_on && tile_is_big_lds(p, sh, sw)) { cls = LC_BIG_LDS; cost = (uint32_t)(p.tw * p.th); }
     else { cls = LC_BIG; cost = (uint32_t)(p.tw * p.th); }
   } else if (sc.rows_on && p.kind != KIND_EXT && tile_is_rows(p, sh, sw)) { cls = LC_ROWS; cost = (uint32_t)rows_tile_cost(p, sh, sw); }
   else if (p.kind != KIND_EXT && tile_is_fast(p, sh, sw)) cls = p.rs_mode == RS_AREA_FAST ? LC_ROT_INT : LC_ROT;
@@ -2333,9 +2423,9 @@
     if (sc.canon[base + i] == (int)(base + i)) {
       if (cls == LC_BIG_LDS) {
         c[9]++;
-        c[10] += sc.plan[base + i].tw * sc.plan[base + i].th;
+        c[10] += (int)r.y;
         atomicAdd(&s_hist[sc.n_tex + tex], 1);
-        atomicAdd(&s_cost[sc.n_tex + tex], (int)r.y);
+        atomicAdd(&s_cost[sc.n_tex + tex], big_lds_cost((int)r.y));
       } else if (cls == LC_BIG) { c[6]++; c[7] += (int)r.y; }
       else if (cls == LC_ROWS) {
         c[8]++;
@@ -2444,8 +2534,8 @@
   const int64_t base = (int64_t)f * max_drops;
   for (int j = t; j < nf; j += 1024) {
     const int i = sc.rows_list[base + j];
-    const DropPlan& p = sc.plan[base + i];
-    const int tex = p.tex + (p.kind == KIND_BIG ? sc.n_tex : 0);
+    const uint32_t lx = sc.lrec[base + i].x;
+    const int tex = (int)(lx >> 8) + ((lx & 15u) == LC_BIG_LDS ? sc.n_tex : 0);
     const int pos = s_start[tex] + atomicAdd(&s_rank[tex], 1);
     sc.rows_sorted[pos] = (int32_t)(base + i);
   }
@@ -2479,10 +2569,12 @@
   double sigma = 0.0;
   const int64_t gi = (int64_t)f * max_drops + (i < frames[f].n_drops ? i : 0);
   if (i < frames[f].n_drops) {
-    const DropPlan& p = sc.plan[gi];
-    if (p.status == RR_DROP_OK && sc.sizes[gi] != 0 && p.r1 > 0 && p.r1 <= BR_MAX) {
-      r = axis ? p.r2 : p.r1;
-      sigma = axis ? p.sig2 : p.sig1;
+    const uint4 w = reinterpret_cast<const uint4*>(&sc.brec[gi])[2];
+    const int r1 = blur_rec_r1(w.w);
+    if (sc.sizes[gi] != 0 && r1 > 0 && r1 <= BR_MAX) {
+      const double sig1 = __hiloint2double((int)w.y, (int)w.x);
+      r = axis ? blur_rec_r2(w.w) : r1;
+      sigma = axis ? sig1 / 2.0 : sig1;
     }
   }
   double* tab = s_hw[grp];
@@ -2545,6 +2637,24 @@
   }
 }
 
+constexpr int BLUR_REC_DW = (int)(sizeof(BlurRec) / 4);
+static_assert(offsetof(BlurRec, a1_off) == 8 && offsetof(BlurRec, tw) == 16 && offsetof(BlurRec, eh) == 28 && offsetof(BlurRec, epitch) == 40 &&
+              offsetof(BlurRec, rrs) == 44, "BlurRec layout (blur_rec_view, k_scan, k_blur_weights)");
+struct BlurRecView {
+  int r1, r2, tw, th, ew, eh, epitch, epad;
+  long long a0, a1;
+};
+__device__ inline BlurRecView blur_rec_view(uint32_t pv) {
+  auto D = [&](int k) { return (uint32_t)__builtin_amdgcn_readlane((int)pv, k); };
+  BlurRecView o;
+  o.a0 = (long long)(((unsigned long long)D(1) << 32) | D(0));
+  o.a1 = (long long)(((unsigned long long)D(3) << 32) | D(2));
+  o.tw = (int)D(4); o.th = (int)D(5); o.ew = (int)D(6); o.eh = (int)D(7);
+  o.epitch = (int)D(10);
+  const uint32_t rrs = D(11);
+  o.r1 = blur_rec_r1(rrs); o.r2 = blur_rec_r2(rrs); o.epad = blur_rec_epad(rrs);
+  return o;
+}
 __device__ inline void glds_dword(const void* src, uint32_t lds_byte) {
   uint32_t keep;
   asm volatile("s_mov_b32 %0, m0\n\ts_mov_b32 m0, %2\n\ts_nop 0\n\tglobal_load_lds_dword %1, off\n\ts_mov_b32 m0, %0"
@@ -2572,20 +2682,18 @@
   const int n_items = sc.counts[f * 8 + 2];
   if ((int)blockIdx.x >= n_items) return;
   const global_ptr<const uint32_t> items_w = as_global(reinterpret_cast<const uint32_t*>(sc.blur_items + (int64_t)f * max_drops * BLUR_ITEMS_PER_DROP));
-  const DropPlan* plans = sc.plan + (int64_t)f * max_drops;
+  const BlurRec* plans = sc.brec + (int64_t)f * max_drops;
   auto load_item = [&](int item) { return items_w[(int64_t)item * 4 + (lane & 3)]; };
-  auto load_plan = [&](int i) { return as_global(reinterpret_cast<const uint32_t*>(plans + i))[lane]; };
+  auto load_plan = [&](int i) { return as_global(reinterpret_cast<const uint32_t*>(plans + i))[imin(lane, BLUR_REC_DW - 1)]; };
   struct PlanView {
     int r1, r2, ew, eh, tw, th, epitch, epad;
     long long a0_off, a1_off;
   };
   auto unpack = [&](uint32_t pv) {
-    auto F = [&](size_t byte_off) { return (int)__builtin_amdgcn_readlane((int)pv, (int)(byte_off / 4)); };
+    const BlurRecView v = blur_rec_view(pv);
     PlanView o;
-    o.r1 = F(offsetof(DropPlan, r1)); o.r2 = F(offsetof(DropPlan, r2)); o.ew = F(offsetof(DropPlan, ew)); o.eh = F(offsetof(DropPlan, eh));
-    o.tw = F(offsetof(DropPlan, tw)); o.th = F(offsetof(DropPlan, th)); o.epitch = F(offsetof(DropPlan, epitch)); o.epad = F(offsetof(DropPlan, epad));
-    o.a0_off = (long long)(((unsigned long long)(unsigned)F(offsetof(DropPlan, a0_off) + 4) << 32) | (unsigned)F(offsetof(DropPlan, a0_off)));
-    o.a1_off = (long long)(((unsigned long long)(unsigned)F(offsetof(DropPlan, a1_off) + 4) << 32) | (unsigned)F(offsetof(DropPlan, a1_off)));
+    o.r1 = v.r1; o.r2 = v.r2; o.ew = v.ew; o.eh = v.eh; o.tw = v.tw; o.th = v.th; o.epitch = v.epitch; o.epad = v.epad;
+    o.a0_off = v.a0; o.a1_off = v.a1;
     return o;
   };
   auto item_of = [&](uint32_t iv) {
@@ -2764,20 +2872,17 @@
   double* Y = Ys[wave];
   const int n_items = sc.counts[f * 8 + 4];
   const global_ptr<const int32_t> list = as_global(sc.list_small + (int64_t)f * max_drops);
-  const DropPlan* plans = sc.plan + (int64_t)f * max_drops;
+  const BlurRec* plans = sc.brec + (int64_t)f * max_drops;
   const int stride = gridDim.x * 4;
   int it = blockIdx.x * 4 + wave;
   if (it >= n_items) return;
-  auto load_plan = [&](int li) { return as_global(reinterpret_cast<const uint32_t*>(plans + li))[lane]; };
+  auto load_plan = [&](int li) { return as_global(reinterpret_cast<const uint32_t*>(plans + li))[imin(lane, BLUR_REC_DW - 1)]; };
   auto unpack = [&](uint32_t pv, int li) {
-    auto F = [&](size_t byte_off) { return (int)__builtin_amdgcn_readlane((int)pv, (int)(byte_off / 4)); };
-    static_assert(offsetof(DropPlan, a1_off) + 8 <= 256, "DropPlan layout");
+    const BlurRecView v = blur_rec_view(pv);
     SmallItem o;
     o.li = li;
-    o.r1 = F(offsetof(DropPlan, r1)); o.r2 = F(offsetof(DropPlan, r2)); o.tw = F(offsetof(DropPlan, tw)); o.th = F(offsetof(DropPlan, th));
-    o.pw = F(offsetof(DropPlan, ew)); o.ph = F(offsetof(DropPlan, eh)); o.epitch = F(offsetof(DropPlan, epitch)); o.epad = F(offsetof(DropPlan, epad));
-    o.a0 = (long long)(((unsigned long long)(unsigned)F(offsetof(DropPlan, a0_off) + 4) << 32) | (unsigned)F(offsetof(DropPlan, a0_off)));
-    o.a1 = (long long)(((unsigned long long)(unsigned)F(offsetof(DropPlan, a1_off) + 4) << 32) | (unsigned)F(offsetof(DropPlan, a1_off)));
+    o.r1 = v.r1; o.r2 = v.r2; o.tw = v.tw; o.th = v.th; o.pw = v.ew; o.ph = v.eh; o.epitch = v.epitch; o.epad = v.epad;
+    o.a0 = v.a0; o.a1 = v.a1;
     return o;
   };
   double2_v R[4];
@@ -2944,7 +3049,8 @@
   const int n_items = imin(sc.counts[f * 8 + 3], SLOW_CAP);
   for (int w = blockIdx.x; w < 2 * n_items; w += gridDim.x) {
     const int it = w >> 1, axis = w & 1;
-    const DropPlan& p = sc.plan[(int64_t)f * max_drops + sc.list_slow[(int64_t)f * max_drops + it]];
+    DropPlan p{};
+    blur_rec_unpack(load_rec_uniform(sc.brec + (int64_t)f * max_drops + sc.list_slow[(int64_t)f * max_drops + it]), p);
     const int r = axis ? p.r2 : p.r1;
     __syncthreads();
     if (r > 0) {
@@ -2965,7 +3071,8 @@
   for (int w = blockIdx.x; w < n_items * BIG_GROUPS; w += gridDim.x) {
     const int it = w / BIG_GROUPS, g = w - it * BIG_GROUPS;
     const int64_t gi = (int64_t)f * max_drops + sc.list_slow[(int64_t)f * max_drops + it];
-    const DropPlan& p = sc.plan[gi];
+    DropPlan p{};
+    blur_rec_unpack(load_rec_uniform(sc.brec + gi), p);
     const int r = AXIS == 0 ? p.r1 : p.r2;
     const int tw = p.tw, th = p.th, ew = p.ew, eh = p.eh, r1 = p.r1, r2 = p.r2;
     if (AXIS == 0 ? g >= tw : g * BIG_ROWS >= eh) continue;
@@ -3121,11 +3228,12 @@
 }
 
 __global__ __launch_bounds__(256) void k_pad_visits(const FrameDesc* frames, Dims dm, int max_drops, Scratch sc) {
-  const int f = blockIdx.y, i = blockIdx.x * 4 + (threadIdx.x >> 6), lane = threadIdx.x & 63;
+  const int f = blockIdx.y, i = __builtin_amdgcn_readfirstlane((int)(blockIdx.x * 4 + (threadIdx.x >> 6))), lane = threadIdx.x & 63;
   if (i >= frames[f].n_drops) return;
   const int64_t gi = (int64_t)f * max_drops + i;
   if (!sc.blended[gi]) return;
-  const DropPlan& p = sc.plan[gi];
+  DropPlan p{};
+  place_rec_unpack(load_rec_uniform(sc.prec + gi), p);
   const int4 e = sc.bbox[gi];
   const int w = p.vis_w, n = p.vis_w * p.vis_h;
   const int64_t base = (int64_t)f * dm.H * dm.W;
@@ -4661,7 +4769,9 @@
     const size_t fd = (size_t)F * (size_t)(D > 0 ? D : 1);
     const int Hp = (dm.He + 3) & ~3;
     int rc;
-    if ((rc = dev_alloc(ctx, ctx->sc.plan, fd))) return rc;
+    if ((rc = dev_alloc(ctx, ctx->sc.trec, fd))) return rc;
+    if ((rc = dev_alloc(ctx, ctx->sc.brec, fd))) return rc;
+    if ((rc = dev_alloc(ctx, ctx->sc.prec, fd))) return rc;
     if ((rc = dev_alloc(ctx, ctx->sc.comp, fd))) return rc;
     if ((rc = dev_alloc(ctx, ctx->sc.comp32, fd))) return rc;
     if ((rc = dev_alloc(ctx, ctx->sc.npts, fd))) return rc;
@@ -4985,7 +5095,8 @@
       HIPCHK(hipMemsetAsync(sc.bigs_n, 0, sizeof(int32_t) * (size_t)n, bs));
       hipLaunchKernelGGL(k_plan, dim3((max_drops + 127) / 128, n), dim3(128), 0, bs, ctx->d_frames, dm, ctx->cam, ctx->d_tex_h,
                          ctx->d_tex_w, D, fs == bs ? 1 : 0, sc);
-      hipLaunchKernelGGL(k_plan_big, dim3((max_drops + 127) / 128, n), dim3(128), 0, bs, ctx->d_frames, ctx->d_tex_h, ctx->d_tex_w, D, sc);
+      hipLaunchKernelGGL(k_plan_big, dim3(imax(1, imin((max_drops + PB_DROPS - 1) / PB_DROPS, imax(32, 16384 / n))), n), dim3(256), 0, bs, ctx->d_frames,
+                         ctx->d_tex_h, ctx->d_tex_w, D, sc);
     }
     {
       ProfScope ps(ctx, bs, "k_scan");
@@ -5612,7 +5723,9 @@
   hipFree(ctx->d_tex_poff);
   hipFree(ctx->d_ctab);
   hipFree(ctx->d_lut);
-  hipFree(ctx->sc.plan);
+  hipFree(ctx->sc.trec);
+  hipFree(ctx->sc.brec);
+  hipFree(ctx->sc.prec);
   hipFree(ctx->sc.comp);
   hipFree(ctx->sc.comp32);
   hipFree(ctx->sc.poly);
diff --git a/rain-rendering_amd/csrc/rr_device.h b/rain-rendering_amd/csrc/rr_device.h
--- a/rain-rendering_amd/csrc/rr_device.h
+++ b/rain-rendering_amd/csrc/rr_device.h
@@ -49,6 +49,37 @@
   double ma[6];
   double scale_x, scale_y, inv_sx, inv_sy;
 };
+
+struct TileRec {
+  uint32_t kft;
+  int32_t tw, th;
+  int32_t bw0;
+  int64_t a0_off;
+  uint32_t u[2];
+  double m[8];
+};
+static_assert(sizeof(TileRec) == 96, "TileRec is read as 16-byte words");
+
+struct BlurRec {
+  int64_t a0_off, a1_off;
+  int32_t tw, th, ew, eh;
+  double sig1;
+  int32_t epitch;
+  uint32_t rrs;
+};
+static_assert(sizeof(BlurRec) == 48, "BlurRec is read as 16-byte words");
+static_assert(RR_MAX_SHIFT < 2048 && 4 * (RR_MAX_SHIFT + 1) / 10 + 1 < 512 && 2 * (RR_MAX_SHIFT + 1) / 10 + 1 < 256,
+              "BlurRec::rrs: r1 < 512, r2 < 256, shift < 2048");
+
+struct PlaceRec {
+  int32_t status, kind;
+  int32_t vis_x0, vis_y0, vis_w, vis_h;
+  int32_t crop_x, crop_y;
+  int32_t pw, ph;
+  int32_t spare[2];
+  double tau_one, g;
+};
+static_assert(sizeof(PlaceRec) == 64, "PlaceRec is read as 16-byte words");
 
 struct CompRec {
   int32_t x0, y0, x1, y1;
@@ -1120,33 +1151,31 @@
   key[1] = (uint32_t)p.tw | ((uint32_t)p.th << 16);
 }
 
-RR_HD void plan_big_homography(const rr_drop& d, int sw, int sh, double mi[9]) {
+RR_HD void big_system_row(const rr_drop& d, int sw, int sh, int r, double row[8], double& rhs) {
   const double d0 = floor(d.iw1), d1 = floor(d.iw2);
   const int minx = imax(imin(d.x0, d.x1), 0), miny = imax(imin(d.y0, d.y1), 0);
-  float src[4][2] = {{0.f, 0.f}, {(float)sw, 0.f}, {(float)sw, (float)sh}, {0.f, (float)sh}};
-  float dst[4][2];
-  dst[0][0] = (float)(d.x0 - minx);                        dst[0][1] = (float)(d.y0 - miny);
-  dst[1][0] = (float)((double)(d.x0 - minx) + d0);         dst[1][1] = (float)(d.y0 - miny);
-  dst[2][0] = (float)(((double)(d.x1 - minx) + d1) + 0.001); dst[2][1] = (float)(d.y1 - miny);
-  dst[3][0] = (float)((double)(d.x1 - minx) + 0.001);      dst[3][1] = (float)(d.y1 - miny);
+  const int i = r & 3;
+  const float srcx = (i == 1 || i == 2) ? (float)sw : 0.f, srcy = i >= 2 ? (float)sh : 0.f;
+  const float dx0 = (float)(d.x0 - minx), dx1 = (float)((double)(d.x0 - minx) + d0);
+  const float dx2 = (float)(((double)(d.x1 - minx) + d1) + 0.001), dx3 = (float)((double)(d.x1 - minx) + 0.001);
+  const float dstx = i == 0 ? dx0 : (i == 1 ? dx1 : (i == 2 ? dx2 : dx3));
+  const float dsty = i < 2 ? (float)(d.y0 - miny) : (float)(d.y1 - miny);
+  const double sx = srcx, sy = srcy, ddx = dstx, ddy = dsty;
+  const bool top = r < 4;
+  row[0] = top ? sx : 0.0;
+  row[1] = top ? sy : 0.0;
+  row[2] = top ? 1.0 : 0.0;
+  row[3] = top ? 0.0 : sx;
+  row[4] = top ? 0.0 : sy;
+  row[5] = top ? 0.0 : 1.0;
+  row[6] = top ? -sx * ddx : -sx * ddy;
+  row[7] = top ? -sy * ddx : -sy * ddy;
+  rhs = top ? ddx : ddy;
+}
+RR_HD void plan_big_homography(const rr_drop& d, int sw, int sh, double mi[9]) {
   double A[8][8], bb[8], xx[8];
 #pragma unroll
-  for (int i = 0; i < 8; i++)
-#pragma unroll
-    for (int j = 0; j < 8; j++) A[i][j] = 0.0;
-#pragma unroll
-  for (int i = 0; i < 4; i++) {
-    double sx = src[i][0], sy = src[i][1], ddx = dst[i][0], ddy = dst[i][1];
-    A[i][0] = A[i + 4][3] = sx;
-    A[i][1] = A[i + 4][4] = sy;
-    A[i][2] = A[i + 4][5] = 1.0;
-    A[i][6] = -sx * ddx;
-    A[i][7] = -sy * ddx;
-    A[i + 4][6] = -sx * ddy;
-    A[i + 4][7] = -sy * ddy;
-    bb[i] = ddx;
-    bb[i + 4] = ddy;
-  }
+  for (int i = 0; i < 8; i++) big_system_row(d, sw, sh, i, A[i], bb[i]);
   solve8(A, bb, xx);
   double M[9] = {xx[0], xx[1], xx[2], xx[3], xx[4], xx[5], xx[6], xx[7], 1.0};
   invert3(M, mi);
@@ -1313,6 +1342,113 @@
   size_out = (p.vis_w > 0 && p.vis_h > 0) ? (((int64_t)p.tw * p.th + 15) & ~15LL) + (p.r1 > 0 ? (((int64_t)p.epitch * p.eh + 15) & ~15LL) : 0) : 0;
 }
 
+RR_HD void tile_rec_pack(const DropPlan& p, TileRec& r) {
+  r.kft = (uint32_t)p.kind | ((uint32_t)(p.flip & 1) << 2) | ((uint32_t)p.rs_mode << 4) | ((uint32_t)p.tex << 8);
+  r.tw = p.tw;
+  r.th = p.th;
+  r.bw0 = p.bw0;
+  r.a0_off = p.a0_off;
+  if (p.kind == KIND_BIG) {
+    for (int k = 0; k < 8; k++) r.m[k] = p.mi[k];
+    uint64_t b;
+    __builtin_memcpy(&b, &p.mi[8], 8);
+    r.u[0] = (uint32_t)b;
+    r.u[1] = (uint32_t)(b >> 32);
+  } else {
+    for (int k = 0; k < 6; k++) r.m[k] = p.ma[k];
+    r.m[6] = p.scale_x;
+    r.m[7] = p.scale_y;
+    r.u[0] = (uint32_t)p.nW;
+    r.u[1] = (uint32_t)p.nH;
+  }
+}
+RR_HD void tile_rec_unpack(const TileRec& r, DropPlan& p) {
+  p.kind = (int32_t)(r.kft & 3u);
+  p.flip = (int32_t)((r.kft >> 2) & 1u);
+  p.rs_mode = (int32_t)((r.kft >> 4) & 3u);
+  p.tex = (int32_t)(r.kft >> 8);
+  p.tw = r.tw;
+  p.th = r.th;
+  p.bw0 = r.bw0;
+  p.a0_off = r.a0_off;
+  const bool big = p.kind == KIND_BIG;
+  for (int k = 0; k < 8; k++) p.mi[k] = big ? r.m[k] : 0.0;
+  const uint64_t b = big ? ((uint64_t)r.u[0] | ((uint64_t)r.u[1] << 32)) : 0ull;
+  __builtin_memcpy(&p.mi[8], &b, 8);
+  for (int k = 0; k < 6; k++) p.ma[k] = big ? 0.0 : r.m[k];
+  p.scale_x = big ? 1.0 : r.m[6];
+  p.scale_y = big ? 1.0 : r.m[7];
+  p.nW = big ? 0 : (int32_t)r.u[0];
+  p.nH = big ? 0 : (int32_t)r.u[1];
+  const bool resized = p.kind == KIND_ROT && p.nW > 0 && p.nH > 0;
+  p.inv_sx = resized ? (double)p.tw / (double)p.nW : 1.0;
+  p.inv_sy = resized ? (double)p.th / (double)p.nH : 1.0;
+  const bool fast = p.rs_mode == RS_AREA_FAST;
+  p.isx = fast ? (int32_t)cv_round(p.scale_x) : 1;
+  p.isy = fast ? (int32_t)cv_round(p.scale_y) : 1;
+}
+
+RR_HD void blur_rec_pack(const DropPlan& p, BlurRec& r) {
+  r.a0_off = p.a0_off;
+  r.a1_off = p.a1_off;
+  r.tw = p.tw;
+  r.th = p.th;
+  r.ew = p.ew;
+  r.eh = p.eh;
+  r.sig1 = p.sig1;
+  r.epitch = p.epitch;
+  r.rrs = ((uint32_t)p.r1 & 511u) | (((uint32_t)p.r2 & 255u) << 9) | (((uint32_t)p.shift & 2047u) << 17) | (((uint32_t)p.epad & 15u) << 28);
+}
+RR_HD int32_t blur_rec_r1(uint32_t rrs) { return (int32_t)(rrs & 511u); }
+RR_HD int32_t blur_rec_r2(uint32_t rrs) { return (int32_t)((rrs >> 9) & 255u); }
+RR_HD int32_t blur_rec_shift(uint32_t rrs) { return (int32_t)((rrs >> 17) & 2047u); }
+RR_HD int32_t blur_rec_epad(uint32_t rrs) { return (int32_t)(rrs >> 28); }
+RR_HD void blur_rec_unpack(const BlurRec& r, DropPlan& p) {
+  p.a0_off = r.a0_off;
+  p.a1_off = r.a1_off;
+  p.tw = r.tw;
+  p.th = r.th;
+  p.ew = r.ew;
+  p.eh = r.eh;
+  p.sig1 = r.sig1;
+  p.sig2 = r.sig1 / 2.0;
+  p.epitch = r.epitch;
+  p.r1 = blur_rec_r1(r.rrs);
+  p.r2 = blur_rec_r2(r.rrs);
+  p.shift = blur_rec_shift(r.rrs);
+  p.epad = blur_rec_epad(r.rrs);
+}
+
+RR_HD void place_rec_pack(const DropPlan& p, PlaceRec& r) {
+  r.status = p.status;
+  r.kind = p.kind;
+  r.vis_x0 = p.vis_x0;
+  r.vis_y0 = p.vis_y0;
+  r.vis_w = p.vis_w;
+  r.vis_h = p.vis_h;
+  r.crop_x = p.crop_x;
+  r.crop_y = p.crop_y;
+  r.pw = p.pw;
+  r.ph = p.ph;
+  r.spare[0] = r.spare[1] = 0;
+  r.tau_one = p.tau_one;
+  r.g = p.g;
+}
+RR_HD void place_rec_unpack(const PlaceRec& r, DropPlan& p) {
+  p.status = r.status;
+  p.kind = r.kind;
+  p.vis_x0 = r.vis_x0;
+  p.vis_y0 = r.vis_y0;
+  p.vis_w = r.vis_w;
+  p.vis_h = r.vis_h;
+  p.crop_x = r.crop_x;
+  p.crop_y = r.crop_y;
+  p.pw = r.pw;
+  p.ph = r.ph;
+  p.tau_one = r.tau_one;
+  p.g = r.g;
+}
+
 RR_HD double blur_axis0(const double* src, int pw, int ph, int x, int y, const double* hw, int r) {
   double acc = src[(int64_t)y * pw + x] * hw[r];
   for (int ii = -r; ii < 0; ii++) {
```

Result: faster. 18950 (median of 6 runs) (+2.6%).
